# algoterranean/3dgan

Hardware: AMD Instinct MI355X
Metric: images/sec (whole node), CIFAR-10 IWGAN bs=512 (higher is better)
Workload: dtype bf16; 1 GPU; --model iwgan --dataset cifar(32x32x3 synthetic) --batch_size 512/GPU --latent_size 200 --optimizer adam --lr 1e-4 --beta1 0.5 --beta2 0.9 --n_disc_train 5; one step = 5 D + 1 G optimizer steps on 6 fresh batches; global_batch=512, parallelism=dp1, ranks_seen=1

## Files before the change

### 3dgan_amd/_lib.py

```python
import ctypes as C
import os

_HERE = os.path.dirname(os.path.abspath(__file__))
LIB_PATH = os.environ.get('TDG_LIB_PATH') or os.path.join(_HERE, 'lib3dgan_hip.so')

F32, BF16 = 0, 1
ACT_NONE, ACT_RELU, ACT_LRELU, ACT_TANH, ACT_SIGMOID = 0, 1, 2, 3, 4
MASK_NONE, MASK_LRELU, MASK_RELU = 0, 1, 2
COL_NONE, COL_SUM, COL_BN = 0, 1, 2


class ConvDesc(C.Structure):
    _fields_ = [(n, C.c_int32) for n in
                ('n', 'h', 'w', 'c', 'cs', 'oh', 'ow', 'k', 'ks', 'kh', 'kw', 'stride', 'pad_t', 'pad_l', 'dtype')]


class Epilogue(C.Structure):
    _fields_ = [('bias', C.c_void_p), ('act', C.c_int32), ('leak', C.c_float),
                ('mask_mode', C.c_int32), ('mask_src', C.c_void_p), ('accumulate', C.c_int32),
                ('col_partial', C.c_void_p), ('col_partial_bytes', C.c_size_t), ('col_mode', C.c_int32),
                ('col_images', C.c_int32), ('col_nblk_out', C.POINTER(C.c_int32)),
                ('splitk_ws', C.c_void_p), ('splitk_ws_bytes', C.c_size_t)]


class PackJob(C.Structure):
    _fields_ = [('desc', ConvDesc), ('w', C.c_void_p), ('packed_fwd', C.c_void_p), ('packed_bwd', C.c_void_p)]


class LaunchRecord(C.Structure):
    _fields_ = [('kernel', C.c_char * 64), ('ms', C.c_double), ('flops', C.c_double)]


_vp, _i, _f, _sz, _u64 = C.c_void_p, C.c_int, C.c_float, C.c_size_t, C.c_uint64
_PD, _PE = C.POINTER(ConvDesc), C.POINTER(Epilogue)

SIGNATURES = {
    'tdg_last_error': (C.c_char_p, []),
    'tdg_version': (_i, []),
    'tdg_last_kernel': (C.c_char_p, []),
    'tdg_timing_begin': (_i, []),
    'tdg_timing_end': (_i, [C.POINTER(LaunchRecord), _i, C.POINTER(_i)]),
    'tdg_packed_filter_fwd_bytes': (_sz, [_PD]),
    'tdg_packed_filter_bwd_bytes': (_sz, [_PD]),
    'tdg_pack_filter_fwd': (_i, [_PD, _vp, _vp, _vp]),
    'tdg_pack_filter_bwd': (_i, [_PD, _vp, _vp, _vp]),
    'tdg_pack_filters': (_i, [C.POINTER(PackJob), _i, _vp]),
    'tdg_conv2d_fwd': (_i, [_PD, _i, _vp, _vp, _vp, _PE, _vp]),
    'tdg_conv2d_bwd_data': (_i, [_PD, _i, _vp, _vp, _vp, _PE, _vp]),
    'tdg_conv2d_bwd_filter_workspace_bytes': (_sz, [_PD, _i]),
    'tdg_conv2d_bwd_filter': (_i, [_PD, _i, _vp, _vp, _vp, _f, _vp, _sz, _vp]),
    'tdg_conv2d_bwd_filter2': (_i, [_PD, _i, _vp, _i, _vp, _vp, _vp, _f, _vp, _sz, _vp]),
    'tdg_conv2d_dispatch': (_i, [_PD, _i, _i, _PE, _i, C.c_char_p, _sz]),
    'tdg_rowdot': (_i, [_i, _vp, _i, _i, _vp, _vp, _i, _vp, _vp]),
    'tdg_rowouter': (_i, [_i, _vp, _vp, _i, _i, _i, _f, _vp, _vp, _vp]),
    'tdg_col_finalize_sum': (_i, [_vp, _i, _i, _vp, _f, _vp]),
    'tdg_instance_norm_fwd': (_i, [_i, _vp, _i, _i, _i, _i, _vp, _vp, _f, _i, _f, _vp, _i, _vp, _vp]),
    'tdg_instance_norm_bwd': (_i, [_i, _vp, _i, _vp, _i, _i, _i, _i, _vp, _vp, _vp, _i, _f, _vp, _vp, _vp, _f, _vp, _sz, _vp]),
    'tdg_add_act': (_i, [_i, _vp, _vp, _sz, _i, _f, _vp, _vp]),
    'tdg_bn_fwd_from_partials': (_i, [_i, _vp, _i, _i, _i, _vp, _f, _i, _f, _vp, _vp, _i, _vp, _vp, _i, _vp, _vp]),
    'tdg_colsum_weighted': (_i, [_i, _vp, _i, _i, _i, _vp, _vp, _f, _vp, _sz, _vp]),
    'tdg_colsum_workspace_bytes': (_sz, [_i, _i]),
    'tdg_bn_workspace_bytes': (_sz, [_i, _i]),
    'tdg_bn_fwd': (_i, [_i, _vp, _i, _i, _i, _vp, _f, _i, _f, _vp, _vp, _i, _vp, _vp, _sz, _vp]),
    'tdg_bn_fwd_groups': (_i, [_i, _vp, _i, _i, _i, _i, _vp, _f, _i, _f, _vp, _vp, _i, _vp, _vp, _sz, _vp]),
    'tdg_bn_bwd': (_i, [_i, _vp, _i, _vp, _i, _i, _i, _vp, _vp, _i, _f, _vp, _vp, _f, _vp, _f, _vp, _sz, _vp]),
    'tdg_affine_cast_pair': (_i, [_i, _vp, _i, _vp, _i, _sz, _f, _f, _vp, _vp, _vp]),
    'tdg_bias_act': (_i, [_i, _vp, _i, _i, _i, _vp, _i, _f, _vp, _vp]),
    'tdg_act_bwd': (_i, [_i, _vp, _vp, _sz, _i, _f, _vp, _vp]),
    'tdg_affine_cast': (_i, [_i, _vp, _sz, _f, _f, _vp, _vp]),
    'tdg_affine_cast_rows': (_i, [_i, _vp, _i, _i, _i, _f, _f, _vp, _vp]),
    'tdg_cast_to_f32': (_i, [_i, _vp, _sz, _vp, _vp]),
    'tdg_cast_from_f32': (_i, [_i, _vp, _sz, _vp, _vp]),
    'tdg_gp_interp': (_i, [_i, _vp, _vp, _vp, _i, _i, _vp, _vp]),
    'tdg_sumsq': (_i, [_i, _vp, _sz, _vp, _f, _vp, _sz, _vp]),
    'tdg_reduce_workspace_bytes': (_sz, [_sz]),
    'tdg_mean_f32': (_i, [_vp, _i, _vp, _vp]),
    'tdg_sum_f32': (_i, [_vp, _i, _vp, _f, _vp]),
    'tdg_mean_segments_f32': (_i, [_vp, _i, _i, _vp, _vp]),
    'tdg_gan_logloss': (_i, [_vp, _vp, _i, _vp, _vp, _vp, _vp, _vp]),
    'tdg_p2p_xent': (_i, [_i, _vp, _i, _i, _i, _vp, _vp, _vp]),
    'tdg_p2p_l1': (_i, [_i, _vp, _vp, _i, _i, _f, _vp, _i, _vp, _vp, _sz, _vp]),
    'tdg_cgan_prep': (_i, [_i, _vp, _i, _i, _vp, _i, _vp, _vp, _vp, _vp, _i, _vp, _i, _vp]),
    'tdg_cgan_head_fwd': (_i, [_i, _vp, _i, _i, _i, _i, _i, _vp, _vp, _vp, _vp, _vp, _i, _vp]),
    'tdg_cgan_head_bwd': (_i, [_i, _vp, _i, _vp, _i, _i, _i, _i, _i, _vp, _i, _f, _vp, _vp, _vp, _vp, _sz, _vp]),
    'tdg_cgan_head_noise_fwd': (_i, [_i, _vp, _i, _i, _i, _i, _i, _vp, _vp, _vp, _vp, _vp, _vp, _vp, _i, _vp]),
    'tdg_cgan_head_noise_bwd': (_i, [_i, _vp, _i, _vp, _i, _i, _i, _i, _i, _vp, _vp, _i, _f, _vp, _vp, _vp, _vp, _sz, _vp]),
    'tdg_cgan_join': (_i, [_i, _i, _i, _i, _i, _vp, _i, _vp, _i, _vp, _i, _vp]),
    'tdg_cgan_wgan_loss': (_i, [_i, _vp, _i, _i, _i, _vp, _vp, _vp]),
    'tdg_cgan_metrics': (_i, [_vp, _vp, _vp, _i, _i, _vp, _vp, _vp, _sz, _vp]),
    'tdg_cgan_metrics_workspace_bytes': (_sz, []),
    'tdg_cgan_eval_batch': (_i, [_vp, _vp, _vp, _vp, _f, _i, _i, _i, _vp, _vp, _vp, _sz, _vp]),
    'tdg_cgan_eval_workspace_bytes': (_sz, []),
    'tdg_cgan_eval_acc_bytes': (_sz, [_i]),
    'tdg_cgan_eval_moments': (_i, [_vp, _i, _i, _vp, _vp]),
    'tdg_cgan_eval_finish': (_i, [_vp, _vp, _i, _f, _vp, _vp, _vp, _vp]),
    'tdg_cgan_sample_stats': (_i, [_vp, _vp, _vp, _vp, _vp, _f, _i, _i, _f, _vp, _vp, _vp, _vp, _sz, _vp]),
    'tdg_cgan_sample_stats_workspace_bytes': (_sz, [_i, _i]),
    'tdg_cgan_rmse_loss': (_i, [_i, _vp, _vp, _i, _i, _vp, _i, _vp, _vp, _sz, _vp]),
    'tdg_cgan_rmse_loss_workspace_bytes': (_sz, [_i, _i]),
    'tdg_cgan_bar_fill': (_i, [_i, _vp, _i, _i, _vp, _i, _vp, _vp]),
    'tdg_mde_loss': (_i, [_i, _vp, _i, _i, _vp, _i, _vp, _vp, _i, _vp, _vp, _sz, _vp]),
    'tdg_mde_loss_workspace_bytes': (_sz, [_i]),
    'tdg_xsamp_prep': (_i, [_i, _vp, _vp, _vp, _vp, _vp, _vp, _vp, _i, _i, _i, _i, _vp, _i, _vp, _i, _vp, _i, _vp, _vp]),
    'tdg_xsamp_head_fwd': (_i, [_i, _vp, _i, _i, _i, _i, _vp, _vp, _vp, _vp, _i, _vp]),
    'tdg_xsamp_head_bwd': (_i, [_i, _vp, _i, _vp, _vp, _i, _i, _i, _i, _vp, _i, _f, _vp, _vp, _vp, _vp, _sz, _vp]),
    'tdg_cgan_full_gather': (_i, [_vp, _vp, _i, _i, _i, _vp, _i, _vp, _vp, _vp]),
    'tdg_cgan_full_store': (_i, [_vp, _vp, _i, C.c_longlong, _vp, _vp, _vp, _vp]),
    'tdg_cgan_full_blend': (_i, [_vp, _vp, C.c_longlong, _i, _i, _i, _i, _vp, _vp, _vp]),
    'tdg_cgan_full_rmse': (_i, [_vp, _vp, _i, _i, _vp, _vp, _sz, _vp]),
    'tdg_cgan_full_gather_rep': (_i, [_vp, _vp, _i, _i, _i, _vp, _i, _i, _vp, _vp, _vp]),
    'tdg_cgan_full_sample_store': (_i, [_vp, _vp, _vp, _i, _i, C.c_longlong, _vp, _vp, _vp, _vp, _vp, _vp]),
    'tdg_vae_reparam': (_i, [_i, _vp, _i, _vp, _i, _i, _i, _vp, _i, _vp]),
    'tdg_vae_reparam_bwd': (_i, [_i, _vp, _i, _vp, _i, _i, _i, _vp, _i, _vp]),
    'tdg_vae_reparam_bwd_kl': (_i, [_i, _vp, _i, _vp, _i, _vp, _i, _f, _i, _i, _vp, _i, _vp]),
    'tdg_gp_rows': (_i, [_i, _vp, _i, _i, _f, _vp, _vp, _vp]),
    'tdg_vae_kl': (_i, [_i, _vp, _i, _i, _i, _vp, _vp, _sz, _vp]),
    'tdg_vae_bce': (_i, [_i, _vp, _vp, _i, _i, _i, _vp, _vp, _vp, _sz, _vp]),
    'tdg_dropout': (_i, [_i, _vp, _i, _i, _i, _vp, _f, _vp]),
    'tdg_l1_loss': (_i, [_i, _vp, _vp, _i, _i, _i, _f, _f, _vp, _vp, _vp, _sz, _vp]),
    'tdg_gp_scalars': (_i, [_vp, _f, _vp, _vp]),
    'tdg_gp_sumsq': (_i, [_i, _vp, _sz, _vp, _f, _vp, _vp, _sz, _vp]),
    'tdg_scale_by_dev': (_i, [_i, _vp, _sz, _vp, _vp, _vp]),
    'tdg_fill_f32': (_i, [_vp, _sz, _f, _vp]),
    'tdg_bias_grad': (_i, [_i, _vp, _i, _i, _i, _vp, _f, _vp, _sz, _vp]),
    'tdg_adam_step': (_i, [_vp, _vp, _vp, _vp, _sz, _f, _f, _f, _f, _f, _vp]),
    'tdg_adam_step_dev': (_i, [_vp, _vp, _vp, _vp, _sz, _f, _f, _f, _f, _f, _vp, _vp]),
    'tdg_add_i32': (_i, [_vp, _i, _vp]),
    'tdg_rmsprop_step': (_i, [_vp, _vp, _vp, _vp, _sz, _f, _f, _f, _f, _f, _vp]),
    'tdg_rmsprop_centered_step': (_i, [_vp, _vp, _vp, _vp, _vp, _sz, _f, _f, _f, _f, _f, _vp]),
    'tdg_adagrad_step': (_i, [_vp, _vp, _vp, _sz, _f, _f, _vp]),
    'tdg_adadelta_step': (_i, [_vp, _vp, _vp, _vp, _sz, _f, _f, _f, _f, _vp]),
    'tdg_ftrl_step': (_i, [_vp, _vp, _vp, _vp, _sz, _f, _f, _f, _f, _vp]),
    'tdg_sgd_momentum_step': (_i, [_vp, _vp, _vp, _sz, _f, _f, _f, _vp]),
    'tdg_clamp': (_i, [_vp, _sz, _f, _f, _vp]),
    'tdg_check_finite': (_i, [_vp, _sz, _vp, _vp]),
# ... 43 lines not shown
```

### 3dgan_amd/csrc/tdg_elementwise.hip

```cpp
#include <stdarg.h>

#include <atomic>

#include "tdg_common.h"
#include <type_traits>

static thread_local char g_err[512] = "";
void tdg_set_error(const char* fmt, ...) {
  va_list ap;
  va_start(ap, fmt);
  vsnprintf(g_err, sizeof(g_err), fmt, ap);
  va_end(ap);
}
extern "C" const char* tdg_last_error(void) { return g_err; }
extern "C" int tdg_version(void) { return 100; }
static thread_local const char* g_last_kernel = "";
void tdg_note_kernel(const char* name) { g_last_kernel = name; }
extern "C" const char* tdg_last_kernel(void) { return g_last_kernel; }

#include <vector>
struct TimingSlot { const char* name; double flops; hipEvent_t e0, e1; };
static std::vector<TimingSlot> g_slots;
static int g_timing_on = 0, g_timing_n = 0;
bool tdg_timing_enabled() { return g_timing_on != 0; }
void tdg_timing_start(const char* name, double flops, hipStream_t s) {
  if (!g_timing_on) return;
  if (g_timing_n == (int)g_slots.size()) {
    TimingSlot t;
    t.name = ""; t.flops = 0;
    (void)hipEventCreate(&t.e0);
    (void)hipEventCreate(&t.e1);
    g_slots.push_back(t);
  }
  TimingSlot& t = g_slots[g_timing_n];
  t.name = name;
  t.flops = flops;
  (void)hipEventRecord(t.e0, s);
}
void tdg_timing_stop(hipStream_t s) {
  if (!g_timing_on) return;
  (void)hipEventRecord(g_slots[g_timing_n].e1, s);
  ++g_timing_n;
}
extern "C" int tdg_timing_begin(void) {
  g_timing_on = 1;
  g_timing_n = 0;
  return TDG_OK;
}
extern "C" int tdg_timing_end(TdgLaunchRecord* out, int capacity, int* count) {
  g_timing_on = 0;
  TDG_CHECK_ARG(count != nullptr, "tdg_timing_end: null count");
  int n = 0;
  for (int i = 0; i < g_timing_n; ++i) {
    if (hipEventSynchronize(g_slots[i].e1) != hipSuccess) { tdg_set_error("tdg_timing_end: event sync failed"); return TDG_EHIP; }
    float ms = 0.f;
    (void)hipEventElapsedTime(&ms, g_slots[i].e0, g_slots[i].e1);
    if (out && n < capacity) {
      strncpy(out[n].kernel, g_slots[i].name, sizeof(out[n].kernel) - 1);
      out[n].kernel[sizeof(out[n].kernel) - 1] = 0;
      out[n].ms = ms;
      out[n].flops = g_slots[i].flops;
    }
    ++n;
  }
  *count = n;
  g_timing_n = 0;
  return TDG_OK;
}

static inline int ew_blocks(size_t n, int per_block = 1024) {
  size_t b = (n + per_block - 1) / per_block;
  return (int)(b < 1 ? 1 : (b > 4096 ? 4096 : b));
}

__device__ __forceinline__ float wave_sum(float v) {
#pragma unroll
  for (int o = 32; o > 0; o >>= 1) v += __shfl_down(v, o, 64);
  return v;
}

__device__ __forceinline__ float block_sum256(float v, float* sh ) {
  v = wave_sum(v);
  if ((threadIdx.x & 63) == 0) sh[threadIdx.x >> 6] = v;
  __syncthreads();
  float r = 0.f;
  if (threadIdx.x == 0) r = sh[0] + sh[1] + sh[2] + sh[3];
  __syncthreads();
// ... 134 lines not shown
  const int CL = g.CL, RL = 256 / CL;
  const int tx = threadIdx.x % CL, ty = threadIdx.x / CL;
  const int r0 = blockIdx.x * g.rows_per_blk;
  const int r1 = min(g.rows, r0 + g.rows_per_blk);
  const T* x = static_cast<const T*>(a.x) + (size_t)blockIdx.z * g.rows * g.xcs;
  const T* y = static_cast<const T*>(a.y);
  float* const partial = a.partial + (size_t)blockIdx.z * gridDim.x * 2 * g.C;
  const int c = (blockIdx.y * CL + tx) * VW;
  Acc s0[VW], s1[VW];
#pragma unroll
  for (int e = 0; e < VW; ++e) s0[e] = s1[e] = 0;
  if (c < g.C) {
    float pivot[VW], bta[VW];
#pragma unroll
    for (int e = 0; e < VW; ++e) pivot[e] = bta[e] = 0.f;
    if (MODE == COL_BN_STATS) load_vw<T, VW>(x + c, pivot);
    if (MODE == COL_BN_BWD) {
#pragma unroll
      for (int e = 0; e < VW; ++e) bta[e] = a.beta[c + e];
    }
    for (int rb = r0 + ty; rb < r1; rb += 4 * RL) {
      float v4[4][VW], p4[4][VW];
#pragma unroll
      for (int u = 0; u < 4; ++u) {
        const int r = rb + u * RL;
        if (r < r1) {
          load_vw<T, VW>(x + (size_t)r * g.xcs + c, v4[u]);
          if (MODE == COL_BN_BWD) load_vw<T, VW>(y + (size_t)r * g.cs + c, p4[u]);
        }
      }
#pragma unroll
      for (int u = 0; u < 4; ++u) {
        const int r = rb + u * RL;
        if (r >= r1) continue;
        float (&v)[VW] = v4[u];
        if (MODE == COL_BN_STATS) {
#pragma unroll
          for (int e = 0; e < VW; ++e) { const float d = v[e] - pivot[e]; s0[e] += d; s1[e] += d * d; }
        } else if (MODE == COL_BN_BWD) {
          float (&pre)[VW] = p4[u];
#pragma unroll
          for (int e = 0; e < VW; ++e) {
            const float dpre = v[e] * act_deriv_from_pre(pre[e], a.act, a.leak);
            s0[e] += dpre; s1[e] += dpre * (pre[e] - bta[e]);
          }
        } else if (MODE == COL_SUM) {
#pragma unroll
          for (int e = 0; e < VW; ++e) s0[e] += v[e];
        } else {
          const float k = a.coef ? a.coef[r] : 1.f;
#pragma unroll
          for (int e = 0; e < VW; ++e) s0[e] += v[e] * k;
        }
      }
    }
  }
#pragma unroll
  for (int e = 0; e < VW; ++e) { sh[0][e][threadIdx.x] = s0[e]; sh[1][e][threadIdx.x] = s1[e]; }
  __syncthreads();
  if (ty == 0 && c < g.C) {
#pragma unroll
    for (int e = 0; e < VW; ++e) {
      Acc t0 = 0, t1 = 0;
      for (int k = 0; k < RL; ++k) { t0 += sh[0][e][k * CL + tx]; t1 += sh[1][e][k * CL + tx]; }
      partial[((size_t)blockIdx.x * 2 + 0) * g.C + c + e] = (float)t0;
      partial[((size_t)blockIdx.x * 2 + 1) * g.C + c + e] = (float)t1;
    }
  }
}

enum { FIN_BN_STATS = 0, FIN_BN_BWD = 1, FIN_ACC = 2, FIN_ACC2 = 3 };
struct FinArgs {
  const float* partial; int nblk, C, rows;
  const void* x0;
  const float* pivot_f;
  float eps;
  float* out0;
  float* out1;
  float beta_acc;
  long long x0_group;
};
#define FIN_CH 8
template <typename T, int MODE, int CH>
__global__ void __launch_bounds__(256) col_finalize_kernel(const FinArgs a) {
  constexpr int RL = 256 / CH;
  using Acc = typename std::conditional<sizeof(T) == 4, double, float>::type;
  __shared__ Acc sh[2][RL][CH];
  const int tx = threadIdx.x & (CH - 1), ty = threadIdx.x / CH;
  const int c = blockIdx.x * CH + tx;
  const float* const partial = a.partial + (size_t)blockIdx.y * a.nblk * 2 * a.C;
  Acc s0 = 0, s1 = 0;
  if (c < a.C)
    for (int b0 = ty; b0 < a.nblk; b0 += 4 * RL) {
      float p0[4], p1[4];
#pragma unroll
      for (int u = 0; u < 4; ++u) {
        const int b = b0 + RL * u;
        const bool ok = b < a.nblk;
        p0[u] = ok ? partial[((size_t)b * 2 + 0) * a.C + c] : 0.f;
        p1[u] = (ok && MODE != FIN_ACC) ? partial[((size_t)b * 2 + 1) * a.C + c] : 0.f;
      }
#pragma unroll
      for (int u = 0; u < 4; ++u) { s0 += p0[u]; s1 += p1[u]; }
    }
  sh[0][ty][tx] = s0;
  sh[1][ty][tx] = s1;
  __syncthreads();
  if (ty != 0 || c >= a.C) return;
  s0 = s1 = 0;
#pragma unroll
  for (int k = 0; k < RL; ++k) { s0 += sh[0][k][tx]; s1 += sh[1][k][tx]; }
  const Acc inv = (Acc)1 / (Acc)a.rows;
  if (MODE == FIN_BN_STATS) {
    const float pivot = a.pivot_f ? a.pivot_f[c] : (a.x0 ? to_f32<T>(static_cast<const T*>(a.x0)[(size_t)blockIdx.y * a.x0_group + c]) : 0.f);
    const Acc md = s0 * inv;
    const Acc var = s1 * inv - md * md > 0 ? s1 * inv - md * md : 0;
    float* const out = a.out0 + (size_t)blockIdx.y * 2 * a.C;
    out[c] = (float)(pivot + md);
    out[a.C + c] = (float)(1.0 / sqrt((double)var + (double)a.eps));
  } else if (MODE == FIN_BN_BWD) {
    a.out0[c] = (float)((a.beta_acc != 0.f ? (Acc)a.beta_acc * a.out0[c] : 0) + s0);
    a.out1[c] = (float)(s0 * inv);
    a.out1[a.C + c] = (float)(s1 * inv);
  } else if (MODE == FIN_ACC2) {
    a.out0[c] = (float)((a.beta_acc != 0.f ? (Acc)a.beta_acc * a.out0[c] : 0) + s0);
    a.out1[c] = (float)((a.beta_acc != 0.f ? (Acc)a.beta_acc * a.out1[c] : 0) + s1);
  } else {
    a.out0[c] = (float)((a.beta_acc != 0.f ? (Acc)a.beta_acc * a.out0[c] : 0) + s0);
  }
}
template <typename T, int MODE>
static void launch_col_finalize(const FinArgs& f, hipStream_t s, int ngroups = 1) {
  if (f.nblk >= 1024)
    hipLaunchKernelGGL((col_finalize_kernel<T, MODE, 2>), dim3((f.C + 1) / 2, ngroups), dim3(256), 0, s, f);
  else
    hipLaunchKernelGGL((col_finalize_kernel<T, MODE, FIN_CH>), dim3((f.C + FIN_CH - 1) / FIN_CH, ngroups), dim3(256), 0, s, f);
}

template <typename T, int VW>
__device__ __forceinline__ void store_vw(T* p, const float (&v)[VW]) {
  if constexpr (VW == 1) {
    p[0] = from_f32<T>(v[0]);
  } else if constexpr (sizeof(T) == 4) {
    *reinterpret_cast<f32x4*>(p) = f32x4{v[0], v[1], v[2], v[3]};
  } else {
    *reinterpret_cast<bf16x4*>(p) = bf16x4{(bf16_t)v[0], (bf16_t)v[1], (bf16_t)v[2], (bf16_t)v[3]};
  }
}

template <typename T, int VW>
__global__ void __launch_bounds__(256) bn_fwd_apply_kernel(const ColGeom g, const T* __restrict__ u,
                                                          const float* __restrict__ beta, const float* __restrict__ stats,
                                                          int act, float leak, T* __restrict__ pre, T* __restrict__ h, int hcs) {
  const int CL = g.CL, RL = 256 / CL, C = g.C;
  const int tx = threadIdx.x % CL, ty = threadIdx.x / CL;
  const int c = (blockIdx.y * CL + tx) * VW;
  if (c >= C) return;
  stats += (size_t)blockIdx.z * 2 * C;
  u += (size_t)blockIdx.z * g.rows * g.cs;
  if (pre) pre += (size_t)blockIdx.z * g.rows * g.cs;
  h += (size_t)blockIdx.z * g.rows * hcs;
  float mean[VW], rstd[VW], b[VW];
#pragma unroll
  for (int e = 0; e < VW; ++e) { mean[e] = stats[c + e]; rstd[e] = stats[C + c + e]; b[e] = beta[c + e]; }
  for (int r = blockIdx.x * RL + ty; r < g.rows; r += gridDim.x * RL) {
    const size_t i = (size_t)r * g.cs + c;
    float v[VW], p[VW], a[VW];
    load_vw<T, VW>(u + i, v);
#pragma unroll
    for (int e = 0; e < VW; ++e) { p[e] = (v[e] - mean[e]) * rstd[e] + b[e]; a[e] = apply_act(p[e], act, leak); }
    if (pre) store_vw<T, VW>(pre + i, p);
    store_vw<T, VW>(h + (size_t)r * hcs + c, a);
  }
}

template <typename T, int VW, bool DB>
__global__ void __launch_bounds__(256) bn_bwd_apply_kernel(const ColGeom g, const T* __restrict__ dh, int dhcs, const T* __restrict__ pre,
                                                          const float* __restrict__ beta, const float* __restrict__ stats,
                                                          const float* __restrict__ sums, int act, float leak, T* __restrict__ du,
                                                          float* __restrict__ db_partial) {
  __shared__ float sh[DB ? VW : 1][DB ? 256 : 1];
  const int CL = g.CL, RL = 256 / CL, C = g.C;
  const int tx = threadIdx.x % CL, ty = threadIdx.x / CL;
  const int c = (blockIdx.y * CL + tx) * VW;
  const bool okc = c < C;
  if (!DB && !okc) return;
  float rstd[VW], b[VW], m0[VW], m1[VW], acc[VW];
#pragma unroll
  for (int e = 0; e < VW; ++e) {
    rstd[e] = okc ? stats[C + c + e] : 0.f; b[e] = okc ? beta[c + e] : 0.f; m0[e] = okc ? sums[c + e] : 0.f; m1[e] = okc ? sums[C + c + e] : 0.f;
    acc[e] = 0.f;
  }
  if (okc)
    for (int r = blockIdx.x * RL + ty; r < g.rows; r += gridDim.x * RL) {
      const size_t i = (size_t)r * g.cs + c;
      float d[VW], p[VW], o[VW];
      load_vw<T, VW>(dh + (size_t)r * dhcs + c, d);
      load_vw<T, VW>(pre + i, p);
#pragma unroll
      for (int e = 0; e < VW; ++e) {
        const float f = act_deriv_from_pre(p[e], act, leak);
        o[e] = rstd[e] * (d[e] * f - m0[e] - (p[e] - b[e]) * m1[e]);
        if (DB) acc[e] += to_f32<T>(from_f32<T>(o[e]));
      }
      store_vw<T, VW>(du + i, o);
    }
  if constexpr (DB) {
#pragma unroll
    for (int e = 0; e < VW; ++e) sh[e][threadIdx.x] = acc[e];
    __syncthreads();
    if (ty == 0 && okc) {
#pragma unroll
// ... 127 lines not shown

extern "C" int tdg_bn_bwd(int dtype, const void* dh, int dh_cs, const void* pre, int rows, int c, int cs, const float* beta,
                          const float* stats, int act, float leak, void* du, float* dbeta, float beta_acc,
                          float* dbias, float dbias_acc, void* workspace, size_t workspace_bytes, void* stream) {
  TDG_CHECK_ARG(dh && pre && beta && stats && du && dbeta && workspace, "tdg_bn_bwd: null pointer");
  TDG_CHECK_ARG(rows > 0 && c > 0 && cs >= c && dh_cs >= c, "tdg_bn_bwd: bad shape");
  if (workspace_bytes < tdg_bn_workspace_bytes(rows, c)) { tdg_set_error("tdg_bn_bwd: workspace too small"); return TDG_EWORKSPACE; }
  hipStream_t s = (hipStream_t)stream;
  ColGeom g = col_geom(rows, c, cs, dh, pre, tdg_dtype_size(dtype), dh_cs % 4 == 0);
  g.xcs = dh_cs;
  ColArgs a; memset(&a, 0, sizeof(a));
  a.x = dh; a.y = pre; a.beta = beta; a.act = act; a.leak = leak; a.partial = static_cast<float*>(workspace);
  float* sums = a.partial + (size_t)1024 * 2 * c;
  FinArgs f; memset(&f, 0, sizeof(f));
  f.partial = a.partial; f.nblk = g.nblk; f.C = c; f.rows = rows; f.out0 = dbeta; f.out1 = sums; f.beta_acc = beta_acc;
  ColGeom ga = col_geom(rows, c, cs, dh, (const void*)((uintptr_t)pre | (uintptr_t)du), tdg_dtype_size(dtype), dh_cs % 4 == 0);
  ga.xcs = dh_cs;
  int arows = apply_row_blocks(ga);
  if (dbias && arows > 1024) arows = 1024;
  const dim3 agrid(arows, ga.ncol);
  FinArgs fb; memset(&fb, 0, sizeof(fb));
  fb.partial = a.partial; fb.nblk = arows; fb.C = c; fb.rows = rows; fb.out0 = dbias; fb.beta_acc = dbias_acc;
  DISPATCH_T(dtype, {
    int rc = run_col_partial<T, COL_BN_BWD>(g, a, s);
    if (rc) return rc;
    launch_col_finalize<T, FIN_BN_BWD>(f, s);
    if (dbias) {
      if (ga.vw == 4)
        hipLaunchKernelGGL((bn_bwd_apply_kernel<T, 4, true>), agrid, dim3(256), 0, s, ga, static_cast<const T*>(dh), dh_cs,
                           static_cast<const T*>(pre), beta, stats, sums, act, leak, static_cast<T*>(du), a.partial);
      else
        hipLaunchKernelGGL((bn_bwd_apply_kernel<T, 1, true>), agrid, dim3(256), 0, s, ga, static_cast<const T*>(dh), dh_cs,
                           static_cast<const T*>(pre), beta, stats, sums, act, leak, static_cast<T*>(du), a.partial);
      launch_col_finalize<T, FIN_ACC>(fb, s);
    } else {
      if (ga.vw == 4)
        hipLaunchKernelGGL((bn_bwd_apply_kernel<T, 4, false>), agrid, dim3(256), 0, s, ga, static_cast<const T*>(dh), dh_cs,
                           static_cast<const T*>(pre), beta, stats, sums, act, leak, static_cast<T*>(du), nullptr);
      else
        hipLaunchKernelGGL((bn_bwd_apply_kernel<T, 1, false>), agrid, dim3(256), 0, s, ga, static_cast<const T*>(dh), dh_cs,
                           static_cast<const T*>(pre), beta, stats, sums, act, leak, static_cast<T*>(du), nullptr);
    }
  })
  TDG_HIP_LAUNCH_CHECK("bn_bwd");
  return TDG_OK;
}

extern "C" int tdg_bias_grad(int dtype, const void* dy, int rows, int c, int cs, float* db, float beta, void* workspace,
                             size_t workspace_bytes, void* stream) {
  TDG_CHECK_ARG(dy && db && workspace && rows > 0 && c > 0 && cs >= c, "tdg_bias_grad: bad argument");
  if (workspace_bytes < tdg_bn_workspace_bytes(rows, c)) { tdg_set_error("tdg_bias_grad: workspace too small"); return TDG_EWORKSPACE; }
  hipStream_t s = (hipStream_t)stream;
  const ColGeom g = col_geom(rows, c, cs, dy, nullptr, tdg_dtype_size(dtype));
  ColArgs a; memset(&a, 0, sizeof(a));
  a.x = dy; a.partial = static_cast<float*>(workspace);
  FinArgs f; memset(&f, 0, sizeof(f));
  f.partial = a.partial; f.nblk = g.nblk; f.C = c; f.rows = rows; f.out0 = db; f.beta_acc = beta;
  DISPATCH_T(dtype, {
    int rc = run_col_partial<T, COL_SUM>(g, a, s);
    if (rc) return rc;
    launch_col_finalize<T, FIN_ACC>(f, s);
  })
  TDG_HIP_LAUNCH_CHECK("bias_grad");
  return TDG_OK;
}

extern "C" int tdg_colsum_weighted(int dtype, const void* x, int rows, int cols, int cs, const float* coef, float* dw,
                                   float beta, void* workspace, size_t workspace_bytes, void* stream) {
  TDG_CHECK_ARG(x && dw && workspace && rows > 0 && cols > 0 && cs >= cols, "tdg_colsum_weighted: bad argument");
  if (workspace_bytes < tdg_bn_workspace_bytes(rows, cols)) { tdg_set_error("tdg_colsum_weighted: workspace too small"); return TDG_EWORKSPACE; }
  hipStream_t s = (hipStream_t)stream;
  const ColGeom g = col_geom(rows, cols, cs, x, nullptr, tdg_dtype_size(dtype));
  ColArgs a; memset(&a, 0, sizeof(a));
  a.x = x; a.coef = coef; a.partial = static_cast<float*>(workspace);
  FinArgs f; memset(&f, 0, sizeof(f));
  f.partial = a.partial; f.nblk = g.nblk; f.C = cols; f.rows = rows; f.out0 = dw; f.beta_acc = beta;
  DISPATCH_T(dtype, {
    int rc = run_col_partial<T, COL_WSUM>(g, a, s);
    if (rc) return rc;
    launch_col_finalize<T, FIN_ACC>(f, s);
  })
  TDG_HIP_LAUNCH_CHECK("colsum_weighted");
  return TDG_OK;
}

template <typename T>
__global__ void __launch_bounds__(256) instance_norm_fwd_kernel(const T* __restrict__ u, int hw, int c, int cs,
                                                               const float* __restrict__ scale, const float* __restrict__ shift, float eps,
                                                               int act, float leak, T* __restrict__ h, int hcs, float* __restrict__ stats) {
  __shared__ float sh[2][4][64];
  const int n = blockIdx.x, tx = threadIdx.x & 63, ty = threadIdx.x >> 6;
  const int ch = blockIdx.y * 64 + tx;
  const bool okc = ch < c;
  const T* un = u + (size_t)n * hw * cs;
  const float pivot = okc ? to_f32<T>(un[ch]) : 0.f;
  float s0 = 0.f, s1 = 0.f;
  if (okc)
    for (int r = ty; r < hw; r += 4) { const float d = to_f32<T>(un[(size_t)r * cs + ch]) - pivot; s0 += d; s1 += d * d; }
  sh[0][ty][tx] = s0; sh[1][ty][tx] = s1;
  __syncthreads();
  s0 = sh[0][0][tx] + sh[0][1][tx] + sh[0][2][tx] + sh[0][3][tx];
  s1 = sh[1][0][tx] + sh[1][1][tx] + sh[1][2][tx] + sh[1][3][tx];
  if (!okc) return;
  const float md = s0 / (float)hw, var = fmaxf(s1 / (float)hw - md * md, 0.f);
  const float mu = pivot + md, rstd = rsqrtf(var + eps);
  if (ty == 0) { stats[((size_t)n * 2 + 0) * c + ch] = mu; stats[((size_t)n * 2 + 1) * c + ch] = rstd; }
  const float g = scale[ch], b = shift[ch];
  T* hn = h + (size_t)n * hw * hcs;
  for (int r = ty; r < hw; r += 4)
    hn[(size_t)r * hcs + ch] = from_f32<T>(apply_act(g * (to_f32<T>(un[(size_t)r * cs + ch]) - mu) * rstd + b, act, leak));
}
extern "C" int tdg_instance_norm_fwd(int dtype, const void* u, int n, int hw, int c, int cs, const float* scale, const float* shift,
                                     float eps, int act, float leak, void* h, int h_cs, float* stats, void* stream) {
  TDG_CHECK_ARG(u && scale && shift && h && stats && n > 0 && hw > 0 && c > 0 && cs >= c && h_cs >= c, "tdg_instance_norm_fwd: bad argument");
  DISPATCH_T(dtype, {
    hipLaunchKernelGGL(instance_norm_fwd_kernel<T>, dim3(n, (c + 63) / 64), dim3(256), 0, (hipStream_t)stream, static_cast<const T*>(u),
                       hw, c, cs, scale, shift, eps, act, leak, static_cast<T*>(h), h_cs, stats);
  })
  TDG_HIP_LAUNCH_CHECK("instance_norm_fwd");
  return TDG_OK;
}
template <typename T>
__global__ void __launch_bounds__(256) instance_norm_bwd_kernel(const T* __restrict__ dh, int dhcs, const T* __restrict__ u, int hw, int c,
                                                               int cs, const float* __restrict__ scale, const float* __restrict__ shift,
                                                               const float* __restrict__ stats, int act, float leak, T* __restrict__ du,
                                                               float* __restrict__ part) {
  __shared__ float sh[2][4][64];
  const int n = blockIdx.x, tx = threadIdx.x & 63, ty = threadIdx.x >> 6;
  const int ch = blockIdx.y * 64 + tx;
  const bool okc = ch < c;
  const T* un = u + (size_t)n * hw * cs;
  const T* dn = dh + (size_t)n * hw * dhcs;
  const float mu = okc ? stats[((size_t)n * 2 + 0) * c + ch] : 0.f, rstd = okc ? stats[((size_t)n * 2 + 1) * c + ch] : 0.f;
  const float g0 = okc ? scale[ch] : 0.f, b0 = okc ? shift[ch] : 0.f;
  float s0 = 0.f, s1 = 0.f;
  if (okc)
    for (int r = ty; r < hw; r += 4) {
      const float xh = (to_f32<T>(un[(size_t)r * cs + ch]) - mu) * rstd;
      const float g = to_f32<T>(dn[(size_t)r * dhcs + ch]) * act_deriv_from_pre(g0 * xh + b0, act, leak);
      s0 += g; s1 += g * xh;
    }
  sh[0][ty][tx] = s0; sh[1][ty][tx] = s1;
  __syncthreads();
  s0 = sh[0][0][tx] + sh[0][1][tx] + sh[0][2][tx] + sh[0][3][tx];
  s1 = sh[1][0][tx] + sh[1][1][tx] + sh[1][2][tx] + sh[1][3][tx];
  if (!okc) return;
  if (ty == 0) { part[((size_t)n * 2 + 0) * c + ch] = s1; part[((size_t)n * 2 + 1) * c + ch] = s0; }
  const float m0 = s0 / (float)hw, m1 = s1 / (float)hw;
  T* dun = du + (size_t)n * hw * cs;
  for (int r = ty; r < hw; r += 4) {
    const float xh = (to_f32<T>(un[(size_t)r * cs + ch]) - mu) * rstd;
    const float g = to_f32<T>(dn[(size_t)r * dhcs + ch]) * act_deriv_from_pre(g0 * xh + b0, act, leak);
    dun[(size_t)r * cs + ch] = from_f32<T>(g0 * rstd * (g - m0 - xh * m1));
  }
}
extern "C" int tdg_instance_norm_bwd(int dtype, const void* dh, int dh_cs, const void* u, int n, int hw, int c, int cs,
                                     const float* scale, const float* shift, const float* stats, int act, float leak, void* du,
                                     float* dscale, float* dshift, float beta, void* workspace, size_t workspace_bytes, void* stream) {
  TDG_CHECK_ARG(dh && u && scale && shift && stats && du && dscale && dshift && workspace && n > 0 && hw > 0 && c > 0 && cs >= c && dh_cs >= c,
                "tdg_instance_norm_bwd: bad argument");
  if (workspace_bytes < (size_t)n * 2 * c * sizeof(float)) { tdg_set_error("tdg_instance_norm_bwd: workspace too small"); return TDG_EWORKSPACE; }
  float* part = static_cast<float*>(workspace);
  FinArgs f; memset(&f, 0, sizeof(f));
  f.partial = part; f.nblk = n; f.C = c; f.rows = 1; f.out0 = dscale; f.out1 = dshift; f.beta_acc = beta;
  DISPATCH_T(dtype, {
    hipLaunchKernelGGL(instance_norm_bwd_kernel<T>, dim3(n, (c + 63) / 64), dim3(256), 0, (hipStream_t)stream, static_cast<const T*>(dh),
// ... 208 lines not shown
  }
  for (size_t i = blockIdx.x * (size_t)256 + threadIdx.x; i < n; i += (size_t)gridDim.x * 256) {
    const size_t r = i / c;
    const int ch = (int)(i - r * c);
    out[r * cs + ch] = from_f32<T>(scale * (in[i] + shift));
  }
}
template <typename T>
__global__ void __launch_bounds__(256) affine_cast_pair_kernel(const float* __restrict__ a, int ca, const float* __restrict__ b, int cb,
                                                              size_t rows, float scale, float shift, T* __restrict__ out_ab,
                                                              T* __restrict__ out_a0) {
  for (size_t r = blockIdx.x * (size_t)256 + threadIdx.x; r < rows; r += (size_t)gridDim.x * 256) {
    float v[4] = {0.f, 0.f, 0.f, 0.f}, w[4] = {0.f, 0.f, 0.f, 0.f};
    for (int ch = 0; ch < ca; ++ch) v[ch] = w[ch] = scale * (a[r * ca + ch] + shift);
    for (int ch = 0; ch < cb; ++ch) v[ca + ch] = scale * (b[r * cb + ch] + shift);
    store_vw<T, 4>(out_ab + r * 4, v);
    store_vw<T, 4>(out_a0 + r * 4, w);
  }
}
extern "C" int tdg_affine_cast_pair(int dtype, const float* a, int ca, const float* b, int cb, size_t rows, float scale, float shift,
                                    void* out_ab, void* out_a0, void* stream) {
  TDG_CHECK_ARG(a && b && out_ab && out_a0 && rows > 0 && ca > 0 && cb > 0 && ca + cb == 4, "tdg_affine_cast_pair: bad argument");
  TDG_CHECK_ARG((((uintptr_t)out_ab | (uintptr_t)out_a0) & 15) == 0, "tdg_affine_cast_pair: outputs must be 16-byte aligned");
  DISPATCH_T(dtype, {
    hipLaunchKernelGGL(affine_cast_pair_kernel<T>, dim3(ew_blocks(rows)), dim3(256), 0, (hipStream_t)stream, a, ca, b, cb, rows, scale,
                       shift, static_cast<T*>(out_ab), static_cast<T*>(out_a0));
  })
  TDG_HIP_LAUNCH_CHECK("affine_cast_pair");
  return TDG_OK;
}

extern "C" int tdg_affine_cast_rows(int dtype, const float* in, int rows, int c, int cs, float scale, float shift, void* out,
                                    void* stream) {
  TDG_CHECK_ARG(in && out && rows > 0 && c > 0 && cs >= c, "tdg_affine_cast_rows: bad argument");
  const size_t n = (size_t)rows * c;
  DISPATCH_T(dtype, {
    hipLaunchKernelGGL(affine_cast_rows_kernel<T>, dim3(ew_blocks(n)), dim3(256), 0, (hipStream_t)stream, in, n, c, cs, scale,
                       shift, static_cast<T*>(out));
  })
  TDG_HIP_LAUNCH_CHECK("affine_cast_rows");
  return TDG_OK;
}
extern "C" int tdg_cast_from_f32(int dtype, const float* in, size_t n, void* out, void* stream) {
  return tdg_affine_cast(dtype, in, n, 1.f, 0.f, out, stream);
}

template <typename T>
__global__ void __launch_bounds__(256) cast_to_f32_kernel(const T* __restrict__ in, size_t n, float* __restrict__ out) {
  for (size_t i = blockIdx.x * (size_t)256 + threadIdx.x; i < n; i += (size_t)gridDim.x * 256) out[i] = to_f32<T>(in[i]);
}
extern "C" int tdg_cast_to_f32(int dtype, const void* in, size_t n, float* out, void* stream) {
  TDG_CHECK_ARG(in && out && n > 0, "tdg_cast_to_f32: bad argument");
  DISPATCH_T(dtype, {
    hipLaunchKernelGGL(cast_to_f32_kernel<T>, dim3(ew_blocks(n)), dim3(256), 0, (hipStream_t)stream, static_cast<const T*>(in),
                       n, out);
  })
  TDG_HIP_LAUNCH_CHECK("cast_to_f32");
  return TDG_OK;
}

template <typename T>
__global__ void __launch_bounds__(256) gp_interp_kernel(const T* __restrict__ x, const T* __restrict__ g,
                                                       const float* __restrict__ alpha, int rows, int cols, T* __restrict__ xhat) {
  for (int r = blockIdx.x; r < rows; r += gridDim.x) {
    const float al = alpha[r];
    for (int c = threadIdx.x; c < cols; c += 256) {
      const size_t i = (size_t)r * cols + c;
      const float xv = to_f32<T>(x[i]);
      xhat[i] = from_f32<T>(xv + al * (to_f32<T>(g[i]) - xv));
    }
  }
}
extern "C" int tdg_gp_interp(int dtype, const void* x, const void* g, const float* alpha, int rows, int cols, void* xhat,
                             void* stream) {
  TDG_CHECK_ARG(x && g && alpha && xhat && rows > 0 && cols > 0, "tdg_gp_interp: bad argument");
  DISPATCH_T(dtype, {
    hipLaunchKernelGGL(gp_interp_kernel<T>, dim3(rows < 4096 ? rows : 4096), dim3(256), 0, (hipStream_t)stream,
                       static_cast<const T*>(x), static_cast<const T*>(g), alpha, rows, cols, static_cast<T*>(xhat));
  })
  TDG_HIP_LAUNCH_CHECK("gp_interp");
  return TDG_OK;
}

#define RED_BLOCKS 256
extern "C" size_t tdg_reduce_workspace_bytes(size_t) { return RED_BLOCKS * sizeof(float); }

template <typename T>
__global__ void __launch_bounds__(256) sumsq_partial_kernel(const T* __restrict__ x, size_t n, float* __restrict__ partial,
                                                           float* __restrict__ acc, float beta, float gp_lambda = 0.f,
                                                           float* __restrict__ gp_scal = nullptr) {
  __shared__ float sh[4];
  float s = 0.f;
  constexpr int VW = 16 / (int)sizeof(T);
  if ((((uintptr_t)x) & 15) == 0) {
    const size_t nv = n / VW;
    for (size_t i = blockIdx.x * (size_t)256 + threadIdx.x; i < nv; i += (size_t)gridDim.x * 256) {
      float v[VW];
      if constexpr (sizeof(T) == 2) {
        const bf16x8 t = reinterpret_cast<const bf16x8*>(x)[i];
#pragma unroll
        for (int e = 0; e < 8; ++e) v[e] = (float)t[e];
      } else {
        const f32x4 t = reinterpret_cast<const f32x4*>(x)[i];
#pragma unroll
        for (int e = 0; e < 4; ++e) v[e] = t[e];
      }
#pragma unroll
      for (int e = 0; e < VW; ++e) s += v[e] * v[e];
    }
    for (size_t i = nv * VW + blockIdx.x * (size_t)256 + threadIdx.x; i < n; i += (size_t)gridDim.x * 256) {
      const float v = to_f32<T>(x[i]);
      s += v * v;
    }
  } else {
    for (size_t i = blockIdx.x * (size_t)256 + threadIdx.x; i < n; i += (size_t)gridDim.x * 256) {
      const float v = to_f32<T>(x[i]);
      s += v * v;
    }
  }
  s = block_sum256(s, sh);
  if (threadIdx.x == 0) partial[blockIdx.x] = s;
  if (!last_block_arrives(TICKET_SUMSQ, gridDim.x)) return;
  float t = 0.f;
  for (int i = threadIdx.x; i < (int)gridDim.x; i += 256) t += partial[i];
  t = block_sum256(t, sh);
  if (threadIdx.x == 0) {
    const float ss = (beta != 0.f ? beta * acc[0] : 0.f) + t;
    acc[0] = ss;
    if (gp_scal) {
      const float sl = sqrtf(ss);
      gp_scal[0] = (sl - 1.f) * (sl - 1.f);
      gp_scal[1] = gp_lambda * 2.f * (sl - 1.f) / sl;
    }
  }
}
__global__ void __launch_bounds__(256) reduce_final_kernel(const float* __restrict__ partial, int np, float* __restrict__ acc,
                                                          float beta, float scale) {
  __shared__ float sh[4];
  const float* p = partial + (size_t)blockIdx.x * np;
  float s = 0.f;
  for (int i = threadIdx.x; i < np; i += 256) s += p[i];
  s = block_sum256(s, sh);
  if (threadIdx.x == 0) acc[blockIdx.x] = (beta != 0.f ? beta * acc[blockIdx.x] : 0.f) + scale * s;
}
__global__ void __launch_bounds__(256) reduce_mean_kernel(const float* __restrict__ partial, int np, float* __restrict__ out) {
  __shared__ float sh[4];
  const float* p = partial + (size_t)blockIdx.x * np;
  float s = 0.f;
  for (int i = threadIdx.x; i < np; i += 256) s += p[i];
  s = block_sum256(s, sh);
  if (threadIdx.x == 0) out[blockIdx.x] = s / (float)np;
}
extern "C" int tdg_sumsq(int dtype, const void* x, size_t n, float* acc, float beta, void* workspace,
                         size_t workspace_bytes, void* stream) {
  TDG_CHECK_ARG(x && acc && workspace && n > 0, "tdg_sumsq: bad argument");
  if (workspace_bytes < RED_BLOCKS * sizeof(float)) { tdg_set_error("tdg_sumsq: workspace too small"); return TDG_EWORKSPACE; }
  TDG_TICKET_STREAM("tdg_sumsq", stream);
  DISPATCH_T(dtype, {
    hipLaunchKernelGGL(sumsq_partial_kernel<T>, dim3(RED_BLOCKS), dim3(256), 0, (hipStream_t)stream, static_cast<const T*>(x),
                       n, static_cast<float*>(workspace), acc, beta);
  })
  TDG_HIP_LAUNCH_CHECK("sumsq");
  return TDG_OK;
}
extern "C" int tdg_gp_sumsq(int dtype, const void* x, size_t n, float* sumsq, float lambda, float* scal, void* workspace,
                            size_t workspace_bytes, void* stream) {
  TDG_CHECK_ARG(x && sumsq && scal && workspace && n > 0, "tdg_gp_sumsq: bad argument");
  if (workspace_bytes < RED_BLOCKS * sizeof(float)) { tdg_set_error("tdg_gp_sumsq: workspace too small"); return TDG_EWORKSPACE; }
  TDG_TICKET_STREAM("tdg_gp_sumsq", stream);
  DISPATCH_T(dtype, {
    hipLaunchKernelGGL(sumsq_partial_kernel<T>, dim3(RED_BLOCKS), dim3(256), 0, (hipStream_t)stream, static_cast<const T*>(x),
                       n, static_cast<float*>(workspace), sumsq, 0.f, lambda, scal);
  })
  TDG_HIP_LAUNCH_CHECK("gp_sumsq");
  return TDG_OK;
}
extern "C" int tdg_mean_segments_f32(const float* x, int nseg, int seglen, float* out, void* stream) {
  TDG_CHECK_ARG(x && out && nseg > 0 && nseg <= 65535 && seglen > 0, "tdg_mean_segments_f32: bad argument");
  hipLaunchKernelGGL(reduce_mean_kernel, dim3(nseg), dim3(256), 0, (hipStream_t)stream, x, seglen, out);
  TDG_HIP_LAUNCH_CHECK("mean_segments_f32");
  return TDG_OK;
}
extern "C" int tdg_sum_f32(const float* x, int n, float* out, float beta, void* stream) {
  TDG_CHECK_ARG(x && out && n > 0, "tdg_sum_f32: bad argument");
  hipLaunchKernelGGL(reduce_final_kernel, dim3(1), dim3(256), 0, (hipStream_t)stream, x, n, out, beta, 1.f);
  TDG_HIP_LAUNCH_CHECK("sum_f32");
  return TDG_OK;
}
extern "C" int tdg_mean_f32(const float* x, int n, float* out, void* stream) {
  TDG_CHECK_ARG(x && out && n > 0, "tdg_mean_f32: bad argument");
  hipLaunchKernelGGL(reduce_mean_kernel, dim3(1), dim3(256), 0, (hipStream_t)stream, x, n, out);
  TDG_HIP_LAUNCH_CHECK("mean_f32");
  return TDG_OK;
}

__global__ void __launch_bounds__(256) gan_logloss_kernel(const float* __restrict__ dr, const float* __restrict__ df, int n,
                                                         float* __restrict__ sr, float* __restrict__ sfd, float* __restrict__ sfg,
                                                         float* __restrict__ scal) {
  __shared__ float sh[4];
  float ld = 0.f, lg = 0.f;
  const float inv = 1.f / (float)n;
  for (int i = threadIdx.x; i < n; i += 256) {
    const float r = dr[i], f = df[i];
    ld += -logf(r + 1e-8f) - logf(1.f - f + 1e-8f);
    lg += -logf(f + 1e-8f);
    sr[i] = -inv / (r + 1e-8f) * r * (1.f - r);
    sfd[i] = inv / (1.f - f + 1e-8f) * f * (1.f - f);
    sfg[i] = -inv / (f + 1e-8f) * f * (1.f - f);
  }
  ld = block_sum256(ld, sh);
  lg = block_sum256(lg, sh);
  if (threadIdx.x == 0) { scal[0] = ld * inv; scal[1] = lg * inv; }
}
extern "C" int tdg_gan_logloss(const float* d_real, const float* d_fake, int n, float* seed_real, float* seed_fake_d,
                               float* seed_fake_g, float* scal, void* stream) {
  TDG_CHECK_ARG(d_real && d_fake && seed_real && seed_fake_d && seed_fake_g && scal && n > 0, "tdg_gan_logloss: bad argument");
  hipLaunchKernelGGL(gan_logloss_kernel, dim3(1), dim3(256), 0, (hipStream_t)stream, d_real, d_fake, n, seed_real, seed_fake_d,
                     seed_fake_g, scal);
  TDG_HIP_LAUNCH_CHECK("gan_logloss");
  return TDG_OK;
}

template <typename T>
__global__ void __launch_bounds__(256) p2p_xent_kernel(const T* __restrict__ z, int rows, int cs, int mode, T* __restrict__ seed,
                                                      float* __restrict__ scal) {
  __shared__ float sh[4];
  float dr = 0.f, df = 0.f, gf = 0.f;
  const float inv = 1.f / (float)rows;
  for (int i = threadIdx.x; i < rows; i += 256) {
    const float zr = to_f32<T>(z[(size_t)i * cs]), zf = to_f32<T>(z[(size_t)(rows + i) * cs]);
    const float sr = log1pf(expf(-fabsf(zr))), sf = log1pf(expf(-fabsf(zf)));
    dr += fmaxf(zr, 0.f) - zr + sr;
    df += fmaxf(zf, 0.f) + sf;
    gf += fmaxf(zf, 0.f) - zf + sf;
    if (mode) {
      const float pr = 1.f / (1.f + expf(-zr)), pf = 1.f / (1.f + expf(-zf));
      seed[(size_t)i * cs] = from_f32<T>(mode == 1 ? (pr - 1.f) * inv : 0.f);
      seed[(size_t)(rows + i) * cs] = from_f32<T>(mode == 1 ? pf * inv : (pf - 1.f) * inv);
    }
  }
  dr = block_sum256(dr, sh);
  df = block_sum256(df, sh);
  gf = block_sum256(gf, sh);
  if (threadIdx.x == 0) { scal[0] = dr * inv; scal[1] = df * inv; scal[2] = gf * inv; }
}
extern "C" int tdg_p2p_xent(int dtype, const void* logits, int rows, int cs, int mode, void* seed, float* scal, void* stream) {
  TDG_CHECK_ARG(logits && scal && rows > 0 && cs > 0 && (mode == 0 || seed), "tdg_p2p_xent: bad argument");
  DISPATCH_T(dtype, {
    hipLaunchKernelGGL(p2p_xent_kernel<T>, dim3(1), dim3(256), 0, (hipStream_t)stream, static_cast<const T*>(logits), rows, cs,
                       mode, static_cast<T*>(seed), scal);
  })
  TDG_HIP_LAUNCH_CHECK("p2p_xent");
  return TDG_OK;
}
template <typename T>
__global__ void __launch_bounds__(256) p2p_l1_kernel(const T* __restrict__ y, const T* __restrict__ g, int rows, int cs, float wgt,
                                                    T* __restrict__ dg, int dgs, float* __restrict__ partial) {
  __shared__ float sh[4];
  float a = 0.f, q = 0.f;
  const float inv = 1.f / (float)rows;
  for (int i = blockIdx.x * 256 + threadIdx.x; i < rows; i += gridDim.x * 256) {
    const float d = 0.5f * (to_f32<T>(g[(size_t)i * cs]) - to_f32<T>(y[(size_t)i * cs]));
    a += fabsf(d);
    q += d * d;
    if (dg) {
      const float s = d > 0.f ? 1.f : (d < 0.f ? -1.f : 0.f);
      dg[(size_t)i * dgs] = from_f32<T>(to_f32<T>(dg[(size_t)i * dgs]) + wgt * 0.5f * s * inv);
    }
  }
  a = block_sum256(a, sh);
  q = block_sum256(q, sh);
  if (threadIdx.x == 0) { partial[blockIdx.x] = a; partial[RED_BLOCKS + blockIdx.x] = q; }
}
__global__ void __launch_bounds__(256) p2p_l1_final_kernel(const float* __restrict__ partial, int rows, float* __restrict__ scal) {
  __shared__ float sh[4];
  float a = 0.f, q = 0.f;
// ... 584 lines not shown
```

### 3dgan_amd/csrc/tdg_igemm.hip

```cpp
#include <stdarg.h>
#include <stdlib.h>

#include "tdg_igemm.h"
#include "tdg_wgrad_patch.h"
#include <type_traits>

#define OOB_OFFSET 0xFFFFFF00u

#ifdef TDG_STAMPS
#define TDG_STAMP(var)                                                                            \
  do {                                                                                            \
    __builtin_amdgcn_sched_barrier(0);                                                            \
    asm volatile("s_memtime %0\n\ts_waitcnt lgkmcnt(0)" : "=s"(var)::"memory");                  \
    __builtin_amdgcn_sched_barrier(0);                                                            \
  } while (0)
#else
#define TDG_STAMP(var) do { } while (0)
#endif

template <int I, int N, class F>
__device__ __forceinline__ void static_for(F&& f) {
  if constexpr (I < N) {
    f(IntC<I>{});
    static_for<I + 1, N>(f);
  }
}

template <typename T>
struct Mma;
template <>
struct Mma<bf16_t> {
  using frag = bf16x8;
  static __device__ __forceinline__ void run(f32x4& acc, const frag& a, const frag& b) {
    acc = __builtin_amdgcn_mfma_f32_16x16x32_bf16(a, b, acc, 0, 0, 0);
  }
};
template <>
struct Mma<float> {
  using frag = f32x4;
  static __device__ __forceinline__ void run(f32x4& acc, const frag& a, const frag& b) {
#pragma unroll
    for (int e = 0; e < 4; ++e) acc = __builtin_amdgcn_mfma_f32_16x16x4f32(a[e], b[e], acc, 0, 0, 0);
  }
};

__device__ __forceinline__ __amdgpu_buffer_rsrc_t make_rsrc(const void* p, unsigned bytes) {
  return __builtin_amdgcn_make_buffer_rsrc(const_cast<void*>(p), 0, (int)bytes, 0x00020000);
}

__device__ __forceinline__ i32x4 make_rsrc_words(const void* p, unsigned bytes) {
  const unsigned long long a = (unsigned long long)p;
  return i32x4{(int)(unsigned)a, (int)((unsigned)(a >> 32) & 0xffffu), (int)bytes, 0x00020000};
}
__device__ __forceinline__ void lds_dma_b128(const i32x4& rsrc, unsigned voff, unsigned lds_byte) {
  asm volatile("s_mov_b32 m0, %2\n\ts_nop 0\n\tbuffer_load_dwordx4 %0, %1, 0 offen lds" ::"v"(voff), "s"(rsrc), "s"(lds_byte) : "memory");
}

template <typename T>
__device__ __forceinline__ T buffer_load_elem(__amdgpu_buffer_rsrc_t r, unsigned off);
template <>
__device__ __forceinline__ float buffer_load_elem<float>(__amdgpu_buffer_rsrc_t r, unsigned off) {
  return __builtin_bit_cast(float, __builtin_amdgcn_raw_buffer_load_b32(r, off, 0, 0));
}
template <>
__device__ __forceinline__ bf16_t buffer_load_elem<bf16_t>(__amdgpu_buffer_rsrc_t r, unsigned off) {
  return __builtin_bit_cast(bf16_t, __builtin_amdgcn_raw_buffer_load_b16(r, off, 0, 0));
}

__device__ __forceinline__ int tap_dh(int pk) { return (pk << 24) >> 24; }
__device__ __forceinline__ int tap_dw(int pk) { return (pk << 16) >> 24; }

__device__ __forceinline__ int lds_swz(int row, int chunk) {
  return row * IG_BKB + ((chunk ^ ((row >> 1) & 7)) << 4);
}

struct KChunk { int tap, cv; bool ok; };
__device__ __forceinline__ KChunk k_decode(unsigned chunk, const FastDiv& fd_ck, const FastDiv& fd_nt, int nslices) {
  const unsigned u = fd_div(chunk, fd_ck);
  const unsigned j = chunk - u * fd_ck.d;
  const unsigned sl = fd_div(u, fd_nt);
  KChunk r;
  r.tap = (int)(u - sl * fd_nt.d);
  r.cv = (int)(sl * fd_ck.d + j);
  r.ok = (int)sl < nslices;
  return r;
}

// ... 2174 lines not shown
        __builtin_amdgcn_sched_group_barrier(0x008, TK, 0);
      });
      __builtin_amdgcn_sched_barrier(0);
#ifdef TDG_STAMPS
      unsigned long long wt1, wt2, wt3;
      TDG_STAMP(wt1);
#endif
      asm volatile("s_waitcnt vmcnt(0)" ::: "memory");
#ifdef TDG_STAMPS
      TDG_STAMP(wt2);
#endif
      __syncthreads();
#ifdef TDG_STAMPS
      TDG_STAMP(wt3);
      w_wait += wt2 - wt1; w_bar += wt3 - wt2;
#endif
      __builtin_amdgcn_sched_barrier(0);
      const char* nA = smem + nstage;
      const char* nG = nA + SLAB;
      static_for<0, NTAIL>([&](auto u_c) {
        constexpr int u = decltype(u_c)::value, t = TS + u;
        constexpr int g_lo = u == 0 ? 0 : 1 + ((TNW - 1) * (u - 1)) / (NTAIL - 1 > 0 ? NTAIL - 1 : 1);
        constexpr int g_hi = u == 0 ? 1 : (u == NTAIL - 1 ? TNW : 1 + ((TNW - 1) * u) / (NTAIL - 1 > 0 ? NTAIL - 1 : 1));
        if constexpr (u == 0) static_for<0, TK>([&](auto i_c) { constexpr int i = decltype(i_c)::value; FA[0][i] = frag(nA, 0, col_a + i * 16); });
        static_for<g_lo, g_hi>([&](auto g_c) { constexpr int g = decltype(g_c)::value; FG[0][g] = frag(nG, 0, col_g + g * 16); });
        mma_tile(IntC<1>{}, IntC<t>{});
        constexpr bool has_piece = u < 8 - NPA && TDG_WG_ABLATE != 3;
        if constexpr (has_piece) ld.template piece<u>(dn2, mstep + 2 * WD_MR, stage * STAGE);
        __builtin_amdgcn_sched_group_barrier(0x100, 2 * ((u == 0 ? TK : 0) + (g_hi - g_lo)), 0);
        __builtin_amdgcn_sched_group_barrier(0x008, TK, 0);
        if constexpr (has_piece) __builtin_amdgcn_sched_group_barrier(0x020, 1, 0);
      });
      stage ^= 1;
      dn1 = dn2;
    }
    asm volatile("s_waitcnt vmcnt(0)" ::: "memory");
  };
  if constexpr (TN1 == TN) {
    run(IntC<TN>{});
  } else {
    if (wn == 0) run(IntC<TN>{});
    else run(IntC<TN1>{});
  }
  TDG_STAMP(ws2);

  float* slab = args.slabs + (size_t)split * (size_t)args.slab_stride;
  const int Ceff = (int)args.fd_c.d * VEC;
#pragma unroll
  for (int i = 0; i < TK; ++i) {
    const int kk = kk0 + wk * 64 + i * 16 + r16;
    if (kk >= args.KK) continue;
    const int tap = kk / Ceff;
    const int c = kk - tap * Ceff;
    if (c >= args.Clog) continue;
    float* rowp = slab + ((size_t)tap * args.Clog + c) * (size_t)args.Nlog;
#pragma unroll
    for (int j = 0; j < TN; ++j) {
      const int n = n0 + (wn * TN + j) * 16 + q * 4;
      if (j >= tnw) continue;
      if (n + 3 < args.Nlog && (args.Nlog & 3) == 0) {
        *reinterpret_cast<f32x4*>(rowp + n) = acc[i][j];
      } else {
#pragma unroll
        for (int e = 0; e < 4; ++e)
          if (n + e < args.Nlog) rowp[n + e] = acc[i][j][e];
      }
    }
  }
#ifdef TDG_STAMPS
  if (args.stamps) {
    asm volatile("s_waitcnt vmcnt(0)" ::: "memory");
    TDG_STAMP(ws3);
    if (lane == 0) {
      unsigned long long* o = args.stamps + (((size_t)blockIdx.z * gridDim.x + blockIdx.x) * 8 + wave) * 8;
      o[0] = ws0; o[1] = ws1; o[2] = ws2; o[3] = ws3; o[4] = (ws2 - ws1) - w_wait - w_bar; o[5] = w_wait; o[6] = w_bar;
    }
  }
#endif
}

__global__ void __launch_bounds__(256) slab_reduce_kernel(const float* __restrict__ slabs, float* __restrict__ dw,
                                                         size_t n, int nsplit, size_t stride, float beta) {
  __shared__ f32x4 sh[16][16];
  const int tx = threadIdx.x & 15, tz = threadIdx.x >> 4;
  const size_t n4 = (n + 3) >> 2;
  const size_t i = (size_t)blockIdx.x * 16 + tx;
  f32x4 s = {0.f, 0.f, 0.f, 0.f};
  if (i < n4)
    for (int z = tz; z < nsplit; z += 16) s += *reinterpret_cast<const f32x4*>(slabs + (size_t)z * stride + 4 * i);
  sh[tz][tx] = s;
  __syncthreads();
  if (tz != 0 || i >= n4) return;
  s = sh[0][tx];
#pragma unroll
  for (int k = 1; k < 16; ++k) s += sh[k][tx];
#pragma unroll
  for (int e = 0; e < 4; ++e)
    if (4 * i + e < n) dw[4 * i + e] = (beta != 0.f ? beta * dw[4 * i + e] : 0.f) + s[e];
}

__global__ void __launch_bounds__(256) slab_reduce_few_kernel(const float* __restrict__ slabs, float* __restrict__ dw,
                                                             size_t n, int nsplit, size_t stride, float beta) {
  const size_t n4 = (n + 3) >> 2;
  const size_t i = (size_t)blockIdx.x * 256 + threadIdx.x;
  if (i >= n4) return;
  f32x4 v[8];
#pragma unroll
  for (int z = 0; z < 8; ++z)
    v[z] = z < nsplit ? *reinterpret_cast<const f32x4*>(slabs + (size_t)z * stride + 4 * i) : f32x4{0.f, 0.f, 0.f, 0.f};
  f32x4 s = v[0];
#pragma unroll
  for (int z = 1; z < 8; ++z) s += v[z];
  if (4 * i + 3 < n) {
    f32x4 o = s;
    if (beta != 0.f) o += beta * *reinterpret_cast<const f32x4*>(dw + 4 * i);
    *reinterpret_cast<f32x4*>(dw + 4 * i) = o;
  } else {
#pragma unroll
    for (int e = 0; e < 4; ++e)
      if (4 * i + e < n) dw[4 * i + e] = (beta != 0.f ? beta * dw[4 * i + e] : 0.f) + s[e];
  }
}

struct PackArgs {
  const float* w;
  void* out;
  int rows, ntaps, C, Ceff, Kp;
  int CK;
  int stride_tap, stride_row, stride_ch;
  FastDiv fd_slice, fd_ck;
  unsigned char tap_ids[IG_MAX_TAPS];
};
static inline void pack_finish(PackArgs* a) {
  a->fd_slice = make_fastdiv((uint32_t)(a->ntaps * a->CK));
  a->fd_ck = make_fastdiv((uint32_t)a->CK);
}

#define PACK_TK 64
#define PACK_RT 4
template <typename T>
__device__ __forceinline__ void pack_tiles(const PackArgs& a, int bx, int byg, float (*tile)[33]) {
  const int k0 = bx * PACK_TK;
  const int tx = threadIdx.x & 31, ty = threadIdx.x >> 5;
  const bool row_fast = a.stride_row == 1;
  const int kmax = a.ntaps * a.Ceff;
  auto k_src = [&](int k) -> int {
    if (k >= kmax) return -1;
    const int sl = (int)fd_div((unsigned)k, a.fd_slice), kr = k - sl * (a.ntaps * a.CK);
    const int ti = (int)fd_div((unsigned)kr, a.fd_ck), c = sl * a.CK + (kr - ti * a.CK);
    return c < a.C ? (int)a.tap_ids[ti] * a.stride_tap + c * a.stride_ch : -1;
  };
  int ks[PACK_TK / 8];
  if (row_fast) {
#pragma unroll
    for (int p = 0; p < PACK_TK / 8; ++p) ks[p] = k_src(k0 + ty + 8 * p);
  } else {
#pragma unroll
    for (int h = 0; h < PACK_TK / 32; ++h) ks[h] = k_src(k0 + h * 32 + tx);
  }
  T* out = static_cast<T*>(a.out);
  for (int s = 0; s < PACK_RT; ++s) {
    const int r0 = (byg * PACK_RT + s) * 32;
    if (r0 >= a.rows) break;
    if (row_fast) {
      const int r = r0 + tx;
#pragma unroll
      for (int p = 0; p < PACK_TK / 8; ++p)
        tile[ty + 8 * p][tx] = (ks[p] >= 0 && r < a.rows) ? a.w[(size_t)ks[p] + (size_t)r] : 0.f;
    } else {
#pragma unroll
      for (int h = 0; h < PACK_TK / 32; ++h)
#pragma unroll
        for (int p = 0; p < 4; ++p) {
          const int i = ty + 8 * p, r = r0 + i;
          tile[h * 32 + tx][i] = (ks[h] >= 0 && r < a.rows) ? a.w[(size_t)ks[h] + (size_t)r * a.stride_row] : 0.f;
        }
    }
    __syncthreads();
#pragma unroll
    for (int p = 0; p < 4; ++p) {
      const int rl = ty + 8 * p;
      const int r = r0 + rl, k = k0 + 2 * tx;
      if (r >= a.rows || k >= a.Kp) continue;
      const float v0 = tile[2 * tx][rl], v1 = tile[2 * tx + 1][rl];
      if (k + 1 < a.Kp && ((a.Kp & 1) == 0)) {
        if constexpr (sizeof(T) == 2) {
          typedef bf16_t bf16x2_t __attribute__((ext_vector_type(2)));
          *reinterpret_cast<bf16x2_t*>(out + (size_t)r * a.Kp + k) = bf16x2_t{(bf16_t)v0, (bf16_t)v1};
        } else {
          *reinterpret_cast<float2*>(out + (size_t)r * a.Kp + k) = float2{v0, v1};
        }
      } else {
        out[(size_t)r * a.Kp + k] = from_f32<T>(v0);
        if (k + 1 < a.Kp) out[(size_t)r * a.Kp + k + 1] = from_f32<T>(v1);
      }
    }
    __syncthreads();
  }
}

template <typename T>
__global__ void __launch_bounds__(256) pack_filter_kernel(const PackArgs a) {
  __shared__ float tile[PACK_TK][33];
  pack_tiles<T>(a, blockIdx.x, blockIdx.y, tile);
// ... 1822 lines not shown
        case 1: hipLaunchKernelGGL(bwd_col2im_kernel<1>, grid, dim3(256), cp.lds, s, f); break;
        case 2: hipLaunchKernelGGL(bwd_col2im_kernel<2>, grid, dim3(256), cp.lds, s, f); break;
        case 3: hipLaunchKernelGGL(bwd_col2im_kernel<3>, grid, dim3(256), cp.lds, s, f); break;
        case 4: hipLaunchKernelGGL(bwd_col2im_kernel<4>, grid, dim3(256), cp.lds, s, f); break;
        default: hipLaunchKernelGGL(bwd_col2im_kernel<5>, grid, dim3(256), cp.lds, s, f); break;
      }
    });
  }
  if (p.form == BWD_FUSED) {
    if (dry) return answer(dry, "bwd_fused_kernel<bf16>");
    const FusedPlan& fp = p.fp;
    FusedBwdArgs f;
    memset(&f, 0, sizeof(f));
    f.y = static_cast<const bf16_t*>(y);
    f.w = static_cast<const bf16_t*>(wp);
    f.x = static_cast<bf16_t*>(x);
    set_epilogue(f, epi);
    f.SH = d->oh; f.SW = d->ow; f.Cs = d->ks; f.ke = fp.ke;
    f.OH = d->h; f.OW = d->w; f.Cso = d->cs; f.C = d->c;
    f.GH = fp.GH; f.GW = fp.GW;
    f.nhm = fp.nhm; f.nwm = fp.nwm; f.dh_min = fp.dh_min; f.dw_min = fp.dw_min; f.ntap = fp.ntap;
    f.KP = fp.KP; f.PP = fp.PP; f.wpitch = fp.wpitch; f.TA = fp.TA; f.ntr = fp.ntr; f.TW = fp.TW; f.ntc = fp.ntc; f.y_off = fp.y_off;
    f.fd_vpp = make_fastdiv(fp.PP / 8);
    f.fd_hc = make_fastdiv(fp.TW + fp.nwm - 1);
#ifdef TDG_STAMPS
    f.stamps = stamp_ptr();
#endif
    return tdg_launch<bwd_fused_kernel>("bwd_fused_kernel<bf16>", 160 * 1024, flops, s, [&] {
      hipLaunchKernelGGL(bwd_fused_kernel, dim3(n_images * fp.ntr * fp.ntc), dim3(512), fp.lds, s, f);
    });
  }
  IgArgs a = ig_args(y, wp, x, epi);
  a.src_bytes = (unsigned)((long long)n_images * d->oh * d->ow * d->ks * p.es);
  a.w_bytes = (unsigned)p.bytes;
  a.SH = d->oh; a.SW = d->ow; a.sigma = 1;
  a.C = p.C; a.Cs = d->ks;
  a.fd_c = make_fastdiv(p.veca ? p.C / p.vec : p.C);
  a.fd_ck = make_fastdiv(p.ck);
  a.nslices = (int)(a.fd_c.d / a.fd_ck.d);
  a.N = d->c; a.OH = d->h; a.OW = d->w; a.os = d->stride; a.Cso = d->cs;
  for (int i = 0; i < p.nc; ++i) {
    const BwdClassPlan& pc = p.cls[i];
    if (pc.ntaps == 0 || pc.GH <= 0 || pc.GW <= 0) {
      TDG_CHECK_ARG(pc.GH <= 0 || pc.GW <= 0, "tdg_conv2d_bwd_data: filter smaller than stride");
      continue;
    }
    IgClass& c = a.cls[a.nclasses++];
    c.M = n_images * pc.GH * pc.GW;
    c.GH = pc.GH; c.GW = pc.GW;
    c.ntaps = pc.ntaps;
    c.K = c.ntaps * p.C;
    c.Kp = p.Kp[i];
    c.nsteps = p.Kp[i] / p.bke;
    c.oh0 = pc.oh0; c.ow0 = pc.ow0;
    c.w_off_bytes = (unsigned)p.off[i];
    c.fd_ghw = make_fastdiv(c.GH * c.GW);
    c.fd_gw = make_fastdiv(c.GW);
    for (int t = 0; t < c.ntaps; ++t) c.tap[t] = pack_tap(pc.dh[t], pc.dw[t]);
    c.nh = pc.nh; c.nw = pc.nw; c.dh0 = pc.dh[0]; c.dw0 = pc.dw[0]; c.sh = c.sw = -1;
    c.fd_nw = make_fastdiv(c.nw);
    c.fd_nt = make_fastdiv(c.ntaps);
  }
  return choose_and_launch_fwd(a, p.veca, pick_bn(d->c), d->dtype, flops, epi, sw, s, dry);
}

int tdg_conv2d_bwd_data(const TdgConvDesc* d, int n_images, const void* y, const void* wp, void* x,
                        const TdgEpilogue* epi, void* stream) {
  return conv_bwd_data(d, n_images, y, wp, x, epi, (hipStream_t)stream, nullptr);
}

size_t tdg_conv2d_bwd_filter_workspace_bytes(const TdgConvDesc* d, int n_images) {
  if (validate_desc(d, "tdg_conv2d_bwd_filter_workspace_bytes") != TDG_OK) return 0;
  return plan_wgrad(d, n_images, conv_switches()).ws_bytes;
}

static int validate_wgrad(const TdgConvDesc* d, int n_images) {
  int rc = validate_desc(d, "tdg_conv2d_bwd_filter");
  if (rc) return rc;
  TDG_CHECK_ARG(n_images > 0 && n_images <= d->n, "tdg_conv2d_bwd_filter: n_images %d outside (0, %d]", n_images, d->n);
  return TDG_OK;
}

static int bwd_filter_impl(const TdgConvDesc* d, const ConvSwitches& sw, int n_images, const void* x, int n_first, const void* x2,
                           const void* y, float* dw, float beta, void* workspace, size_t workspace_bytes, hipStream_t s, const char** dry);

static int conv_bwd_filter(const TdgConvDesc* d, int n_images, const void* x, const void* y, float* dw, float beta, void* workspace,
                           size_t workspace_bytes, hipStream_t s, const char** dry) {
  const int rc = validate_wgrad(d, n_images);
  if (rc) return rc;
  return bwd_filter_impl(d, conv_switches(), n_images, x, n_images, nullptr, y, dw, beta, workspace, workspace_bytes, s, dry);
}

static int conv_bwd_filter2(const TdgConvDesc* d, int n_images, const void* x, int n_first, const void* x2, const void* y, float* dw,
                            float beta, void* workspace, size_t workspace_bytes, hipStream_t s, const char** dry) {
  TDG_CHECK_ARG(n_first > 0 && n_first < n_images && x2, "tdg_conv2d_bwd_filter2: n_first %d outside (0, %d) or null x2", n_first, n_images);
  int rc = validate_wgrad(d, n_images);
  if (rc) return rc;
  const ConvSwitches sw = conv_switches();
  if (plan_wgrad(d, n_images, sw).dma && ((long long)n_first * d->oh * d->ow) % 2 == 0)
    return bwd_filter_impl(d, sw, n_images, x, n_first, x2, y, dw, beta, workspace, workspace_bytes, s, dry);
  rc = bwd_filter_impl(d, sw, n_first, x, n_first, nullptr, y, dw, beta, workspace, workspace_bytes, s, dry);
  if (rc) return rc;
  const char* y2 = static_cast<const char*>(y) + (size_t)n_first * d->oh * d->ow * d->ks * tdg_dtype_size(d->dtype);
  const int n2 = n_images - n_first;
  return bwd_filter_impl(d, sw, n2, x2, n2, nullptr, y2, dw, 1.0f, workspace, workspace_bytes, s, dry);
}

static int bwd_filter_impl(const TdgConvDesc* d, const ConvSwitches& sw, int n_images, const void* x, int n_first, const void* x2,
                           const void* y, float* dw, float beta, void* workspace, size_t workspace_bytes, hipStream_t s, const char** dry) {
  const WgradPlan p = plan_wgrad(d, n_images, sw);
  TDG_CHECK_ARG(x && y && dw && workspace, "tdg_conv2d_bwd_filter: null pointer");
  if (workspace_bytes < p.ws_bytes) {
    tdg_set_error("tdg_conv2d_bwd_filter: workspace %zu < %zu bytes", workspace_bytes, p.ws_bytes);
    return TDG_EWORKSPACE;
  }
  const int es = tdg_dtype_size(d->dtype), vec = 16 / es;
  const int ce = eff_channels(d->c, d->cs, vec);
  const bool veca = ce != 0;
  const int C = veca ? ce : d->c;
  TDG_CHECK_ARG(d->ks % vec == 0, "tdg_conv2d_bwd_filter: small-side channel stride %d not a multiple of %d", d->ks, vec);
  TDG_CHECK_ARG(((uintptr_t)y & 15) == 0 && (!veca || ((uintptr_t)x & 15) == 0), "tdg_conv2d_bwd_filter: operands must be 16-byte aligned");
  WgArgs a;
  memset(&a, 0, sizeof(a));
  a.src = x;
  a.g = y;
  a.slabs = static_cast<float*>(workspace);
  a.src_bytes = (unsigned)((long long)n_first * d->h * d->w * d->cs * es);
  a.src2 = x2;
  a.src2_bytes = (unsigned)((long long)(n_images - n_first) * d->h * d->w * d->cs * es);
  a.g_bytes = (unsigned)((long long)n_images * d->oh * d->ow * d->ks * es);
  a.M = n_images * d->oh * d->ow;
  a.m_switch = n_first * d->oh * d->ow;
  a.img_switch = n_first;
  TDG_CHECK_ARG(!x2 || ((uintptr_t)x2 & 15) == 0, "tdg_conv2d_bwd_filter2: x2 must be 16-byte aligned");
  a.GH = d->oh; a.GW = d->ow; a.SH = d->h; a.SW = d->w; a.sigma = d->stride;
  a.C = C; a.Clog = d->c; a.Cs = d->cs; a.ntaps = d->kh * d->kw;
  a.KK = a.ntaps * C;
  a.fd_c = make_fastdiv(veca ? C / vec : C);
  a.fd_ghw = make_fastdiv(d->oh * d->ow);
  a.fd_gw = make_fastdiv(d->ow);
  a.N = (int)tdg_round_up(d->k, vec) <= d->ks ? (int)tdg_round_up(d->k, vec) : d->k;
  a.Gs = d->ks;
  a.Nlog = d->k;
  a.nsplit = p.nsplit;
  a.m_per_split = p.m_per_split;
  a.slab_stride = tdg_round_up((long long)a.ntaps * d->c * d->k, 4);
  a.ntiles_n = tdg_ceil_div(a.N, p.bn);
  a.ntiles_k = p.ntiles_k;
  for (int kh = 0; kh < d->kh; ++kh)
    for (int kw = 0; kw < d->kw; ++kw) a.tap[kh * d->kw + kw] = pack_tap(kh - d->pad_t, kw - d->pad_l);
  const WgChoice c = choose_wgrad(d, p, a, veca, sw);
  if (dry) return answer(dry, wgrad_choice_name(c));
  const int rc = launch_wgrad(a, c, conv_flops(d, n_images), s);
  if (rc) return rc;
  const size_t n = (size_t)a.ntaps * d->c * d->k;
  return tdg_launch("slab_reduce", 0, 0.0, s, [&] {
    if (a.nsplit <= 8 && ((uintptr_t)dw & 15) == 0) {
      hipLaunchKernelGGL(slab_reduce_few_kernel, dim3((unsigned)(((n + 3) / 4 + 255) / 256)), dim3(256), 0, s, a.slabs, dw, n, a.nsplit,
                         (size_t)a.slab_stride, beta);
    } else {
      const int blocks = (int)(((n + 3) / 4 + 15) / 16);
      hipLaunchKernelGGL(slab_reduce_kernel, dim3(blocks), dim3(256), 0, s, a.slabs, dw, n, a.nsplit, (size_t)a.slab_stride, beta);
    }
  }, false);
}

int tdg_conv2d_bwd_filter(const TdgConvDesc* d, int n_images, const void* x, const void* y, float* dw,
                          float beta, void* workspace, size_t workspace_bytes, void* stream) {
  return conv_bwd_filter(d, n_images, x, y, dw, beta, workspace, workspace_bytes, (hipStream_t)stream, nullptr);
}

int tdg_conv2d_bwd_filter2(const TdgConvDesc* d, int n_images, const void* x, int n_first, const void* x2, const void* y,
                           float* dw, float beta, void* workspace, size_t workspace_bytes, void* stream) {
  return conv_bwd_filter2(d, n_images, x, n_first, x2, y, dw, beta, workspace, workspace_bytes, (hipStream_t)stream, nullptr);
}

int tdg_conv2d_dispatch(const TdgConvDesc* d, int n_images, int form, const TdgEpilogue* epi, int n_first, char* name, size_t name_bytes) {
  TDG_CHECK_ARG(name && name_bytes > 0, "tdg_conv2d_dispatch: no name buffer");
  name[0] = 0;
  void* const p = reinterpret_cast<void*>((uintptr_t)4096);
  TdgEpilogue e;
  int nblk = 0;
  if (epi) {
    e = *epi;
    if (e.col_nblk_out) e.col_nblk_out = &nblk;
  }
  const char* kernel = nullptr;
  int rc;
  switch (form) {
    case TDG_FORM_FWD: rc = conv_fwd(d, n_images, p, p, p, epi ? &e : nullptr, nullptr, &kernel); break;
    case TDG_FORM_BWD_DATA: rc = conv_bwd_data(d, n_images, p, p, p, epi ? &e : nullptr, nullptr, &kernel); break;
    case TDG_FORM_BWD_FILTER:
      rc = n_first ? conv_bwd_filter2(d, n_images, p, n_first, p, p, static_cast<float*>(p), 0.f, p, (size_t)-1, nullptr, &kernel)
                   : conv_bwd_filter(d, n_images, p, p, static_cast<float*>(p), 0.f, p, (size_t)-1, nullptr, &kernel);
      break;
    default: TDG_CHECK_ARG(false, "tdg_conv2d_dispatch: bad form %d", form);
  }
  if (rc == TDG_OK) snprintf(name, name_bytes, "%s", kernel);
  return rc;
}

}
```

### 3dgan_amd/engine.py

```python
import collections
import ctypes as C
import math

import numpy as np
import torch

from . import _lib
from . import kernels as K
from .ops import activations as A


Part = collections.namedtuple('Part', 'name store optimizer repack')


def default_session(args):
    from .runtime import Session
    return Session(dtype=getattr(args, 'dtype_code', K.BF16), seed=getattr(args, 'seed', 0) or 0)


class Replica:

    def __init__(self, args, sess=None):
        self.args = args
        self.sess = sess = sess or default_session(args)
        self.parts, self._staging = [], ()
        self.use_graphs = bool(getattr(args, 'use_graphs', True)) and sess.device.type == 'cuda'
        self._warm, self._graphs = set(), {}

    @classmethod
    def train_function(cls, x, args, sess=None):
        replica = cls(x, args, sess)

        def train_func(sess_=None, args_=None):
            return replica.train_func(sess_, args_)
        train_func.replica = replica
        return train_func

    def register(self, name, store, optimizer, repack):
        self.parts.append(Part(name, store, optimizer, repack))

    def stores(self):
        return [p.store for p in self.parts]

    def optimizers(self):
        return {'optimizers/' + p.name: p.optimizer for p in self.parts}

    def refresh(self):
        for p in self.parts:
            p.repack()

    def load_variables(self, arrays):
        for store in self.stores():
            store.load(arrays)
        self.refresh()

    def variables(self):
        d = {}
        for store in self.stores():
            d.update(store.state_dict())
        return d

    def gradients(self):
        d = {}
        for store in self.stores():
            d.update(store.grads_dict())
        return d

    def staging(self, *shapes):
        self._staging = tuple(torch.zeros(*s, dtype=torch.float32, device=self.sess.device) for s in shapes)
        return self._staging

    def _stage(self, batch):
        for buf, t in zip(self._staging, batch if len(self._staging) > 1 else (batch,)):
            buf.copy_(t.reshape(buf.shape))

    def _run(self, name, body):
        if not self.use_graphs or self.sess.inject:
            return body()
        g = self._graphs.get(name)
        if g is not None:
            return g.replay()
        if name not in self._warm:
            self._warm.add(name)
            return body()
        torch.cuda.synchronize()
        g = torch.cuda.CUDAGraph()
        with torch.cuda.graph(g, capture_error_mode='thread_local'):
            body()
        self._graphs[name] = g
        g.replay()

    def optimizer_step(self, store, grads, apply, what):
        self._run(*grads)
        self.sess.assert_finite(store, what)
        self._scale = self.sess.allreduce_mean_scale(store.grads)
        self._run(*apply)
        self.sess.global_step += 1


class ParamStore:

    def __init__(self, device):
        self.device = device
        self.index = {}
        self.size = 0
        self.params = self.grads = None
        self.views, self.grad_views = {}, {}

    def declare(self, name, shape):
        if name in self.index:
            raise ValueError('variable %s already exists' % name)
        n = int(np.prod(shape))
        self.index[name] = (self.size, tuple(shape))
        self.size += (n + 3) // 4 * 4

    def allocate(self):
        self.params = torch.zeros(self.size, dtype=torch.float32, device=self.device)
        self.grads = torch.zeros(self.size, dtype=torch.float32, device=self.device)
        for name, (off, shape) in self.index.items():
            n = int(np.prod(shape))
            self.views[name] = self.params[off:off + n].view(shape)
            self.grad_views[name] = self.grads[off:off + n].view(shape)

    def __getitem__(self, name):
        return self.views[name]

    def grad(self, name):
        return self.grad_views[name]

    def load(self, arrays):
        for name in self.index:
            self.views[name].copy_(torch.as_tensor(np.asarray(arrays[name]), dtype=torch.float32))

    def state_dict(self):
        return {k: v.detach().cpu().numpy().copy() for k, v in self.views.items()}

    def grads_dict(self):
        return {k: v.detach().cpu().numpy().copy() for k, v in self.grad_views.items()}

    def num_params(self):
        return sum(int(np.prod(s)) for _, s in self.index.values())


def xavier_uniform_(t, shape, gen):
    if len(shape) == 1:
        fan_in = fan_out = shape[0]
    else:
        rf = int(np.prod(shape[:-2])) if len(shape) > 2 else 1
        fan_in, fan_out = rf * shape[-2], rf * shape[-1]
    lim = math.sqrt(6.0 / (fan_in + fan_out))
    t.copy_((torch.rand(shape, generator=gen, dtype=torch.float32) * 2 - 1) * lim)


def init_variable(store, name, shape, init, gen):
    cpu = torch.empty(shape, dtype=torch.float32)
    if init == 'xavier':
        xavier_uniform_(cpu, shape, gen)
    else:
        cpu.copy_(torch.randn(shape, generator=gen) * 0.02)
    store[name].copy_(cpu)


def declare_weights(store, net, layers):
    for l in layers:
        store.declare(net.var_name(l, 'weights'), l.filter_shape)
        store.declare(net.var_name(l, 'bias'), (l.out_size,))


def init_weights(store, net, layers, gen):
    for l in layers:
        init_variable(store, net.var_name(l, 'weights'), l.filter_shape, l.init, gen)
        init_variable(store, net.var_name(l, 'bias'), (l.out_size,), l.init, gen)


def conv_pads(spec, big, small):
    if spec.padding != 'SAME':
        return 0, 0
    return (max((small.h - 1) * spec.stride + spec.k - big.h, 0) // 2,
            max((small.w - 1) * spec.stride + spec.k - big.w, 0) // 2)


class Optimizer:

    def __init__(self, store):
        self.store = store
        self.t = 0

    def _slot(self, fill=0.0):
        return torch.full_like(self.store.params, fill)

# ... 254 lines not shown

    def share_filters(self, other):
        for L, O in zip(self.layers, other.layers):
            if L.rowdot:
                continue
            if L.spec.kind == 'residual' or L.spec is not O.spec:
                raise NotImplementedError('share_filters: layer %s' % L.spec.name)
            if (L.conv.fwd_bytes, L.conv.bwd_bytes) != (O.conv.fwd_bytes, O.conv.bwd_bytes):
                raise ValueError('layer %s: packed filter sizes differ between the two bindings' % L.spec.name)
            L.conv.w_fwd, L.conv.w_bwd = O.conv.w_fwd, O.conv.w_bwd
        self._pack_jobs = ()

    def forward_groups(self, ngroups, n):
        if ngroups * n > self.cap:
            raise ValueError('%d x %d images, capacity %d' % (ngroups, n, self.cap))
        for L in self.layers:
            if L.rowdot or L.spec.kind == 'residual' or L.spec.use_in:
                raise NotImplementedError('forward_groups: layer %s' % L.spec.name)
            rn = ngroups * n * L.rpi
            bias = self.store[L.bname]
            if L.spec.use_bn:
                epi, target = K.epilogue(bias=bias), L.pre
            else:
                epi, target = K.epilogue(bias=bias, act=L.act.code, leak=L.act.leak), L.h
            if L.spec.kind == 'deconv2d':
                L.conv.bwd_data(L.inp.ptr(0), target.ptr(0), rn, epi)
            else:
                L.conv.fwd(L.inp.ptr(0), target.ptr(0), rn, epi)
            if L.spec.use_bn:
                C = L.spec.out_size
                if getattr(L, 'bn_stats_groups', None) is None or L.bn_stats_groups.numel() < ngroups * 2 * C:
                    L.bn_stats_groups = torch.zeros(ngroups * 2 * C, dtype=torch.float32, device=self.device)
                K.bn_fwd_groups(self.ws, L.pre, C, self.store[L.bn_names[0]], L.act.code, None, L.h, L.bn_stats_groups,
                                n * L.rpi * L.h.h * L.h.w, ngroups, leak=L.act.leak)
        return self.layers[-1].h

    def forward(self, img0, n, bn_pass=0, keep_pre=True):
        for L in self.layers:
            r0, rn = img0 * L.rpi, n * L.rpi
            if L.rowdot:
                cols = L.spec.in_size
                _lib.call('tdg_rowdot', self.dtype, L.inp.ptr(r0), rn, cols, K.ptr(self.store[L.wname]),
                          K.ptr(self.store[L.bname]), L.act.code, K.ptr(L.out, 4 * r0), K.stream())
                continue
            if L.spec.kind == 'residual':
                L.res.forward(r0, rn, bn_pass)
                continue
            bias = self.store[L.bname]
            if L.spec.use_in:
                epi = K.epilogue(bias=bias)
                target = L.pre
            elif L.spec.use_bn:
                epi = K.colsum_epilogue(self.ws, rn * L.h.h * L.h.w, L.spec.out_size, K.COL_BN, bias=bias)
                target = L.pre
            else:
                epi = K.epilogue(bias=bias, act=L.act.code, leak=L.act.leak)
                target = L.h
            if L.spec.kind == 'deconv2d':
                L.conv.bwd_data(L.inp.ptr(r0), target.ptr(r0), rn, epi)
            else:
                L.conv.fwd(L.inp.ptr(r0), target.ptr(r0), rn, epi)
            if L.spec.use_in:
                K.in_fwd(L.pre, rn, L.spec.out_size, self.store[L.in_names[0]], self.store[L.in_names[1]], L.act.code, L.h,
                         L.in_stats[r0 * 2 * L.spec.out_size:], leak=L.act.leak, u_ptr=L.pre.ptr(r0), h_ptr=L.h.ptr(r0))
            elif L.spec.use_bn:
                rows = rn * L.h.h * L.h.w
                if K.nblk(epi):
                    K.bn_fwd_from_partials(epi, L.pre, L.spec.out_size, self.store[L.bn_names[bn_pass]], L.act.code,
                                           L.pre if keep_pre else None, L.h,
                                           L.bn_stats[bn_pass], bias, rows=rows, leak=L.act.leak,
                                           u_ptr=L.pre.ptr(r0), pre_ptr=L.pre.ptr(r0), h_ptr=L.h.ptr(r0))
                else:
                    K.bn_fwd(self.ws, L.pre, L.spec.out_size, self.store[L.bn_names[bn_pass]], L.act.code, L.pre, L.h,
                             L.bn_stats[bn_pass], rows=rows, leak=L.act.leak,
                             u_ptr=L.pre.ptr(r0), pre_ptr=L.pre.ptr(r0), h_ptr=L.h.ptr(r0))
        last = self.layers[-1]
        return last.out if last.rowdot else last.h

    def backward(self, img0, n, bn_pass=0, want_params=True, want_dx=False, acc=False, param_images=None,
                 dx_images=None, defer_wgrad=False):
        beta = 1.0 if acc else 0.0
        p0, pn = (img0, n) if param_images is None else param_images
        g = self.store.grad
        have_db = None
        for L in reversed(self.layers):
            r0, rn = img0 * L.rpi, n * L.rpi
            q0, qn = p0 * L.rpi, pn * L.rpi
            below = self.layers[L.idx - 1] if L.idx > 0 else None
            need_in = below is not None or want_dx
            d0, dn, dimg = r0, rn, img0
            if below is None and want_dx and dx_images is not None:
                d0, dn, dimg = dx_images[0] * L.rpi, dx_images[1] * L.rpi, dx_images[0]
            if below is not None and not below.spec.normed and below.spec.kind != 'residual' and below.act.code in (K.ACT_LRELU, K.ACT_RELU):
                mmode = K.MASK_LRELU if below.act.code == K.ACT_LRELU else K.MASK_RELU
                msrc, mleak = below.h, below.act.leak
            else:
                mmode, msrc, mleak = K.MASK_NONE, None, 0.0
            if L.rowdot:
                cols = L.spec.in_size
                if want_params and qn > 0:
                    K.colsum_weighted(self.ws, self.dtype, L.inp.ptr(q0), qn, cols, cols, _sub(L.seed, q0, qn),
                                      g(L.wname), beta)
                    _lib.call('tdg_sum_f32', K.ptr(L.seed, 4 * q0), qn, K.ptr(g(L.bname)), beta, K.stream())
                if need_in:
                    _lib.call('tdg_rowouter', self.dtype, K.ptr(L.seed, 4 * d0), K.ptr(self.store[L.wname]), dn, cols,
                              mmode, mleak, msrc.ptr(dimg * below.rpi) if msrc is not None else None, L.gin.ptr(d0), K.stream())
                continue
            if L.spec.kind == 'residual':
                L.res.backward(r0, rn, q0, qn, bn_pass, want_params, beta, need_in, mmode, mleak,
                               msrc.ptr(dimg * below.rpi) if msrc is not None else None)
                have_db = None
                continue
            hw = L.h.h * L.h.w
            if L.spec.use_in:
                scale, shift = self.store[L.in_names[0]], self.store[L.in_names[1]]
                if want_params:
                    dsc, dsh = g(L.in_names[0]), g(L.in_names[1])
                else:
                    if getattr(L, 'in_sink', None) is None:
                        L.in_sink = torch.zeros(2 * L.spec.out_size, dtype=torch.float32, device=self.device)
                    dsc, dsh = L.in_sink[:L.spec.out_size], L.in_sink[L.spec.out_size:]
                K.in_bwd(self.ws, L.gout, L.pre, rn, L.spec.out_size, scale, shift, L.in_stats[r0 * 2 * L.spec.out_size:], L.act.code,
                         L.delta, dsc, dsh, leak=L.act.leak, beta=beta if want_params else 0.0,
                         dh_ptr=L.gout.ptr(r0), u_ptr=L.pre.ptr(r0), du_ptr=L.delta.ptr(r0))
            elif L.spec.use_bn:
                if want_params:
                    dbeta = g(L.bn_names[bn_pass])
                else:
                    if getattr(L, 'dbeta_sink', None) is None:
                        L.dbeta_sink = torch.zeros(L.spec.out_size, dtype=torch.float32, device=self.device)
                    dbeta = L.dbeta_sink
                db_here = want_params and (q0, qn) == (r0, rn)
                K.bn_bwd(self.ws, L.gout, L.pre, L.spec.out_size, self.store[L.bn_names[bn_pass]], L.bn_stats[bn_pass],
                         L.act.code, L.delta, dbeta, rows=rn * hw, leak=L.act.leak, beta_acc=0.0,
                         dh_ptr=L.gout.ptr(r0), pre_ptr=L.pre.ptr(r0), du_ptr=L.delta.ptr(r0),
                         dbias=g(L.bname) if db_here else None, dbias_acc=beta)
                if db_here:
                    have_db = (L, None)
            elif L.act.code in (K.ACT_TANH, K.ACT_SIGMOID):
                _lib.call('tdg_act_bwd', self.dtype, L.gout.ptr(r0), L.h.ptr(r0), rn * L.h.image_elems, L.act.code,
                          L.act.leak, L.delta.ptr(r0), K.stream())
            elif L.idx == len(self.layers) - 1 and L.act.code in (K.ACT_LRELU, K.ACT_RELU):
                _lib.call('tdg_act_bwd', self.dtype, L.gout.ptr(r0), L.h.ptr(r0), rn * L.h.image_elems, L.act.code,
                          L.act.leak, L.delta.ptr(r0), K.stream())
            if want_params and qn > 0:
                if have_db is not None and have_db[0] is L and have_db[1] is None:
                    pass
                elif have_db is not None and have_db[0] is L and K.nblk(have_db[1]):
                    K.bias_grad_from_partials(have_db[1], L.spec.out_size, g(L.bname), beta)
                else:
                    K.bias_grad(self.ws, L.delta, L.spec.out_size, g(L.bname), rows=qn * hw, beta=beta, dy_ptr=L.delta.ptr(q0))
                if defer_wgrad:
                    pass
                elif L.spec.kind == 'deconv2d':
                    L.conv.bwd_filter(L.delta.ptr(q0), L.inp.ptr(q0), g(L.wname), qn, beta)
                else:
                    L.conv.bwd_filter(L.inp.ptr(q0), L.delta.ptr(q0), g(L.wname), qn, beta)
            if need_in:
                mptr = msrc.ptr(dimg * below.rpi) if msrc is not None else None
                fuse = (want_params and below is not None and not below.rowdot and not below.spec.normed and below.spec.kind != 'residual' and
                        below.act.code in (K.ACT_LRELU, K.ACT_RELU, K.ACT_NONE) and below.gout is below.delta and
                        L.rpi == 1 and below.rpi == 1 and p0 == img0 and 0 < pn <= n and (d0, dn) == (r0, rn))
                if fuse:
                    epi = K.colsum_epilogue(self.ws, dn * below.h.h * below.h.w, below.spec.out_size, K.COL_SUM,
                                            images=(pn if pn < n else 0), mask_mode=mmode, leak=mleak, mask_src=mptr)
                    have_db = (below, epi)
                else:
                    epi = K.epilogue(mask_mode=mmode, leak=mleak, mask_src=mptr)
                    have_db = None
                if L.spec.kind == 'deconv2d':
                    L.conv.fwd(L.delta.ptr(d0), L.gin.ptr(d0), dn, epi)
                else:
                    L.conv.bwd_data(L.delta.ptr(d0), L.gin.ptr(d0), dn, epi)
        return self.dx

    def tangent_forward(self, img0, n, acc=True):
        beta = 1.0 if acc else 0.0
        g = self.store.grad
        t_prev = self.tan_in
        for L in self.layers:
            r0, rn = img0 * L.rpi, n * L.rpi
            if L.rowdot:
                cols = L.spec.in_size
                K.colsum_weighted(self.ws, self.dtype, t_prev.ptr(0), rn, cols, cols, None, g(L.wname), beta)
                break
            if L.spec.normed or L.spec.kind != 'conv2d' or L.act.code not in (K.ACT_LRELU, K.ACT_RELU):
                raise NotImplementedError('tangent pass: layer %s is not a BN-free (l)relu conv' % L.spec.name)
            L.tan_src = _alias_rows(t_prev, L.rpi, *L.spec.in_shape) if t_prev is not self.tan_in else self.tan_in
            mmode = K.MASK_LRELU if L.act.code == K.ACT_LRELU else K.MASK_RELU
            L.conv.fwd(L.tan_src.ptr(0), L.tan.ptr(0), rn, K.epilogue(mask_mode=mmode, leak=L.act.leak, mask_src=L.h.ptr(r0)))
            t_prev = L.tan

    def tangent_wgrad(self, img0, n, layers, acc=True):
        beta = 1.0 if acc else 0.0
        for L in layers:
            L.conv.bwd_filter(L.tan_src.ptr(0), L.delta.ptr(img0 * L.rpi), self.store.grad(L.wname), n * L.rpi, beta)

    def conv_layers(self):
        return [L for L in self.layers if not L.rowdot]

    def merged_wgrad(self, n_first, n_tan, layers, acc=False):
        beta = 1.0 if acc else 0.0
        for L in layers:
            L.conv.bwd_filter2(L.inp.ptr(0), n_first * L.rpi, L.tan_src.ptr(0), L.delta.ptr(0), self.store.grad(L.wname),
                               (n_first + n_tan) * L.rpi, beta)

    def tangent_backward(self, img0, n, acc=True):
        beta = 1.0 if acc else 0.0
        g = self.store.grad
        t_prev = self.tan_in
        for L in self.layers:
            r0, rn = img0 * L.rpi, n * L.rpi
            if L.rowdot:
                cols = L.spec.in_size
                K.colsum_weighted(self.ws, self.dtype, t_prev.ptr(0), rn, cols, cols, None, g(L.wname), beta)
                break
            if L.spec.normed or L.spec.kind != 'conv2d' or L.act.code not in (K.ACT_LRELU, K.ACT_RELU):
                raise NotImplementedError('tangent pass: layer %s is not a BN-free (l)relu conv' % L.spec.name)
            t_in = _alias_rows(t_prev, L.rpi, *L.spec.in_shape) if t_prev is not self.tan_in else self.tan_in
            L.conv.bwd_filter(t_in.ptr(0), L.delta.ptr(r0), g(L.wname), rn, beta)
            mmode = K.MASK_LRELU if L.act.code == K.ACT_LRELU else K.MASK_RELU
            L.conv.fwd(t_in.ptr(0), L.tan.ptr(0), rn, K.epilogue(mask_mode=mmode, leak=L.act.leak, mask_src=L.h.ptr(r0)))
            t_prev = L.tan


class Residual:

    def __init__(self, seq, L, net, idx, capacity, n_bn_passes):
        self.seq, self.L, self.net, self.idx = seq, L, net, idx
        spec = self.spec = L.spec
        dt, dev = seq.dtype, seq.device
        oh, ow, oc = spec.out_shape
        A = lambda: K.Act(capacity, oh, ow, oc, dt, dev)
        self.S, self.hA, self.T = A(), A(), A()
        self.dZ, self.dT, self.dhA, self.dS = A(), A(), A(), A()
        self.preA = A() if spec.use_bn else None
        self.preB = A() if spec.use_bn else None
        pt = max((oh - 1) + spec.k - spec.in_shape[0], 0) // 2
        pl = max((ow - 1) + spec.k - spec.in_shape[1], 0) // 2
        self.convA = K.Conv(L.inp, self.S, spec.k, spec.k, 1, pt, pl)
        self.convB = K.Conv(self.hA, self.T, spec.k, spec.k, 1, pt, pl)
        self.names = {w: '%s/vars/%s%s/%s' % (net.name, spec.name, ab, w2) for ab in 'AB' for w2 in ('weights', 'bias')
                      for w in ['%s%s' % (ab, w2[0])]}
        self.shapes = {'Aw': (spec.k, spec.k, spec.in_size, oc), 'Ab': (oc,), 'Bw': (spec.k, spec.k, oc, oc), 'Bb': (oc,)}
        self._sink = torch.zeros(oc, dtype=torch.float32, device=dev)
        if spec.use_bn:
            self.statsA = [torch.zeros(2 * oc, dtype=torch.float32, device=dev) for _ in range(n_bn_passes)]
            self.statsB = [torch.zeros(2 * oc, dtype=torch.float32, device=dev) for _ in range(n_bn_passes)]
            self.bnA = [net.bn_name(p, idx, 0) for p in range(n_bn_passes)]
            self.bnB = [net.bn_name(p, idx, 1) for p in range(n_bn_passes)]

    def declare(self, store):
        for k in ('Aw', 'Ab', 'Bw', 'Bb'):
            store.declare(self.names[k], self.shapes[k])

    def declare_bn(self, store, p):
        if self.spec.use_bn:
            store.declare(self.bnA[p], (self.spec.out_size,))
            store.declare(self.bnB[p], (self.spec.out_size,))

    def variables(self):
        return [(self.names[k], self.shapes[k]) for k in ('Aw', 'Ab', 'Bw', 'Bb')]

    def pack_jobs(self, store):
        return [self.convA.pack_job(store[self.names['Aw']]), self.convB.pack_job(store[self.names['Bw']])]

    def forward(self, r0, rn, bn_pass):
        st, sp, L, ws = self.seq.store, self.spec, self.L, self.seq.ws
        act, oc, dt = L.act, sp.out_size, self.seq.dtype
        rows = rn * self.S.h * self.S.w
        nel = rn * self.S.image_elems
        self.convA.fwd(L.inp.ptr(r0), self.S.ptr(r0), rn, K.epilogue(bias=st[self.names['Ab']]))
        if sp.use_bn:
            K.bn_fwd(ws, self.S, oc, st[self.bnA[bn_pass]], act.code, self.preA, self.hA, self.statsA[bn_pass], rows=rows,
                     leak=act.leak, u_ptr=self.S.ptr(r0), pre_ptr=self.preA.ptr(r0), h_ptr=self.hA.ptr(r0))
        else:
            _lib.call('tdg_bias_act', dt, self.S.ptr(r0), rows, oc, self.S.cs, None, act.code, act.leak, self.hA.ptr(r0), K.stream())
        self.convB.fwd(self.hA.ptr(r0), self.T.ptr(r0), rn, K.epilogue(bias=st[self.names['Bb']]))
        branch = self.T
        if sp.use_bn:
            K.bn_fwd(ws, self.T, oc, st[self.bnB[bn_pass]], K.ACT_NONE, self.preB, self.preB, self.statsB[bn_pass], rows=rows,
                     u_ptr=self.T.ptr(r0), pre_ptr=self.preB.ptr(r0), h_ptr=self.preB.ptr(r0))
            branch = self.preB
        K.add_act(dt, branch.ptr(r0), self.S.ptr(r0), nel, L.h.ptr(r0), act.code, act.leak)

    def backward(self, r0, rn, q0, qn, bn_pass, want_params, beta, need_in, mmode, mleak, mptr):
        st, g, sp, L, ws = self.seq.store, self.seq.store.grad, self.spec, self.L, self.seq.ws
        act, oc, dt = L.act, sp.out_size, self.seq.dtype
# ... 45 lines not shown
```

### 3dgan_amd/kernels.py

```python
import ctypes as C

import torch

from . import _lib
from ._lib import (F32, BF16, ACT_NONE, ACT_RELU, ACT_LRELU, ACT_TANH, ACT_SIGMOID,
                   MASK_NONE, MASK_LRELU, MASK_RELU, COL_NONE, COL_SUM, COL_BN, ConvDesc, Epilogue)

TORCH_DTYPE = {F32: torch.float32, BF16: torch.bfloat16}
ELEM_SIZE = {F32: 4, BF16: 2}


def stream():
    return C.c_void_p(torch.cuda.current_stream().cuda_stream)


def ptr(t, byte_offset=0):
    if t is None:
        return C.c_void_p(0)
    return C.c_void_p(t.data_ptr() + byte_offset)


def pad_channels(c, multiple=8):
    return (c + multiple - 1) // multiple * multiple


class Act:

    def __init__(self, n, h, w, c, dtype, device, cs=None, buf=None):
        self.n, self.h, self.w, self.c = n, h, w, c
        self.cs = pad_channels(c) if cs is None else cs
        self.dtype = dtype
        self.buf = buf if buf is not None else torch.zeros(n * h * w * self.cs, dtype=TORCH_DTYPE[dtype], device=device)

    @property
    def rows(self):
        return self.n * self.h * self.w

    @property
    def image_elems(self):
        return self.h * self.w * self.cs

    def ptr(self, image=0):
        return ptr(self.buf, image * self.image_elems * ELEM_SIZE[self.dtype])

    def view(self, image0, count):
        e = self.image_elems
        return Act(count, self.h, self.w, self.c, self.dtype, self.buf.device, self.cs,
                   self.buf[image0 * e:(image0 + count) * e])

    def like(self):
        return Act(self.n, self.h, self.w, self.c, self.dtype, self.buf.device, self.cs)

    def window(self, c_off, c):
        assert c_off + c <= self.cs
        return Act(self.n, self.h, self.w, c, self.dtype, self.buf.device, self.cs, self.buf[c_off:])

    def set(self, array):
        t = torch.as_tensor(array, dtype=torch.float32).reshape(self.n, self.h, self.w, self.c)
        full = torch.zeros(self.n, self.h, self.w, self.cs, dtype=torch.float32)
        full[..., :self.c] = t
        self.buf.copy_(full.reshape(-1).to(self.buf.device, TORCH_DTYPE[self.dtype]))
        return self

    def get(self):
        return self.buf.float().reshape(self.n, self.h, self.w, self.cs)[..., :self.c].cpu().numpy()


def conv_desc(big, small, kh, kw, stride, pad_t, pad_l):
    assert big.dtype == small.dtype and big.n == small.n
    return ConvDesc(big.n, big.h, big.w, big.c, big.cs, small.h, small.w, small.c, small.cs,
                    kh, kw, stride, pad_t, pad_l, big.dtype)


_SPLITK = {}


def splitk_workspace(device):
    buf = _SPLITK.get(device)
    if buf is None:
        buf = _SPLITK[device] = torch.empty(64 << 20, dtype=torch.uint8, device=device)
    return buf


def epilogue(bias=None, act=ACT_NONE, leak=0.2, mask_mode=MASK_NONE, mask_src=None, accumulate=False):
    e = Epilogue()
    e.accumulate = 1 if accumulate else 0
    e.bias = bias.data_ptr() if bias is not None else None
    e.act, e.leak, e.mask_mode = act, leak, mask_mode
    e.mask_src = mask_src if isinstance(mask_src, int) or mask_src is None else mask_src.value
    return e


def colsum_epilogue(ws, rows, c, mode, images=0, **kw):
    e = epilogue(**kw)
    nblk_max = rows // 64 + 8
    nbytes = nblk_max * 2 * c * 4
    buf = ws.ensure(nbytes)
    e.col_partial, e.col_partial_bytes, e.col_mode, e.col_images = buf.data_ptr(), nbytes, mode, images
    e._nblk = C.c_int32(0)
    e.col_nblk_out = C.pointer(e._nblk)
    return e


def nblk(e):
    return int(e._nblk.value) if hasattr(e, '_nblk') else 0


def bias_grad_from_partials(e, c, db, beta=0.0):
    _lib.call('tdg_col_finalize_sum', C.c_void_p(e.col_partial), nblk(e), c, ptr(db), beta, stream())


def bn_fwd_from_partials(e, u, c, beta, act, pre, h, stats, bias, rows=None, leak=0.2, eps=1e-3, u_ptr=None, pre_ptr=None, h_ptr=None):
    rows = u.rows if rows is None else rows
    _lib.call('tdg_bn_fwd_from_partials', u.dtype, u_ptr or u.ptr(), rows, c, u.cs, ptr(beta), eps, act, leak,
              (pre_ptr or pre.ptr()) if pre is not None else None, h_ptr or h.ptr(), h.cs, ptr(stats), C.c_void_p(e.col_partial),
              nblk(e), ptr(bias), stream())


class GemmTimer:

    def __init__(self):
        self.records = []

    def wrap(self, kind, flops, fn):
        a, b = torch.cuda.Event(enable_timing=True), torch.cuda.Event(enable_timing=True)
        a.record()
        fn()
        b.record()
        symbol = _lib.load().tdg_last_kernel().decode()
        self.records.append((kind, a, b, flops, symbol))

    def summary(self, by_symbol=False):
        out = {}
        for kind, a, b, fl, symbol in self.records:
            key = symbol if by_symbol else kind
            n, ms, f = out.get(key, (0, 0.0, 0.0))
            out[key] = (n + 1, ms + a.elapsed_time(b), f + fl)
        return out


TIMER = None


def timing_begin():
    _lib.call('tdg_timing_begin')


def timing_end(capacity=65536):
    buf = (_lib.LaunchRecord * capacity)()
    n = C.c_int(0)
    _lib.call('tdg_timing_end', buf, capacity, C.byref(n))
    return [(buf[i].kernel.decode(), buf[i].ms, buf[i].flops) for i in range(min(n.value, capacity))]


def pack_all(jobs):
    _lib.call('tdg_pack_filters', jobs, len(jobs), stream())


def make_pack_jobs(job_list):
    return (_lib.PackJob * len(job_list))(*job_list)


class Conv:

    def __init__(self, big, small, kh, kw, stride, pad_t, pad_l):
        self.big, self.small = big, small
        self.desc = conv_desc(big, small, kh, kw, stride, pad_t, pad_l)
        lib = _lib.load()
        dev = big.buf.device
        self.fwd_bytes = lib.tdg_packed_filter_fwd_bytes(C.byref(self.desc))
        self.bwd_bytes = lib.tdg_packed_filter_bwd_bytes(C.byref(self.desc))
        if self.fwd_bytes == 0 or self.bwd_bytes == 0:
            raise _lib.TdgError('conv descriptor rejected: %s' % lib.tdg_last_error().decode())
        self.w_fwd = torch.zeros(self.fwd_bytes, dtype=torch.uint8, device=dev)
        self.w_bwd = torch.zeros(self.bwd_bytes, dtype=torch.uint8, device=dev)
        self.ws_bytes = lib.tdg_conv2d_bwd_filter_workspace_bytes(C.byref(self.desc), big.n)
        self.ws = None
        self.filter_shape = (kh, kw, big.c, small.c)

    def workspace(self):
        if self.ws is None:
            self.ws = torch.empty(max(self.ws_bytes, 16), dtype=torch.uint8, device=self.big.buf.device)
        return self.ws

    def pack(self, w, fwd=True, bwd=True):
        if fwd:
            _lib.call('tdg_pack_filter_fwd', C.byref(self.desc), ptr(w), ptr(self.w_fwd), stream())
        if bwd:
            _lib.call('tdg_pack_filter_bwd', C.byref(self.desc), ptr(w), ptr(self.w_bwd), stream())

    def pack_job(self, w, fwd=True, bwd=True):
        return _lib.PackJob(self.desc, ptr(w), ptr(self.w_fwd) if fwd else None, ptr(self.w_bwd) if bwd else None)

    def flops(self, n_images):
        d = self.desc
        return 2.0 * n_images * d.oh * d.ow * d.kh * d.kw * d.c * d.k

    def _tag(self, form):
        d = self.desc
        return '%s/%s/%dx%d_c%d_k%d' % (form, 'bf16' if d.dtype == BF16 else 'f32', d.kh, d.kw, d.c, d.k)

    def _with_splitk(self, epi):
        if epi is None:
            epi = epilogue()
        ws = splitk_workspace(self.big.buf.device)
        epi.splitk_ws, epi.splitk_ws_bytes = ws.data_ptr(), ws.numel()
        return epi

    def fwd(self, x_ptr, y_ptr, n_images, epi=None):
        epi = self._with_splitk(epi)

        def go():
            _lib.call('tdg_conv2d_fwd', C.byref(self.desc), n_images, x_ptr, ptr(self.w_fwd), y_ptr,
                      C.byref(epi) if epi is not None else None, stream())
        TIMER.wrap(self._tag('fwd'), self.flops(n_images), go) if TIMER is not None else go()

    def bwd_data(self, y_ptr, x_ptr, n_images, epi=None):
        epi = self._with_splitk(epi)

        def go():
            _lib.call('tdg_conv2d_bwd_data', C.byref(self.desc), n_images, y_ptr, ptr(self.w_bwd), x_ptr,
                      C.byref(epi) if epi is not None else None, stream())
        TIMER.wrap(self._tag('bwd_data'), self.flops(n_images), go) if TIMER is not None else go()

    def bwd_filter(self, x_ptr, y_ptr, dw, n_images, beta=0.0):
        ws = self.workspace()

        def go():
            _lib.call('tdg_conv2d_bwd_filter', C.byref(self.desc), n_images, x_ptr, y_ptr, ptr(dw), beta,
                      ptr(ws), ws.numel(), stream())
        TIMER.wrap(self._tag('bwd_filter'), self.flops(n_images), go) if TIMER is not None else go()


    def bwd_filter2(self, x_ptr, n_first, x2_ptr, y_ptr, dw, n_images, beta=0.0):
        ws = self.workspace()

        def go():
            _lib.call('tdg_conv2d_bwd_filter2', C.byref(self.desc), n_images, x_ptr, n_first, x2_ptr, y_ptr, ptr(dw), beta,
                      ptr(ws), ws.numel(), stream())
        TIMER.wrap(self._tag('bwd_filter'), self.flops(n_images), go) if TIMER is not None else go()


class Workspace:

    def __init__(self, device, nbytes=8 << 20):
        self.buf = torch.empty(nbytes, dtype=torch.uint8, device=device)
        self._retired = []

    def ensure(self, nbytes):
        if self.buf.numel() < nbytes:
            self._retired.append(self.buf)
            self.buf = torch.empty(nbytes, dtype=torch.uint8, device=self.buf.device)
        return self.buf


def bn_fwd(ws, u, c, beta, act, pre, h, stats, rows=None, leak=0.2, eps=1e-3, u_ptr=None, pre_ptr=None, h_ptr=None):
    rows = u.rows if rows is None else rows
    lib = _lib.load()
    need = lib.tdg_bn_workspace_bytes(rows, c)
    w = ws.ensure(need)
    _lib.call('tdg_bn_fwd', u.dtype, u_ptr or u.ptr(), rows, c, u.cs, ptr(beta), eps, act, leak,
              pre_ptr or pre.ptr(), h_ptr or h.ptr(), h.cs, ptr(stats), ptr(w), w.numel(), stream())


def bn_fwd_groups(ws, u, c, beta, act, pre, h, stats, rows_per_group, ngroups, leak=0.2, eps=1e-3, u_ptr=None, pre_ptr=None, h_ptr=None):
    need = ngroups * _lib.load().tdg_bn_workspace_bytes(rows_per_group, c)
    w = ws.ensure(need)
    _lib.call('tdg_bn_fwd_groups', u.dtype, u_ptr or u.ptr(), rows_per_group, ngroups, c, u.cs, ptr(beta), eps, act, leak,
              (pre_ptr or pre.ptr()) if pre is not None else None, h_ptr or h.ptr(), h.cs, ptr(stats), ptr(w), w.numel(), stream())


def bn_bwd(ws, dh, pre, c, beta, stats, act, du, dbeta, rows=None, leak=0.2, beta_acc=0.0,
           dh_ptr=None, pre_ptr=None, du_ptr=None, dbias=None, dbias_acc=0.0):
    rows = dh.rows if rows is None else rows
    lib = _lib.load()
    need = lib.tdg_bn_workspace_bytes(rows, c)
    w = ws.ensure(need)
    _lib.call('tdg_bn_bwd', dh.dtype, dh_ptr or dh.ptr(), dh.cs, pre_ptr or pre.ptr(), rows, c, pre.cs, ptr(beta), ptr(stats),
              act, leak, du_ptr or du.ptr(), ptr(dbeta), beta_acc, ptr(dbias) if dbias is not None else None, dbias_acc,
              ptr(w), w.numel(), stream())


def bias_grad(ws, dy, c, db, rows=None, beta=0.0, dy_ptr=None):
    rows = dy.rows if rows is None else rows
    need = _lib.load().tdg_bn_workspace_bytes(rows, c)
    w = ws.ensure(need)
    _lib.call('tdg_bias_grad', dy.dtype, dy_ptr or dy.ptr(), rows, c, dy.cs, ptr(db), beta, ptr(w), w.numel(), stream())


def colsum_weighted(ws, dtype, x_ptr, rows, cols, cs, coef, dw, beta=0.0):
    need = _lib.load().tdg_colsum_workspace_bytes(rows, cols)
    w = ws.ensure(need)
    _lib.call('tdg_colsum_weighted', dtype, x_ptr, rows, cols, cs, ptr(coef), ptr(dw), beta, ptr(w), w.numel(), stream())


def sumsq(ws, dtype, x_ptr, n, acc, beta=0.0):
    w = ws.ensure(4096)
    _lib.call('tdg_sumsq', dtype, x_ptr, n, ptr(acc), beta, ptr(w), w.numel(), stream())


def in_fwd(u, n, c, scale, shift, act, h, stats, leak=0.2, eps=1e-3, u_ptr=None, h_ptr=None):
    _lib.call('tdg_instance_norm_fwd', u.dtype, u_ptr or u.ptr(), n, u.h * u.w, c, u.cs, ptr(scale), ptr(shift), eps, act, leak,
              h_ptr or h.ptr(), h.cs, ptr(stats), stream())


def in_bwd(ws, dh, u, n, c, scale, shift, stats, act, du, dscale, dshift, leak=0.2, beta=0.0, dh_ptr=None, u_ptr=None, du_ptr=None):
    w = ws.ensure(n * 2 * c * 4)
    _lib.call('tdg_instance_norm_bwd', dh.dtype, dh_ptr or dh.ptr(), dh.cs, u_ptr or u.ptr(), n, u.h * u.w, c, u.cs, ptr(scale),
              ptr(shift), ptr(stats), act, leak, du_ptr or du.ptr(), ptr(dscale), ptr(dshift), beta, ptr(w), w.numel(), stream())


def add_act(dtype, a_ptr, b_ptr, n_elems, out_ptr, act=ACT_NONE, leak=0.2):
    _lib.call('tdg_add_act', dtype, a_ptr, b_ptr, n_elems, act, leak, out_ptr, stream())
```

### 3dgan_amd/models/gan.py

```python
import os

import torch

from .. import _lib
from .. import kernels as K
from .. import engine
from ..ops.layers import (dense, conv2d, deconv2d, flatten, reshape, random_normal, arg_scope,
                          variable_scope, placeholder, reset_graph)
from ..ops.activations import lrelu, relu, tanh, sigmoid
from ..util import tower_scope_range, average_gradients, init_optimizer, collection_to_dict

GP_LAMBDA = 10.0


def generator(batch_size, latent_size, args, reuse=False):
    h, w, c = args.image_shape
    s0h, s0w = h // 16, w // 16
    output_dim = h * w * c
    with arg_scope([dense, deconv2d], reuse=reuse, use_batch_norm=True, activation=relu):
        z = random_normal([batch_size, latent_size])
        y = dense(z, latent_size, s0h * s0w * 4 * latent_size, name='fc1')
        y = reshape(y, [-1, s0h, s0w, 4 * latent_size])
        y = deconv2d(y, 4 * latent_size, 2 * latent_size, 5, 2, name='dc1')
        y = deconv2d(y, 2 * latent_size, latent_size, 5, 2, name='dc2')
        y = deconv2d(y, latent_size, int(latent_size / 2), 5, 2, name='dc3')
        y = deconv2d(y, int(latent_size / 2), c, 5, 2, name='dc4', activation=tanh, use_batch_norm=False)
        y = reshape(y, [-1, output_dim])
    return y


def discriminator(x, args, reuse=False):
    use_bn = False if args.model == 'iwgan' else True
    final_activation = None if args.model in ['wgan', 'iwgan'] else sigmoid
    h, w, c = args.image_shape
    with arg_scope([conv2d], use_batch_norm=use_bn, activation=lrelu, reuse=reuse):
        x = reshape(x, [-1, h, w, c])
        x = conv2d(x, c, args.latent_size, 5, 2, name='c1', use_batch_norm=False)
        x = conv2d(x, args.latent_size, args.latent_size * 2, 5, 2, name='c2')
        x = conv2d(x, args.latent_size * 2, args.latent_size * 4, 5, 2, name='c3')
        x = reshape(x, [-1, 4 * 4 * 4 * args.latent_size])
        x = dense(x, 4 * 4 * 4 * args.latent_size, 1, use_batch_norm=False, activation=final_activation,
                  name='fc2', reuse=reuse)
        x = reshape(x, [-1])
    return x


class GanReplica(engine.Replica):

    S_DREAL, S_DFAKE, S_SUMSQ, S_GP, S_GPCOEF, S_GLOSS_AUX, S_GAN_D, S_GAN_G = 0, 1, 2, 3, 4, 5, 6, 7

    def __init__(self, x_source, args, sess):
        engine.Replica.__init__(self, args, sess)
        self.x_source, sess = x_source, self.sess
        self.model = args.model
        B, L = args.batch_size, args.latent_size
        h, w, c = args.image_shape
        dev, dt = sess.device, sess.dtype
        self.B = B
        self.iwgan = self.model == 'iwgan'
        self.display_d_loss = getattr(args, 'display_d_loss', True)
        self.gp_per_sample = bool(getattr(args, 'gp_per_sample', False))
        self._pen_rows = None

        reset_graph()
        x_sym = placeholder((None, h * w * c))
        for _x, scope, gpu_id in tower_scope_range(x_sym, args.n_gpus, B, sess):
            with variable_scope('generator') as gnet:
                g_sym = generator(B, L, args, reuse=False)
            with variable_scope('discriminator') as dnet:
                d_real = discriminator(_x, args, reuse=False)
                d_fake = discriminator(g_sym, args, reuse=True)
                if self.iwgan:
                    d_hat = discriminator(placeholder((None, h * w * c)), args, reuse=True)
        self.rows_per_image = d_real.rows_per_image
        self.gnet, self.dnet = gnet, dnet

        self.nslots = 3 if self.iwgan else 2
        self.ws = K.Workspace(dev)
        self.d_store, self.g_store = engine.ParamStore(dev), engine.ParamStore(dev)
        self.D = engine.SeqNet(dnet, self.nslots * B, (h, w, c), dt, dev, self.d_store,
                               n_bn_passes=(1 if self.iwgan else 2), need_input_grad=True,
                               tangent_capacity=(B if self.iwgan else 0), ws=self.ws)
        self.G = engine.SeqNet(gnet, B, (1, 1, L), dt, dev, self.g_store, ws=self.ws,
                               out_act=self.D.x.view(B, B), out_grad=self.D.dx.view(B, B))
        nd = int(getattr(args, 'n_disc_train', 1) or 1)
        self.G_ahead, self._ahead = None, None
        if self.model != 'gan' and nd > 1 and os.environ.get('TDG_G_AHEAD', '1') != '0':
            self.n_ahead = nd
            self.G_ahead = engine.SeqNet(gnet, nd * B, (1, 1, L), dt, dev, self.g_store, ws=self.ws, forward_only=True,
                                         out_act=K.Act(nd * B, h, w, c, dt, dev, cs=self.D.x.cs))
            self.G_ahead.share_filters(self.G)
        self.D.declare_variables()
        self.G.declare_variables()
        self.d_store.allocate()
        self.g_store.allocate()
        gen = torch.Generator().manual_seed(sess.seed)
        self.G.init_variables(gen)
        self.D.init_variables(gen)
        self.g_opt, self.d_opt = init_optimizer(args, self.g_store), init_optimizer(args, self.d_store)
        self.register('generator', self.g_store, self.g_opt, self.G.repack)
        self.register('discriminator', self.d_store, self.d_opt, self.D.repack)
        self.img_elems = self.D.x.image_elems
        self._d_big_layer = max(self.D.conv_layers(), key=lambda L: self.d_store[L.wname].numel())
        (self.x_stage,) = self.staging((B, h, w, c))
        self._seed_g = None
        self.alpha = torch.zeros(B, dtype=torch.float32, device=dev)
        self.scal = torch.zeros(16, dtype=torch.float32, device=dev)
        self.refresh()

    def _load_real(self, x01):
        h, w, c = self.args.image_shape
        n = self.B * h * w * c
        if x01.dtype != torch.float32 or x01.numel() != n:
            raise ValueError('expected a float32 batch of %d values in [0,1], got %s %s' % (n, x01.dtype, tuple(x01.shape)))
        self._stage(x01)

    def _rescale_real(self):
        h, w, c = self.args.image_shape
        _lib.call('tdg_affine_cast_rows', self.sess.dtype, K.ptr(self.x_stage), self.B * h * w, c, self.D.x.cs, 2.0, -0.5,
                  self.D.x.ptr(0), K.stream())

    def _generate(self, backward_follows=True):
        self.sess.random_normal(self.G.x, self.B, 'z')
        self.G.forward(0, self.B, keep_pre=backward_follows)

    def _generate_ahead(self):
        self.sess.random_normal(self.G_ahead.x, self.n_ahead * self.B, 'z')
        self.G_ahead.forward_groups(self.n_ahead, self.B)

    def _ahead_ok(self, n_steps):
        if self.G_ahead is None or n_steps != self.n_ahead or self.sess.inject.get('z'):
            return False
        staged = self.sess.staged.get('z')
        return staged is None or staged.numel() >= self.n_ahead * self.B * self.G_ahead.x.image_elems

    def _begin_ahead(self, n_steps):
        ahead = self._ahead_ok(n_steps)
        if ahead:
            self._run('g_ahead', self._generate_ahead)
        return ahead

    def _stage_ahead(self):
        if self._ahead is None:
            return ''
        B = self.B
        self.D.x.view(B, B).buf.copy_(self.G_ahead.layers[-1].h.view(self._ahead * B, B).buf)
        return '+ahead'

    def samples(self, n):
        h, w, c = self.args.image_shape
        n = min(n, self.B)
        self._rescale_real()
        self._generate(backward_follows=False)
        view = self.D.x.buf[:2 * self.B * h * w * self.D.x.cs].view(2, self.B, h, w, self.D.x.cs)
        both = view[:, :n, :, :, :c].float().cpu().numpy()
        return both[0], both[1]

    def _interpolate(self, out_slot=2):
        B = self.B
        self.sess.random_uniform(self.alpha, B, 'alpha')
        _lib.call('tdg_gp_interp', self.sess.dtype, self.D.x.ptr(0), self.D.x.ptr(B), K.ptr(self.alpha), B,
                  self.img_elems, self.D.x.ptr(out_slot * B), K.stream())

    def _d_forward(self, first_slot, nslots):
        B = self.B
        if self.iwgan:
            self.D.forward(first_slot * B, nslots * B)
        else:
            for s in range(first_slot, first_slot + nslots):
                self.D.forward(s * B, B, bn_pass=s)
        return self.D.layers[-1].out

    def _means(self, scores):
        R = self.B * self.rows_per_image
        _lib.call('tdg_mean_segments_f32', K.ptr(scores, 0), 2, R, K.ptr(self.scal, 4 * self.S_DREAL), K.stream())

    def _seeds(self, *values):
        bufs = self.__dict__.setdefault('_seed_bufs', {})
        buf = bufs.get(values)
        if buf is None:
            R = self.B * self.rows_per_image
            buf = torch.zeros_like(self.D.layers[-1].seed)
            for slot, v in enumerate(values):
                if v is not None:
                    buf[slot * R:(slot + 1) * R] = v
            bufs[values] = buf
        self.D.layers[-1].seed = buf

    def _penalty_from_v(self, tangent_seed=False, slot=2):
        B = self.B
        if self.gp_per_sample:
            if self._pen_rows is None:
                self._pen_rows = torch.zeros(B, dtype=torch.float32, device=self.sess.device)
                self._u_sink = K.Act(B, *self.args.image_shape, self.sess.dtype, self.sess.device) if not self.D.tangent_capacity else None
            u = self.D.tan_in if self.D.tangent_capacity else self._u_sink
            _lib.call('tdg_gp_rows', self.sess.dtype, self.D.dx.ptr(slot * B), B, self.img_elems, GP_LAMBDA, K.ptr(self._pen_rows),
                      u.ptr(0), K.stream())
            _lib.call('tdg_mean_f32', K.ptr(self._pen_rows), B, K.ptr(self.scal, 4 * self.S_GP), K.stream())
            return
        w = self.ws.ensure(4096)
        _lib.call('tdg_gp_sumsq', self.sess.dtype, self.D.dx.ptr(slot * B), B * self.img_elems, K.ptr(self.scal, 4 * self.S_SUMSQ), GP_LAMBDA,
                  K.ptr(self.scal, 4 * self.S_GP), K.ptr(w), w.numel(), K.stream())
        if tangent_seed:
            _lib.call('tdg_scale_by_dev', self.sess.dtype, self.D.dx.ptr(slot * B), B * self.img_elems,
                      K.ptr(self.scal, 4 * self.S_GPCOEF), self.D.tan_in.ptr(0), K.stream())

    def big_slice(self):
        big, store = self._d_big_layer, self.d_store
        lo, hi = store.index[big.wname][0], store.index[big.bname][0] + (big.spec.out_size + 3) // 4 * 4
        if all(L.rowdot for L in self.D.layers[big.idx + 1:]) and self.D.n_bn_passes == 1 and not any(L.spec.normed for L in self.D.layers):
            hi = store.size
        return lo, hi

    def d_step(self, x01):
        self._load_real(x01)
        sess, store = self.sess, self.d_store
        tag = self._stage_ahead()
        if sess.world_size > 1 and self.iwgan and os.environ.get('TDG_DSPLIT', '1') != '0':
            lo, hi = self.big_slice()
            self._run('d_grads_a' + tag, self._d_grads_a)
            self._scale = sess.allreduce_split(store.grads, lo, hi, between=lambda: self._run('d_grads_b', self._d_grads_b))
            sess.assert_finite(store, 'd_step')
            self._run('d_apply', self._d_apply)
            self.sess.global_step += 1
        elif sess.world_size == 1 and not sess.check_numerics and os.environ.get('TDG_ONE_BODY', '1') != '0':
            self._scale = 1.0
            self._run('d_step' + tag, self._d_grads_and_apply)
            self.sess.global_step += 1
        else:
            self.optimizer_step(store, ('d_grads' + tag, self._d_grads), ('d_apply', self._d_apply), 'd_step')

    def _d_grads_and_apply(self):
        self._d_grads()
        self._d_apply()

    def _g_grads_and_apply(self):
        self._g_grads()
        self._g_apply()

    def _d_apply(self):
        self.d_opt.step(self._scale)
        self.D.repack()

    def _g_apply(self):
        self.g_opt.step(self._scale)
        self.G.repack()

    def _d_grads(self):
        self._d_grads_a(whole=True)

    def _clip_critic(self):
        c = float(getattr(self.args, 'wgan_clip', 0.0) or 0.0)
        if c > 0.0:
            _lib.call('tdg_clamp', K.ptr(self.d_store.params), self.d_store.size, -c, c, K.stream())
            self.D.repack()

    def _d_grads_a(self, whole=False):
        B, R = self.B, self.B * self.rows_per_image
        self._clip_critic()
        self._rescale_real()
        if self._ahead is None:
            self._generate(backward_follows=False)
        if self.iwgan:
            self._interpolate()
        scores = self._d_forward(0, self.nslots)
        self._means(scores)
        self._seeds(-1.0 / R, 1.0 / R, 1.0) if self.iwgan else self._seeds(-1.0 / R, 1.0 / R)
        if self.iwgan:
            self.D.backward(0, 3 * B, want_params=True, want_dx=True, param_images=(0, 2 * B), dx_images=(2 * B, B),
                            defer_wgrad=True)
            self._penalty_from_v(tangent_seed=True)
            self.D.tangent_forward(2 * B, B, acc=True)
            convs = list(reversed(self.D.conv_layers())) if whole else [self._d_big_layer]
            self.D.merged_wgrad(2 * B, B, convs)
        else:
            self.D.backward(0, B, bn_pass=0, want_params=True, acc=False)
            self.D.backward(B, B, bn_pass=1, want_params=True, acc=True)

    def _d_grads_b(self):
        if self.iwgan:
            rest = [L for L in reversed(self.D.conv_layers()) if L is not self._d_big_layer]
            self.D.merged_wgrad(2 * self.B, self.B, rest)

    def g_step(self, x01):
        if self.display_d_loss:
            self._load_real(x01)
        sess, store = self.sess, self.g_store
        if sess.world_size > 1 and self.iwgan and self.display_d_loss and os.environ.get('TDG_GSPLIT', '1') != '0':
            self._run('g_grads_a', self._g_grads_critical)
            work = sess.allreduce_async(store.grads)
            self._run('g_grads_b', self._g_display_d_loss)
            work.wait()
            sess.assert_finite(store, 'g_step')
            self._scale = 1.0 / sess.world_size
            self._run('g_apply', self._g_apply)
            self.sess.global_step += 1
        elif sess.world_size == 1 and not sess.check_numerics and os.environ.get('TDG_ONE_BODY', '1') != '0':
            self._scale = 1.0
            self._run('g_step', self._g_grads_and_apply)
            self.sess.global_step += 1
        else:
            self.optimizer_step(store, ('g_grads', self._g_grads), ('g_apply', self._g_apply), 'g_step')

    def _g_grads_critical(self):
        B, R = self.B, self.B * self.rows_per_image
        self._generate()
        scores = self._d_forward(1, 1)
        _lib.call('tdg_mean_f32', K.ptr(scores, 4 * R), R, K.ptr(self.scal, 4 * self.S_DFAKE), K.stream())
        self._seeds(None, -1.0 / R)
        self.D.backward(B, B, want_params=False, want_dx=True)
        self.G.backward(0, B, want_params=True)

    def _g_display_d_loss(self):
        B, R = self.B, self.B * self.rows_per_image
        self._rescale_real()
        self._interpolate(out_slot=1)
        scores = self._d_forward(0, 2)
        _lib.call('tdg_mean_f32', K.ptr(scores, 0), R, K.ptr(self.scal, 4 * self.S_DREAL), K.stream())
        self._seeds(None, 1.0)
        self.D.backward(B, B, want_params=False, want_dx=True)
        self._penalty_from_v(slot=1)

    def _g_grads(self):
        B, R = self.B, self.B * self.rows_per_image
        self._generate()
        if self.display_d_loss:
            self._rescale_real()
            if self.iwgan:
                self._interpolate()
            scores = self._d_forward(0, self.nslots)
        else:
            scores = self._d_forward(1, 1)
        self._means(scores)
        if self.iwgan and self.display_d_loss:
            self._seeds(None, -1.0 / R, 1.0)
            self.D.backward(B, 2 * B, want_params=False, want_dx=True)
            self._penalty_from_v()
        else:
            self._seeds(None, -1.0 / R)
            self.D.backward(B, B, bn_pass=1, want_params=False, want_dx=True)
        self.G.backward(0, B, want_params=True)

    def _gan_grads(self):
        B, R = self.B, self.B * self.rows_per_image
        last = self.D.layers[-1]
        self._rescale_real()
        self._generate()
        scores = self._d_forward(0, 2)
        if self._seed_g is None:
            self._seed_g = torch.zeros(R, dtype=torch.float32, device=self.sess.device)
        _lib.call('tdg_gan_logloss', K.ptr(scores, 0), K.ptr(scores, 4 * R), R, K.ptr(last.seed, 0), K.ptr(last.seed, 4 * R),
                  K.ptr(self._seed_g), K.ptr(self.scal, 4 * self.S_GAN_D), K.stream())
        self.D.backward(0, B, bn_pass=0, want_params=True, acc=False)
        self.D.backward(B, B, bn_pass=1, want_params=True, acc=True)
        last.seed[R:2 * R].copy_(self._seed_g)
        self.D.backward(B, B, bn_pass=1, want_params=False, want_dx=True)
        self.G.backward(0, B, want_params=True)

    def _gan_apply(self):
        self.d_opt.step(self._scale)
        self.g_opt.step(self._scale)
        self.D.repack()
        self.G.repack()

    def gan_step(self, x01):
        self._load_real(x01)
        self._run('gan_grads', self._gan_grads)
        self.sess.assert_finite(self.d_store, 'gan_step')
        self.sess.assert_finite(self.g_store, 'gan_step')
        self._scale = average_gradients(self.sess, self.d_store)
        average_gradients(self.sess, self.g_store)
        self._run('gan_apply', self._gan_apply)
        self.sess.global_step += 2

    def losses(self):
        s = self.sess.report_scalars(self.scal, mean=getattr(self.args, 'mean_loss', False)).cpu().tolist()
        tower = self.sess.world_size - 1
        if self.model == 'gan':
            return collection_to_dict([('tower_%d/g_loss:0' % tower, s[self.S_GAN_G]),
                                       ('tower_%d/d_loss:0' % tower, s[self.S_GAN_D])])
        g_loss = -s[self.S_DFAKE]
        d_loss = s[self.S_DFAKE] - s[self.S_DREAL]
        if self.iwgan:
            d_loss += GP_LAMBDA * s[self.S_GP]
        return collection_to_dict([('tower_%d/g_loss:0' % tower, g_loss),
                                   ('tower_%d/d_loss:0' % tower, d_loss)])

    def train_func(self, sess=None, args=None):
        args = args or self.args
        if self.model == 'gan':
            self.gan_step(self.x_source.next_batch())
            return self.losses()
        ahead = self._begin_ahead(args.n_disc_train)
        try:
            for i in range(args.n_disc_train):
                self._ahead = i if ahead else None
                self.d_step(self.x_source.next_batch())
        finally:
            self._ahead = None
        self.g_step(self.x_source.next_batch())
        return self.losses()


def gan(x, args, sess=None):
    return GanReplica.train_function(x, args, sess)
```

### include/tdg.h

```cpp
#ifndef TDG_H_
#define TDG_H_

#include <stddef.h>
#include <stdint.h>

#ifdef __cplusplus
extern "C" {
#endif

#define TDG_OK 0
#define TDG_EINVAL (-1)
#define TDG_EUNSUPPORTED (-2)
#define TDG_EHIP (-3)
#define TDG_EWORKSPACE (-4)

#define TDG_F32 0
#define TDG_BF16 1

#define TDG_ACT_NONE 0
#define TDG_ACT_RELU 1
#define TDG_ACT_LRELU 2
#define TDG_ACT_TANH 3
#define TDG_ACT_SIGMOID 4

#define TDG_MASK_NONE 0
#define TDG_MASK_LRELU 1
#define TDG_MASK_RELU 2

typedef struct TdgConvDesc {
  int32_t n, h, w, c, cs;
  int32_t oh, ow, k, ks;
  int32_t kh, kw, stride;
  int32_t pad_t, pad_l;
  int32_t dtype;
} TdgConvDesc;

typedef struct TdgEpilogue {
  const float* bias;
  int32_t act;
  float leak;
  int32_t mask_mode;
  const void* mask_src;
  int32_t accumulate;
  float* col_partial;
  size_t col_partial_bytes;
  int32_t col_mode;
  int32_t col_images;
  int32_t* col_nblk_out;
  void* splitk_ws;
  size_t splitk_ws_bytes;
} TdgEpilogue;
enum { TDG_COL_NONE = 0, TDG_COL_SUM = 1, TDG_COL_BN = 2 };

const char* tdg_last_error(void);
int tdg_version(void);
const char* tdg_last_kernel(void);

typedef struct TdgLaunchRecord {
  char kernel[64];
  double ms;
  double flops;
} TdgLaunchRecord;
int tdg_timing_begin(void);
int tdg_timing_end(TdgLaunchRecord* out, int capacity, int* count);

size_t tdg_packed_filter_fwd_bytes(const TdgConvDesc* d);
size_t tdg_packed_filter_bwd_bytes(const TdgConvDesc* d);
int tdg_pack_filter_fwd(const TdgConvDesc* d, const float* w, void* packed, void* stream);
int tdg_pack_filter_bwd(const TdgConvDesc* d, const float* w, void* packed, void* stream);

typedef struct TdgPackJob {
  TdgConvDesc desc;
  const float* w;
  void* packed_fwd;
  void* packed_bwd;
} TdgPackJob;
int tdg_pack_filters(const TdgPackJob* jobs, int n_jobs, void* stream);

int tdg_conv2d_fwd(const TdgConvDesc* d, int n_images, const void* x, const void* w_packed_fwd,
                   void* y, const TdgEpilogue* epi, void* stream);
int tdg_conv2d_bwd_data(const TdgConvDesc* d, int n_images, const void* y, const void* w_packed_bwd,
                        void* x, const TdgEpilogue* epi, void* stream);
size_t tdg_conv2d_bwd_filter_workspace_bytes(const TdgConvDesc* d, int n_images);
int tdg_conv2d_bwd_filter(const TdgConvDesc* d, int n_images, const void* x, const void* y,
                          float* dw, float beta, void* workspace, size_t workspace_bytes, void* stream);
int tdg_conv2d_bwd_filter2(const TdgConvDesc* d, int n_images, const void* x, int n_first, const void* x2, const void* y,
                           float* dw, float beta, void* workspace, size_t workspace_bytes, void* stream);
enum { TDG_FORM_FWD = 0, TDG_FORM_BWD_DATA = 1, TDG_FORM_BWD_FILTER = 2 };
int tdg_conv2d_dispatch(const TdgConvDesc* d, int n_images, int form, const TdgEpilogue* epi, int n_first, char* name,
                        size_t name_bytes);

int tdg_rowdot(int dtype, const void* x, int rows, int cols, const float* w, const float* bias,
               int act, float* out, void* stream);
int tdg_rowouter(int dtype, const float* dout, const float* w, int rows, int cols, int mask_mode,
                 float leak, const void* mask_src, void* dx, void* stream);
int tdg_col_finalize_sum(const float* partial, int nblk, int c, float* out, float beta, void* stream);
int tdg_colsum_weighted(int dtype, const void* x, int rows, int cols, int cs, const float* coef,
                        float* dw, float beta, void* workspace, size_t workspace_bytes, void* stream);
size_t tdg_colsum_workspace_bytes(int rows, int cols);

size_t tdg_bn_workspace_bytes(int rows, int c);
int tdg_bn_fwd(int dtype, const void* u, int rows, int c, int cs, const float* beta, float eps,
               int act, float leak, void* pre, void* h, int h_cs, float* stats, void* workspace,
               size_t workspace_bytes, void* stream);
int tdg_bn_fwd_groups(int dtype, const void* u, int rows_per_group, int ngroups, int c, int cs, const float* beta,
                      float eps, int act, float leak, void* pre, void* h, int h_cs, float* stats, void* workspace,
                      size_t workspace_bytes, void* stream);
int tdg_instance_norm_fwd(int dtype, const void* u, int n, int hw, int c, int cs, const float* scale, const float* shift,
                          float eps, int act, float leak, void* h, int h_cs, float* stats, void* stream);
int tdg_instance_norm_bwd(int dtype, const void* dh, int dh_cs, const void* u, int n, int hw, int c, int cs, const float* scale,
                          const float* shift, const float* stats, int act, float leak, void* du, float* dscale, float* dshift,
                          float beta, void* workspace, size_t workspace_bytes, void* stream);
int tdg_add_act(int dtype, const void* a, const void* b, size_t n, int act, float leak, void* out, void* stream);
int tdg_bn_fwd_from_partials(int dtype, const void* u, int rows, int c, int cs, const float* beta, float eps, int act,
                             float leak, void* pre, void* h, int h_cs, float* stats, const float* partial, int nblk,
                             const float* pivot_bias, void* stream);
int tdg_bn_bwd(int dtype, const void* dh, int dh_cs, const void* pre, int rows, int c, int cs,
               const float* beta, const float* stats, int act, float leak, void* du, float* dbeta,
               float beta_acc, float* dbias, float dbias_acc, void* workspace, size_t workspace_bytes, void* stream);

int tdg_bias_act(int dtype, const void* x, int rows, int c, int cs, const float* bias, int act,
                 float leak, void* y, void* stream);
int tdg_act_bwd(int dtype, const void* dy, const void* post, size_t n, int act, float leak, void* dx,
                void* stream);
int tdg_affine_cast(int dtype, const float* in, size_t n, float scale, float shift, void* out, void* stream);
int tdg_affine_cast_pair(int dtype, const float* a, int ca, const float* b, int cb, size_t rows, float scale, float shift,
                         void* out_ab, void* out_a0, void* stream);
int tdg_affine_cast_rows(int dtype, const float* in, int rows, int c, int cs, float scale, float shift, void* out,
                         void* stream);
int tdg_cast_to_f32(int dtype, const void* in, size_t n, float* out, void* stream);
int tdg_cast_from_f32(int dtype, const float* in, size_t n, void* out, void* stream);
int tdg_gp_interp(int dtype, const void* x, const void* g, const float* alpha, int rows, int cols,
                  void* xhat, void* stream);
int tdg_sumsq(int dtype, const void* x, size_t n, float* acc, float beta, void* workspace,
              size_t workspace_bytes, void* stream);
size_t tdg_reduce_workspace_bytes(size_t n);
int tdg_mean_f32(const float* x, int n, float* out, void* stream);
int tdg_sum_f32(const float* x, int n, float* out, float beta, void* stream);
int tdg_mean_segments_f32(const float* x, int nseg, int seglen, float* out, void* stream);
int tdg_gan_logloss(const float* d_real, const float* d_fake, int n, float* seed_real, float* seed_fake_d,
                    float* seed_fake_g, float* scal, void* stream);
int tdg_p2p_xent(int dtype, const void* logits, int rows, int cs, int mode, void* seed, float* scal, void* stream);
int tdg_p2p_l1(int dtype, const void* y, const void* g, int rows, int cs, float weight, void* dg, int dgs, float* scal,
               void* workspace, size_t workspace_bytes, void* stream);
int tdg_cgan_prep(int dtype, const float* y, int n, int version, void* depth_real, int depth_cs, void* depth_fake, float* ybar,
                  float* crop, void* g_ones, int g_cs, void* rgb_ybar, int rgb_cs, void* stream);
int tdg_cgan_head_fwd(int dtype, const void* cat, int n, int hw, int cin, int cs, int crop, const float* w, const float* b,
                      const float* ybar, float* yhat, void* fake, int fake_cs, void* stream);
int tdg_cgan_head_bwd(int dtype, const void* dfake, int fake_cs, const void* cat, int n, int hw, int cin, int cs, int crop,
                      const float* w, int mask_mode, float leak, void* dcat, float* dw, float* db, void* workspace,
                      size_t workspace_bytes, void* stream);
int tdg_cgan_head_noise_fwd(int dtype, const void* cat, int n, int hw, int cin, int cs, int crop, const float* w, const float* b,
                            const float* u, const float* ybar, float* yhat, float* g, void* fake, int fake_cs, void* stream);
int tdg_cgan_head_noise_bwd(int dtype, const void* dfake, int fake_cs, const void* cat, int n, int hw, int cin, int cs, int crop,
                            const float* w, const float* u, int mask_mode, float leak, void* dcat, float* dw, float* db,
                            void* workspace, size_t workspace_bytes, void* stream);
int tdg_cgan_join(int dtype, int mode, int n_rgb, int rows, int c, void* comb, int comb_cs, void* rgb, int rgb_cs, void* depth,
                  int depth_cs, void* stream);
int tdg_cgan_wgan_loss(int dtype, const void* logits, int rows, int cs, int mode, void* seed, float* scal, void* stream);
int tdg_cgan_metrics(const float* y, const float* pred, const float* offset, int n, int hw, unsigned long long* counts, float* out,
                     void* workspace, size_t workspace_bytes, void* stream);
size_t tdg_cgan_metrics_workspace_bytes(void);
int tdg_cgan_eval_batch(const float* y, const float* pred, const float* offset, const float* image, float image_scale, int n, int hw,
                        int sets, unsigned long long* counts, double* acc, void* workspace, size_t workspace_bytes, void* stream);
size_t tdg_cgan_eval_workspace_bytes(void);
size_t tdg_cgan_eval_acc_bytes(int hw);
int tdg_cgan_eval_moments(const float* y, int n, int hw, double* acc, void* stream);
int tdg_cgan_sample_stats(const float* y, const float* g, const float* pred, const float* offset, const float* image,
                          float image_scale, int n, int hw, float unit, float* out, float* mean_img, float* var_img,
                          void* workspace, size_t workspace_bytes, void* stream);
size_t tdg_cgan_sample_stats_workspace_bytes(int n, int hw);
int tdg_cgan_rmse_loss(int dtype, const float* y, const float* yhat, int n, int hw, void* dg, int dg_cs, float* scal,
                       void* workspace, size_t workspace_bytes, void* stream);
size_t tdg_cgan_rmse_loss_workspace_bytes(int n, int hw);
int tdg_cgan_bar_fill(int dtype, const float* ybar, int n, int hw2, void* win, int win_cs, float* plane, void* stream);
int tdg_mde_loss(int dtype, const float* y_full, int n, int hw, const void* m, int m_cs, float* mean_out, void* seed, int seed_cs,
                 float* scal, void* workspace, size_t workspace_bytes, void* stream);
size_t tdg_mde_loss_workspace_bytes(int n);
int tdg_xsamp_prep(int dtype, const float* x, const float* x_loc, const float* y_loc, const float* m, const float* y, const int* x_rows,
                   const int* y_rows, int n, int S, int T, int off, void* g_in, int g_cs, void* rgb_in, int rgb_cs, void* depth_real,
                   int depth_cs, float* target, void* stream);
int tdg_xsamp_head_fwd(int dtype, const void* cat, int n, int hw, int cin, int cs, const float* w, const float* b, float* g,
                       void* fake, int fake_cs, void* stream);
int tdg_xsamp_head_bwd(int dtype, const void* dfake, int fake_cs, const float* g, const void* cat, int n, int hw, int cin, int cs,
                       const float* w, int mask_mode, float leak, void* dcat, float* dw, float* db, void* workspace,
                       size_t workspace_bytes, void* stream);
int tdg_cgan_eval_finish(const double* acc, const unsigned long long* counts, int hw, float unit, double* scalars, float* mean_img,
                         float* var_img, void* stream);
int tdg_cgan_full_gather(const float* image, const float* depth, int H, int W, int stride, const int* chunk, int batch,
                         float* x_stage, float* y_stage, void* stream);
int tdg_cgan_full_store(const float* yhat, const float* ybar, int batch, long long slots, int* chunk, float* store_yhat,
                        float* store_ybar, void* stream);
int tdg_cgan_full_blend(const float* store_yhat, const float* store_ybar, long long slots, int H, int W, int stride, int offset,
                        float* canvas_yhat, float* canvas_g, void* stream);
int tdg_cgan_full_rmse(const float* depth, const float* canvas, int H, int W, double* out, void* workspace, size_t workspace_bytes,
                       void* stream);
int tdg_cgan_full_gather_rep(const float* image, const float* depth, int H, int W, int stride, const int* chunk, int batch, int rep,
                             float* x_stage, float* y_stage, void* stream);
int tdg_cgan_full_sample_store(const float* yhat, const float* ybar, const float* crop, int batch, int draws, long long slots,
                               int* chunk, float* store_yhat, float* store_var, float* store_ybar, float* store_err, void* stream);
int tdg_vae_reparam(int dtype, const void* heads, int hs, const void* eps, int es, int rows, int L, void* z, int zs,
                    void* stream);
int tdg_vae_reparam_bwd(int dtype, const void* dz, int zs, const void* eps, int es, int rows, int L, void* dheads, int hs,
                        void* stream);
int tdg_vae_reparam_bwd_kl(int dtype, const void* dz, int zs, const void* eps, int es, const void* heads, int hs_in,
                           float kl_weight, int rows, int L, void* dheads, int hs, void* stream);
int tdg_vae_kl(int dtype, const void* heads, int hs, int rows, int L, float* scal, void* workspace, size_t workspace_bytes,
               void* stream);
int tdg_vae_bce(int dtype, const float* x, const void* d, int rows, int c, int cs, void* seed, float* scal, void* workspace,
                size_t workspace_bytes, void* stream);
int tdg_l1_loss(int dtype, const float* x, const void* d, int rows, int c, int cs, float scale, float shift, void* seed,
                float* scal, void* workspace, size_t workspace_bytes, void* stream);
int tdg_dropout(int dtype, void* y, int rows, int c, int ycs, const float* u, float keep, void* stream);
int tdg_gp_scalars(const float* sumsq, float lambda, float* scal, void* stream);
int tdg_gp_sumsq(int dtype, const void* x, size_t n, float* sumsq, float lambda, float* scal, void* workspace,
                 size_t workspace_bytes, void* stream);
// ... 51 lines not shown
```

Measured before the change: 31730 images/sec.

## Defer gradient reduction finalizes into one multi-job kernel and fuse critic input prep

```diff
diff --git a/3dgan_amd/_lib.py b/3dgan_amd/_lib.py
--- a/3dgan_amd/_lib.py
+++ b/3dgan_amd/_lib.py
@@ -8,6 +8,8 @@
 ACT_NONE, ACT_RELU, ACT_LRELU, ACT_TANH, ACT_SIGMOID = 0, 1, 2, 3, 4
 MASK_NONE, MASK_LRELU, MASK_RELU = 0, 1, 2
 COL_NONE, COL_SUM, COL_BN = 0, 1, 2
+FIN_COLSUM, FIN_SUM, FIN_SLABS = 0, 1, 2
+FINALIZE_MAX_JOBS = 64
 
 
 class ConvDesc(C.Structure):
@@ -25,6 +27,16 @@
 
 class PackJob(C.Structure):
     _fields_ = [('desc', ConvDesc), ('w', C.c_void_p), ('packed_fwd', C.c_void_p), ('packed_bwd', C.c_void_p)]
+
+
+class FinalizeJob(C.Structure):
+    _fields_ = [('kind', C.c_int32), ('acc_f32', C.c_int32), ('src', C.c_void_p), ('out', C.c_void_p), ('n', C.c_int64),
+                ('stride', C.c_int64), ('count', C.c_int32), ('beta', C.c_float)]
+
+
+class SlabLayout(C.Structure):
+    _fields_ = [('ngroups', C.c_int32), ('nsplit', C.c_int32 * 2), ('reserved', C.c_int32), ('slab_stride', C.c_int64),
+                ('n', C.c_int64), ('bytes', C.c_size_t)]
 
 
 class LaunchRecord(C.Structure):
@@ -51,6 +63,14 @@
     'tdg_conv2d_bwd_filter': (_i, [_PD, _i, _vp, _vp, _vp, _f, _vp, _sz, _vp]),
     'tdg_conv2d_bwd_filter2': (_i, [_PD, _i, _vp, _i, _vp, _vp, _vp, _f, _vp, _sz, _vp]),
     'tdg_conv2d_dispatch': (_i, [_PD, _i, _i, _PE, _i, C.c_char_p, _sz]),
+    'tdg_conv2d_bwd_filter_slabs': (_i, [_PD, _i, _vp, _vp, _vp, _sz, C.POINTER(SlabLayout), _vp]),
+    'tdg_conv2d_bwd_filter2_slabs': (_i, [_PD, _i, _vp, _i, _vp, _vp, _vp, _sz, C.POINTER(SlabLayout), _vp]),
+    'tdg_conv2d_bwd_filter_slab_layout': (_i, [_PD, _i, _i, C.POINTER(SlabLayout)]),
+    'tdg_bias_grad_partial': (_i, [_i, _vp, _i, _i, _i, _vp, _sz, C.POINTER(_i), _vp]),
+    'tdg_colsum_weighted_partial': (_i, [_i, _vp, _i, _i, _i, _vp, _vp, _sz, C.POINTER(_i), _vp]),
+    'tdg_col_partial_bytes': (_sz, [_i, _i, _i, _i]),
+    'tdg_finalize_multi': (_i, [C.POINTER(FinalizeJob), _i, _vp]),
+    'tdg_critic_inputs': (_i, [_i, _vp, _i, _i, _i, _i, _f, _f, _vp, _vp, _vp, _vp, _vp, _vp]),
     'tdg_rowdot': (_i, [_i, _vp, _i, _i, _vp, _vp, _i, _vp, _vp]),
     'tdg_rowouter': (_i, [_i, _vp, _vp, _i, _i, _i, _f, _vp, _vp, _vp]),
     'tdg_col_finalize_sum': (_i, [_vp, _i, _i, _vp, _f, _vp]),
diff --git a/3dgan_amd/csrc/tdg_elementwise.hip b/3dgan_amd/csrc/tdg_elementwise.hip
--- a/3dgan_amd/csrc/tdg_elementwise.hip
+++ b/3dgan_amd/csrc/tdg_elementwise.hip
@@ -3,6 +3,7 @@
 #include <atomic>
 
 #include "tdg_common.h"
+#include "tdg_reduce.h"
 #include <type_traits>
 
 static thread_local char g_err[512] = "";
@@ -303,13 +304,13 @@
 };
 #define FIN_CH 8
 template <typename T, int MODE, int CH>
-__global__ void __launch_bounds__(256) col_finalize_kernel(const FinArgs a) {
+__device__ __forceinline__ void col_finalize_body(const FinArgs& a, const int bx, const int by, const unsigned tid,
+                                                  typename std::conditional<sizeof(T) == 4, double, float>::type (*sh)[256 / CH][CH]) {
   constexpr int RL = 256 / CH;
   using Acc = typename std::conditional<sizeof(T) == 4, double, float>::type;
-  __shared__ Acc sh[2][RL][CH];
-  const int tx = threadIdx.x & (CH - 1), ty = threadIdx.x / CH;
-  const int c = blockIdx.x * CH + tx;
-  const float* const partial = a.partial + (size_t)blockIdx.y * a.nblk * 2 * a.C;
+  const int tx = tid & (CH - 1), ty = tid / CH;
+  const int c = bx * CH + tx;
+  const float* const partial = a.partial + (size_t)by * a.nblk * 2 * a.C;
   Acc s0 = 0, s1 = 0;
   if (c < a.C)
     for (int b0 = ty; b0 < a.nblk; b0 += 4 * RL) {
@@ -329,14 +330,14 @@
   __syncthreads();
   if (ty != 0 || c >= a.C) return;
   s0 = s1 = 0;
-#pragma unroll
+#pragma unroll 8
   for (int k = 0; k < RL; ++k) { s0 += sh[0][k][tx]; s1 += sh[1][k][tx]; }
   const Acc inv = (Acc)1 / (Acc)a.rows;
   if (MODE == FIN_BN_STATS) {
-    const float pivot = a.pivot_f ? a.pivot_f[c] : (a.x0 ? to_f32<T>(static_cast<const T*>(a.x0)[(size_t)blockIdx.y * a.x0_group + c]) : 0.f);
+    const float pivot = a.pivot_f ? a.pivot_f[c] : (a.x0 ? to_f32<T>(static_cast<const T*>(a.x0)[(size_t)by * a.x0_group + c]) : 0.f);
     const Acc md = s0 * inv;
     const Acc var = s1 * inv - md * md > 0 ? s1 * inv - md * md : 0;
-    float* const out = a.out0 + (size_t)blockIdx.y * 2 * a.C;
+    float* const out = a.out0 + (size_t)by * 2 * a.C;
     out[c] = (float)(pivot + md);
     out[a.C + c] = (float)(1.0 / sqrt((double)var + (double)a.eps));
   } else if (MODE == FIN_BN_BWD) {
@@ -349,6 +350,12 @@
   } else {
     a.out0[c] = (float)((a.beta_acc != 0.f ? (Acc)a.beta_acc * a.out0[c] : 0) + s0);
   }
+}
+template <typename T, int MODE, int CH>
+__global__ void __launch_bounds__(256) col_finalize_kernel(const FinArgs a) {
+  using Acc = typename std::conditional<sizeof(T) == 4, double, float>::type;
+  __shared__ Acc sh[2][256 / CH][CH];
+  col_finalize_body<T, MODE, CH>(a, blockIdx.x, blockIdx.y, threadIdx.x, sh);
 }
 template <typename T, int MODE>
 static void launch_col_finalize(const FinArgs& f, hipStream_t s, int ngroups = 1) {
@@ -642,6 +649,38 @@
   })
   TDG_HIP_LAUNCH_CHECK("colsum_weighted");
   return TDG_OK;
+}
+
+static int col_partial_only(const char* who, int dtype, const void* x, int rows, int c, int cs, const float* coef, bool weighted,
+                            float* partial, size_t partial_bytes, int* nblk_out, void* stream) {
+  TDG_CHECK_ARG(x && partial && nblk_out && rows > 0 && c > 0 && cs >= c, "%s: bad argument", who);
+  const ColGeom g = col_geom(rows, c, cs, x, nullptr, tdg_dtype_size(dtype));
+  if (partial_bytes < (size_t)g.nblk * 2 * c * sizeof(float)) {
+    tdg_set_error("%s: partial buffer %zu < %zu bytes", who, partial_bytes, (size_t)g.nblk * 2 * c * sizeof(float));
+    return TDG_EWORKSPACE;
+  }
+  ColArgs a; memset(&a, 0, sizeof(a));
+  a.x = x; a.coef = coef; a.partial = partial;
+  DISPATCH_T(dtype, {
+    const int rc = weighted ? run_col_partial<T, COL_WSUM>(g, a, (hipStream_t)stream) : run_col_partial<T, COL_SUM>(g, a, (hipStream_t)stream);
+    if (rc) return rc;
+  })
+  *nblk_out = g.nblk;
+  return TDG_OK;
+}
+extern "C" int tdg_bias_grad_partial(int dtype, const void* dy, int rows, int c, int cs, float* partial, size_t partial_bytes,
+                                     int* nblk_out, void* stream) {
+  return col_partial_only("tdg_bias_grad_partial", dtype, dy, rows, c, cs, nullptr, false, partial, partial_bytes, nblk_out, stream);
+}
+extern "C" int tdg_colsum_weighted_partial(int dtype, const void* x, int rows, int cols, int cs, const float* coef, float* partial,
+                                           size_t partial_bytes, int* nblk_out, void* stream) {
+  return col_partial_only("tdg_colsum_weighted_partial", dtype, x, rows, cols, cs, coef, true, partial, partial_bytes, nblk_out, stream);
+}
+extern "C" size_t tdg_col_partial_bytes(int dtype, int rows, int c, int cs) {
+  if (rows <= 0 || c <= 0 || cs < c) return 0;
+  const ColGeom g4 = col_geom(rows, c, cs, nullptr, nullptr, tdg_dtype_size(dtype));
+  const ColGeom g1 = col_geom(rows, c, cs, nullptr, nullptr, tdg_dtype_size(dtype), false);
+  return (size_t)(g4.nblk > g1.nblk ? g4.nblk : g1.nblk) * 2 * c * sizeof(float);
 }
 
 template <typename T>
@@ -1016,6 +1055,65 @@
   return TDG_OK;
 }
 
+template <typename T, bool VEC>
+__global__ void __launch_bounds__(256) critic_inputs_kernel(const float* __restrict__ in, size_t rows, int c, int cs, int pix_per_image,
+                                                           float scale, float shift, const T* __restrict__ g_src,
+                                                           const float* __restrict__ alpha, T* slot0, T* slot1, T* xhat) {
+  for (size_t r = blockIdx.x * (size_t)256 + threadIdx.x; r < rows; r += (size_t)gridDim.x * 256) {
+    const float al = alpha[r / (size_t)pix_per_image];
+    if constexpr (VEC) {
+      bf16x8 x8 = reinterpret_cast<const bf16x8*>(slot0)[r];
+#pragma unroll
+      for (int ch = 0; ch < 8; ++ch)
+        if (ch < c) x8[ch] = from_f32<bf16_t>(scale * (in[r * c + ch] + shift));
+      const bf16x8 g8 = g_src ? reinterpret_cast<const bf16x8*>(g_src)[r] : reinterpret_cast<const bf16x8*>(slot1)[r];
+      bf16x8 h8;
+#pragma unroll
+      for (int ch = 0; ch < 8; ++ch) {
+        const float xv = (float)x8[ch];
+        h8[ch] = from_f32<bf16_t>(xv + al * ((float)g8[ch] - xv));
+      }
+      reinterpret_cast<bf16x8*>(slot0)[r] = x8;
+      if (g_src) reinterpret_cast<bf16x8*>(slot1)[r] = g8;
+      reinterpret_cast<bf16x8*>(xhat)[r] = h8;
+    } else {
+      for (int ch = 0; ch < cs; ++ch) {
+        const size_t i = r * cs + ch;
+        T x = slot0[i];
+        if (ch < c) slot0[i] = x = from_f32<T>(scale * (in[r * c + ch] + shift));
+        const T g = g_src ? g_src[i] : slot1[i];
+        if (g_src) slot1[i] = g;
+        const float xv = to_f32<T>(x);
+        xhat[i] = from_f32<T>(xv + al * (to_f32<T>(g) - xv));
+      }
+    }
+  }
+}
+extern "C" int tdg_critic_inputs(int dtype, const float* in, int n_images, int pix_per_image, int c, int cs, float scale, float shift,
+                                 const void* g_src, const float* alpha, void* slot0, void* slot1, void* xhat, void* stream) {
+  TDG_CHECK_ARG(in && alpha && slot0 && slot1 && xhat && n_images > 0 && pix_per_image > 0 && c > 0 && cs >= c,
+                "tdg_critic_inputs: bad argument");
+  TDG_CHECK_ARG(slot0 != slot1 && slot0 != xhat && (xhat != slot1 || !g_src) && g_src != slot1 && g_src != xhat && g_src != slot0,
+                "tdg_critic_inputs: overlapping tensors (only xhat == slot1 without g_src is allowed)");
+  const size_t rows = (size_t)n_images * pix_per_image;
+  const bool vec = dtype == TDG_BF16 && cs == 8 &&
+                   ((((uintptr_t)slot0 | (uintptr_t)slot1 | (uintptr_t)xhat | (uintptr_t)g_src) & 15) == 0);
+  const dim3 grid(ew_blocks(rows, 256));
+  hipStream_t s = (hipStream_t)stream;
+  if (vec) {
+    hipLaunchKernelGGL((critic_inputs_kernel<bf16_t, true>), grid, dim3(256), 0, s, in, rows, c, cs, pix_per_image, scale, shift,
+                       static_cast<const bf16_t*>(g_src), alpha, static_cast<bf16_t*>(slot0), static_cast<bf16_t*>(slot1),
+                       static_cast<bf16_t*>(xhat));
+  } else {
+    DISPATCH_T(dtype, {
+      hipLaunchKernelGGL((critic_inputs_kernel<T, false>), grid, dim3(256), 0, s, in, rows, c, cs, pix_per_image, scale, shift,
+                         static_cast<const T*>(g_src), alpha, static_cast<T*>(slot0), static_cast<T*>(slot1), static_cast<T*>(xhat));
+    })
+  }
+  TDG_HIP_LAUNCH_CHECK("critic_inputs");
+  return TDG_OK;
+}
+
 #define RED_BLOCKS 256
 extern "C" size_t tdg_reduce_workspace_bytes(size_t) { return RED_BLOCKS * sizeof(float); }
 
@@ -1068,14 +1166,18 @@
     }
   }
 }
+__device__ __forceinline__ void reduce_final_body(const float* __restrict__ partial, int np, float* __restrict__ acc, float beta,
+                                                  float scale, const int seg, float* sh ) {
+  const float* p = partial + (size_t)seg * np;
+  float s = 0.f;
+  for (int i = threadIdx.x; i < np; i += 256) s += p[i];
+  s = block_sum256(s, sh);
+  if (threadIdx.x == 0) acc[seg] = (beta != 0.f ? beta * acc[seg] : 0.f) + scale * s;
+}
 __global__ void __launch_bounds__(256) reduce_final_kernel(const float* __restrict__ partial, int np, float* __restrict__ acc,
                                                           float beta, float scale) {
   __shared__ float sh[4];
-  const float* p = partial + (size_t)blockIdx.x * np;
-  float s = 0.f;
-  for (int i = threadIdx.x; i < np; i += 256) s += p[i];
-  s = block_sum256(s, sh);
-  if (threadIdx.x == 0) acc[blockIdx.x] = (beta != 0.f ? beta * acc[blockIdx.x] : 0.f) + scale * s;
+  reduce_final_body(partial, np, acc, beta, scale, blockIdx.x, sh);
 }
 __global__ void __launch_bounds__(256) reduce_mean_kernel(const float* __restrict__ partial, int np, float* __restrict__ out) {
   __shared__ float sh[4];
@@ -1126,6 +1228,128 @@
   hipLaunchKernelGGL(reduce_mean_kernel, dim3(1), dim3(256), 0, (hipStream_t)stream, x, n, out);
   TDG_HIP_LAUNCH_CHECK("mean_f32");
   return TDG_OK;
+}
+
+enum { FINJ_FOLLOWS = 1, FINJ_ACC_F32 = 2, FINJ_CH2 = 4, FINJ_FEW = 8, FINJ_WIDE = 16 };
+struct FinJobDev {
+  const float* src;
+  float* out;
+  long long n, stride;
+  int kind, count;
+  float beta;
+  int flags;
+};
+struct FinMultiArgs {
+  int njobs;
+  int start[TDG_FINALIZE_MAX_JOBS + 1];
+  FinJobDev job[TDG_FINALIZE_MAX_JOBS];
+};
+static_assert(sizeof(FinMultiArgs) <= 4096, "kernel argument block");
+
+__global__ void __launch_bounds__(256) finalize_multi_kernel(const FinMultiArgs m) {
+  __shared__ __attribute__((aligned(16))) char smem[4096];
+  int j = 0;
+  while (j + 1 < m.njobs && (int)blockIdx.x >= m.start[j + 1]) ++j;
+  const int local = blockIdx.x - m.start[j];
+  for (;;) {
+    unsigned tid = threadIdx.x;
+    asm volatile("" : "+v"(tid));
+    const FinJobDev& q = m.job[j];
+    if (q.kind == TDG_FIN_COLSUM) {
+      FinArgs f;
+      f.partial = q.src; f.nblk = q.count; f.C = (int)q.n; f.rows = 1; f.x0 = nullptr; f.pivot_f = nullptr; f.eps = 0.f;
+      f.out0 = q.out; f.out1 = nullptr; f.beta_acc = q.beta; f.x0_group = 0;
+      if (q.flags & FINJ_ACC_F32) {
+        if (q.flags & FINJ_CH2) col_finalize_body<bf16_t, FIN_ACC, 2>(f, local, 0, tid, reinterpret_cast<float (*)[128][2]>(smem));
+        else col_finalize_body<bf16_t, FIN_ACC, FIN_CH>(f, local, 0, tid, reinterpret_cast<float (*)[256 / FIN_CH][FIN_CH]>(smem));
+      } else {
+        if (q.flags & FINJ_CH2) col_finalize_body<float, FIN_ACC, 2>(f, local, 0, tid, reinterpret_cast<double (*)[128][2]>(smem));
+        else col_finalize_body<float, FIN_ACC, FIN_CH>(f, local, 0, tid, reinterpret_cast<double (*)[256 / FIN_CH][FIN_CH]>(smem));
+      }
+    } else if (q.kind == TDG_FIN_SUM) {
+      reduce_final_body(q.src, (int)q.n, q.out, q.beta, 1.f, 0, reinterpret_cast<float*>(smem));
+    } else if (q.flags & FINJ_FEW) {
+      slab_reduce_few_body(q.src, q.out, (size_t)q.n, q.count, (size_t)q.stride, q.beta, (size_t)local * 256 + tid);
+    } else if (q.flags & FINJ_WIDE) {
+      const size_t n4 = ((size_t)q.n + 3) >> 2;
+#pragma unroll 1
+      for (int p = 0; p < 16 && ((size_t)local * 16 + p) * 16 < n4; ++p) {
+        slab_reduce_body(q.src, q.out, (size_t)q.n, q.count, (size_t)q.stride, q.beta, (size_t)local * 16 + p, tid,
+                         reinterpret_cast<f32x4 (*)[16]>(smem));
+        __syncthreads();
+      }
+    } else {
+      slab_reduce_body(q.src, q.out, (size_t)q.n, q.count, (size_t)q.stride, q.beta, (size_t)local, tid, reinterpret_cast<f32x4 (*)[16]>(smem));
+    }
+    if (j + 1 >= m.njobs || !(m.job[j + 1].flags & FINJ_FOLLOWS)) break;
+    ++j;
+    __syncthreads();
+  }
+}
+
+static inline int finj_flags(const TdgFinalizeJob& q);
+static inline int finj_blocks(const TdgFinalizeJob& q) {
+  if (q.kind == TDG_FIN_COLSUM) return q.count >= 1024 ? (int)((q.n + 1) / 2) : (int)((q.n + FIN_CH - 1) / FIN_CH);
+  if (q.kind == TDG_FIN_SUM) return 1;
+  return (int)((((q.n + 3) / 4) + (finj_flags(q) & FINJ_FEW ? 255 : 15)) / (finj_flags(q) & FINJ_FEW ? 256 : 16));
+}
+static inline int finj_flags(const TdgFinalizeJob& q) {
+  if (q.kind == TDG_FIN_COLSUM) return (q.acc_f32 ? FINJ_ACC_F32 : 0) | (q.count >= 1024 ? FINJ_CH2 : 0);
+  if (q.kind == TDG_FIN_SLABS) return q.count <= 8 && ((uintptr_t)q.out & 15) == 0 ? FINJ_FEW : 0;
+  return 0;
+}
+extern "C" int tdg_finalize_multi(const TdgFinalizeJob* jobs, int n_jobs, void* stream) {
+  TDG_CHECK_ARG(jobs && n_jobs > 0 && n_jobs <= TDG_FINALIZE_MAX_JOBS, "tdg_finalize_multi: %d jobs outside [1, %d]", n_jobs,
+                TDG_FINALIZE_MAX_JOBS);
+  int leader[TDG_FINALIZE_MAX_JOBS];
+  for (int j = 0; j < n_jobs; ++j) {
+    const TdgFinalizeJob& q = jobs[j];
+    TDG_CHECK_ARG(q.kind == TDG_FIN_COLSUM || q.kind == TDG_FIN_SUM || q.kind == TDG_FIN_SLABS, "tdg_finalize_multi: job %d has kind %d", j, q.kind);
+    TDG_CHECK_ARG(q.src && q.out && q.n > 0 && q.n <= 0x7fffffffLL, "tdg_finalize_multi: job %d: null pointer or n = %lld", j, (long long)q.n);
+    if (q.kind != TDG_FIN_SUM) TDG_CHECK_ARG(q.count > 0, "tdg_finalize_multi: job %d: count %d", j, q.count);
+    if (q.kind == TDG_FIN_COLSUM) TDG_CHECK_ARG((long long)q.count * 2 * q.n <= 0x7fffffffLL * 64, "tdg_finalize_multi: job %d: partials too large", j);
+    if (q.kind == TDG_FIN_SLABS)
+      TDG_CHECK_ARG(((uintptr_t)q.src & 15) == 0 && q.stride % 4 == 0 && q.stride >= (q.n + 3) / 4 * 4,
+                    "tdg_finalize_multi: job %d: slabs must be 16-byte aligned with a stride >= round_up(n, 4) that is a multiple of 4 floats", j);
+    leader[j] = j;
+    const long long len = q.kind == TDG_FIN_SUM ? 1 : q.n;
+    for (int i = j - 1; i >= 0; --i) {
+      const TdgFinalizeJob& e = jobs[i];
+      const long long elen = e.kind == TDG_FIN_SUM ? 1 : e.n;
+      if (q.out + len <= e.out || e.out + elen <= q.out) continue;
+      TDG_CHECK_ARG(e.kind == q.kind && e.out == q.out && elen == len && (finj_flags(e) & FINJ_CH2) == (finj_flags(q) & FINJ_CH2),
+                    "tdg_finalize_multi: jobs %d and %d write overlapping outputs in different ways: launch them separately", i, j);
+      leader[j] = leader[i];
+      break;
+    }
+  }
+  static FinMultiArgs m;
+  m.njobs = 0;
+  m.start[0] = 0;
+  for (int l = 0; l < n_jobs; ++l) {
+    if (leader[l] != l) continue;
+    const int first = m.njobs;
+    bool few = false, many = false;
+    for (int j = l; j < n_jobs; ++j)
+      if (leader[j] == l && jobs[j].kind == TDG_FIN_SLABS) (finj_flags(jobs[j]) & FINJ_FEW ? few : many) = true;
+    const bool wide = few && many;
+    for (int j = l; j < n_jobs; ++j) {
+      if (leader[j] != l) continue;
+      const TdgFinalizeJob& q = jobs[j];
+      FinJobDev& d = m.job[m.njobs];
+      d.src = q.src; d.out = q.out; d.n = q.n; d.stride = q.stride; d.kind = q.kind; d.count = q.count; d.beta = q.beta;
+      d.flags = finj_flags(q) | (j != l ? FINJ_FOLLOWS : 0);
+      if (wide && !(d.flags & FINJ_FEW)) d.flags |= FINJ_WIDE;
+      ++m.njobs;
+    }
+    const long long end = (long long)m.start[first] + (wide ? (int)((((jobs[l].n + 3) / 4) + 255) / 256) : finj_blocks(jobs[l]));
+    TDG_CHECK_ARG(end <= 0x7fffffffLL, "tdg_finalize_multi: too many blocks");
+    for (int k = first + 1; k <= m.njobs; ++k) m.start[k] = (int)end;
+  }
+  hipStream_t s = (hipStream_t)stream;
+  return tdg_launch("finalize_multi", 0, 0.0, s, [&] {
+    hipLaunchKernelGGL(finalize_multi_kernel, dim3(m.start[m.njobs]), dim3(256), 0, s, m);
+  }, false);
 }
 
 __global__ void __launch_bounds__(256) gan_logloss_kernel(const float* __restrict__ dr, const float* __restrict__ df, int n,
diff --git a/3dgan_amd/csrc/tdg_igemm.hip b/3dgan_amd/csrc/tdg_igemm.hip
--- a/3dgan_amd/csrc/tdg_igemm.hip
+++ b/3dgan_amd/csrc/tdg_igemm.hip
@@ -3,6 +3,7 @@
 
 #include "tdg_igemm.h"
 #include "tdg_wgrad_patch.h"
+#include "tdg_reduce.h"
 #include <type_traits>
 
 #define OOB_OFFSET 0xFFFFFF00u
@@ -2343,44 +2344,12 @@
 __global__ void __launch_bounds__(256) slab_reduce_kernel(const float* __restrict__ slabs, float* __restrict__ dw,
                                                          size_t n, int nsplit, size_t stride, float beta) {
   __shared__ f32x4 sh[16][16];
-  const int tx = threadIdx.x & 15, tz = threadIdx.x >> 4;
-  const size_t n4 = (n + 3) >> 2;
-  const size_t i = (size_t)blockIdx.x * 16 + tx;
-  f32x4 s = {0.f, 0.f, 0.f, 0.f};
-  if (i < n4)
-    for (int z = tz; z < nsplit; z += 16) s += *reinterpret_cast<const f32x4*>(slabs + (size_t)z * stride + 4 * i);
-  sh[tz][tx] = s;
-  __syncthreads();
-  if (tz != 0 || i >= n4) return;
-  s = sh[0][tx];
-#pragma unroll
-  for (int k = 1; k < 16; ++k) s += sh[k][tx];
-#pragma unroll
-  for (int e = 0; e < 4; ++e)
-    if (4 * i + e < n) dw[4 * i + e] = (beta != 0.f ? beta * dw[4 * i + e] : 0.f) + s[e];
+  slab_reduce_body(slabs, dw, n, nsplit, stride, beta, blockIdx.x, threadIdx.x, sh);
 }
 
 __global__ void __launch_bounds__(256) slab_reduce_few_kernel(const float* __restrict__ slabs, float* __restrict__ dw,
                                                              size_t n, int nsplit, size_t stride, float beta) {
-  const size_t n4 = (n + 3) >> 2;
-  const size_t i = (size_t)blockIdx.x * 256 + threadIdx.x;
-  if (i >= n4) return;
-  f32x4 v[8];
-#pragma unroll
-  for (int z = 0; z < 8; ++z)
-    v[z] = z < nsplit ? *reinterpret_cast<const f32x4*>(slabs + (size_t)z * stride + 4 * i) : f32x4{0.f, 0.f, 0.f, 0.f};
-  f32x4 s = v[0];
-#pragma unroll
-  for (int z = 1; z < 8; ++z) s += v[z];
-  if (4 * i + 3 < n) {
-    f32x4 o = s;
-    if (beta != 0.f) o += beta * *reinterpret_cast<const f32x4*>(dw + 4 * i);
-    *reinterpret_cast<f32x4*>(dw + 4 * i) = o;
-  } else {
-#pragma unroll
-    for (int e = 0; e < 4; ++e)
-      if (4 * i + e < n) dw[4 * i + e] = (beta != 0.f ? beta * dw[4 * i + e] : 0.f) + s[e];
-  }
+  slab_reduce_few_body(slabs, dw, n, nsplit, stride, beta, (size_t)blockIdx.x * 256 + threadIdx.x);
 }
 
 struct PackArgs {
@@ -4369,34 +4338,46 @@
 }
 
 static int bwd_filter_impl(const TdgConvDesc* d, const ConvSwitches& sw, int n_images, const void* x, int n_first, const void* x2,
-                           const void* y, float* dw, float beta, void* workspace, size_t workspace_bytes, hipStream_t s, const char** dry);
+                           const void* y, float* dw, float beta, void* workspace, size_t workspace_bytes, hipStream_t s, const char** dry,
+                           TdgSlabLayout* defer = nullptr);
 
 static int conv_bwd_filter(const TdgConvDesc* d, int n_images, const void* x, const void* y, float* dw, float beta, void* workspace,
-                           size_t workspace_bytes, hipStream_t s, const char** dry) {
+                           size_t workspace_bytes, hipStream_t s, const char** dry, TdgSlabLayout* defer = nullptr) {
   const int rc = validate_wgrad(d, n_images);
   if (rc) return rc;
-  return bwd_filter_impl(d, conv_switches(), n_images, x, n_images, nullptr, y, dw, beta, workspace, workspace_bytes, s, dry);
+  return bwd_filter_impl(d, conv_switches(), n_images, x, n_images, nullptr, y, dw, beta, workspace, workspace_bytes, s, dry, defer);
+}
+
+static bool wgrad2_one_launch(const TdgConvDesc* d, int n_images, int n_first, const ConvSwitches& sw) {
+  return plan_wgrad(d, n_images, sw).dma && ((long long)n_first * d->oh * d->ow) % 2 == 0;
 }
 
 static int conv_bwd_filter2(const TdgConvDesc* d, int n_images, const void* x, int n_first, const void* x2, const void* y, float* dw,
-                            float beta, void* workspace, size_t workspace_bytes, hipStream_t s, const char** dry) {
+                            float beta, void* workspace, size_t workspace_bytes, hipStream_t s, const char** dry,
+                            TdgSlabLayout* defer = nullptr) {
   TDG_CHECK_ARG(n_first > 0 && n_first < n_images && x2, "tdg_conv2d_bwd_filter2: n_first %d outside (0, %d) or null x2", n_first, n_images);
   int rc = validate_wgrad(d, n_images);
   if (rc) return rc;
   const ConvSwitches sw = conv_switches();
-  if (plan_wgrad(d, n_images, sw).dma && ((long long)n_first * d->oh * d->ow) % 2 == 0)
-    return bwd_filter_impl(d, sw, n_images, x, n_first, x2, y, dw, beta, workspace, workspace_bytes, s, dry);
-  rc = bwd_filter_impl(d, sw, n_first, x, n_first, nullptr, y, dw, beta, workspace, workspace_bytes, s, dry);
+  if (wgrad2_one_launch(d, n_images, n_first, sw))
+    return bwd_filter_impl(d, sw, n_images, x, n_first, x2, y, dw, beta, workspace, workspace_bytes, s, dry, defer);
+  rc = bwd_filter_impl(d, sw, n_first, x, n_first, nullptr, y, dw, beta, workspace, workspace_bytes, s, dry, defer);
   if (rc) return rc;
   const char* y2 = static_cast<const char*>(y) + (size_t)n_first * d->oh * d->ow * d->ks * tdg_dtype_size(d->dtype);
   const int n2 = n_images - n_first;
-  return bwd_filter_impl(d, sw, n2, x2, n2, nullptr, y2, dw, 1.0f, workspace, workspace_bytes, s, dry);
+  if (defer) {
+    const size_t used = (size_t)defer->nsplit[0] * (size_t)defer->slab_stride * sizeof(float);
+    workspace = static_cast<char*>(workspace) + used;
+    workspace_bytes = workspace_bytes > used ? workspace_bytes - used : 0;
+  }
+  return bwd_filter_impl(d, sw, n2, x2, n2, nullptr, y2, dw, 1.0f, workspace, workspace_bytes, s, dry, defer);
 }
 
 static int bwd_filter_impl(const TdgConvDesc* d, const ConvSwitches& sw, int n_images, const void* x, int n_first, const void* x2,
-                           const void* y, float* dw, float beta, void* workspace, size_t workspace_bytes, hipStream_t s, const char** dry) {
+                           const void* y, float* dw, float beta, void* workspace, size_t workspace_bytes, hipStream_t s, const char** dry,
+                           TdgSlabLayout* defer) {
   const WgradPlan p = plan_wgrad(d, n_images, sw);
-  TDG_CHECK_ARG(x && y && dw && workspace, "tdg_conv2d_bwd_filter: null pointer");
+  TDG_CHECK_ARG(x && y && (dw || defer) && workspace, "tdg_conv2d_bwd_filter: null pointer");
   if (workspace_bytes < p.ws_bytes) {
     tdg_set_error("tdg_conv2d_bwd_filter: workspace %zu < %zu bytes", workspace_bytes, p.ws_bytes);
     return TDG_EWORKSPACE;
@@ -4441,6 +4422,13 @@
   const int rc = launch_wgrad(a, c, conv_flops(d, n_images), s);
   if (rc) return rc;
   const size_t n = (size_t)a.ntaps * d->c * d->k;
+  if (defer) {
+    defer->nsplit[defer->ngroups++] = a.nsplit;
+    defer->slab_stride = a.slab_stride;
+    defer->n = (int64_t)n;
+    defer->bytes += (size_t)a.nsplit * (size_t)a.slab_stride * sizeof(float);
+    return TDG_OK;
+  }
   return tdg_launch("slab_reduce", 0, 0.0, s, [&] {
     if (a.nsplit <= 8 && ((uintptr_t)dw & 15) == 0) {
       hipLaunchKernelGGL(slab_reduce_few_kernel, dim3((unsigned)(((n + 3) / 4 + 255) / 256)), dim3(256), 0, s, a.slabs, dw, n, a.nsplit,
@@ -4460,6 +4448,41 @@
 int tdg_conv2d_bwd_filter2(const TdgConvDesc* d, int n_images, const void* x, int n_first, const void* x2, const void* y,
                            float* dw, float beta, void* workspace, size_t workspace_bytes, void* stream) {
   return conv_bwd_filter2(d, n_images, x, n_first, x2, y, dw, beta, workspace, workspace_bytes, (hipStream_t)stream, nullptr);
+}
+
+int tdg_conv2d_bwd_filter_slabs(const TdgConvDesc* d, int n_images, const void* x, const void* y, void* slabs, size_t slabs_bytes,
+                                TdgSlabLayout* layout, void* stream) {
+  TDG_CHECK_ARG(layout, "tdg_conv2d_bwd_filter_slabs: null layout");
+  memset(layout, 0, sizeof(*layout));
+  return conv_bwd_filter(d, n_images, x, y, nullptr, 0.f, slabs, slabs_bytes, (hipStream_t)stream, nullptr, layout);
+}
+
+int tdg_conv2d_bwd_filter2_slabs(const TdgConvDesc* d, int n_images, const void* x, int n_first, const void* x2, const void* y,
+                                 void* slabs, size_t slabs_bytes, TdgSlabLayout* layout, void* stream) {
+  TDG_CHECK_ARG(layout, "tdg_conv2d_bwd_filter2_slabs: null layout");
+  memset(layout, 0, sizeof(*layout));
+  return conv_bwd_filter2(d, n_images, x, n_first, x2, y, nullptr, 0.f, slabs, slabs_bytes, (hipStream_t)stream, nullptr, layout);
+}
+
+int tdg_conv2d_bwd_filter_slab_layout(const TdgConvDesc* d, int n_images, int n_first, TdgSlabLayout* layout) {
+  TDG_CHECK_ARG(layout, "tdg_conv2d_bwd_filter_slab_layout: null layout");
+  memset(layout, 0, sizeof(*layout));
+  const int rc = validate_wgrad(d, n_images);
+  if (rc) return rc;
+  TDG_CHECK_ARG(n_first >= 0 && n_first < n_images, "tdg_conv2d_bwd_filter_slab_layout: n_first %d outside [0, %d)", n_first, n_images);
+  const ConvSwitches sw = conv_switches();
+  layout->n = (int64_t)d->kh * d->kw * d->c * d->k;
+  layout->slab_stride = tdg_round_up(layout->n, 4);
+  if (n_first == 0 || wgrad2_one_launch(d, n_images, n_first, sw)) {
+    layout->ngroups = 1;
+    layout->nsplit[0] = plan_wgrad(d, n_images, sw).nsplit;
+  } else {
+    layout->ngroups = 2;
+    layout->nsplit[0] = plan_wgrad(d, n_first, sw).nsplit;
+    layout->nsplit[1] = plan_wgrad(d, n_images - n_first, sw).nsplit;
+  }
+  layout->bytes = (size_t)(layout->nsplit[0] + layout->nsplit[1]) * (size_t)layout->slab_stride * sizeof(float);
+  return TDG_OK;
 }
 
 int tdg_conv2d_dispatch(const TdgConvDesc* d, int n_images, int form, const TdgEpilogue* epi, int n_first, char* name, size_t name_bytes) {
diff --git a/3dgan_amd/csrc/tdg_reduce.h b/3dgan_amd/csrc/tdg_reduce.h
--- /dev/null
+++ b/3dgan_amd/csrc/tdg_reduce.h
@@ -0,0 +1,43 @@
+#pragma once
+#include "tdg_common.h"
+
+__device__ __forceinline__ void slab_reduce_body(const float* __restrict__ slabs, float* __restrict__ dw, size_t n, int nsplit,
+                                                 size_t stride, float beta, size_t blk, const unsigned tid, f32x4 (*sh)[16]) {
+  const int tx = tid & 15, tz = tid >> 4;
+  const size_t n4 = (n + 3) >> 2;
+  const size_t i = blk * 16 + tx;
+  f32x4 s = {0.f, 0.f, 0.f, 0.f};
+  if (i < n4)
+    for (int z = tz; z < nsplit; z += 16) s += *reinterpret_cast<const f32x4*>(slabs + (size_t)z * stride + 4 * i);
+  sh[tz][tx] = s;
+  __syncthreads();
+  if (tz != 0 || i >= n4) return;
+  s = sh[0][tx];
+#pragma unroll
+  for (int k = 1; k < 16; ++k) s += sh[k][tx];
+#pragma unroll
+  for (int e = 0; e < 4; ++e)
+    if (4 * i + e < n) dw[4 * i + e] = (beta != 0.f ? beta * dw[4 * i + e] : 0.f) + s[e];
+}
+
+__device__ __forceinline__ void slab_reduce_few_body(const float* __restrict__ slabs, float* __restrict__ dw, size_t n, int nsplit,
+                                                     size_t stride, float beta, size_t i) {
+  const size_t n4 = (n + 3) >> 2;
+  if (i >= n4) return;
+  f32x4 v[8];
+#pragma unroll
+  for (int z = 0; z < 8; ++z)
+    v[z] = z < nsplit ? *reinterpret_cast<const f32x4*>(slabs + (size_t)z * stride + 4 * i) : f32x4{0.f, 0.f, 0.f, 0.f};
+  f32x4 s = v[0];
+#pragma unroll
+  for (int z = 1; z < 8; ++z) s += v[z];
+  if (4 * i + 3 < n) {
+    f32x4 o = s;
+    if (beta != 0.f) o += beta * *reinterpret_cast<const f32x4*>(dw + 4 * i);
+    *reinterpret_cast<f32x4*>(dw + 4 * i) = o;
+  } else {
+#pragma unroll
+    for (int e = 0; e < 4; ++e)
+      if (4 * i + e < n) dw[4 * i + e] = (beta != 0.f ? beta * dw[4 * i + e] : 0.f) + s[e];
+  }
+}
diff --git a/3dgan_amd/engine.py b/3dgan_amd/engine.py
--- a/3dgan_amd/engine.py
+++ b/3dgan_amd/engine.py
@@ -1,4 +1,5 @@
 import collections
+import contextlib
 import ctypes as C
 import math
 
@@ -106,6 +107,22 @@
         self.size = 0
         self.params = self.grads = None
         self.views, self.grad_views = {}, {}
+        self.defer = None
+
+    @contextlib.contextmanager
+    def deferring(self, scope):
+        if scope is None:
+            yield
+            return
+        self.defer = scope
+        try:
+            yield
+        except BaseException:
+            scope.drop()
+            raise
+        finally:
+            self.defer = None
+        scope.flush()
 
     def declare(self, name, shape):
         if name in self.index:
@@ -526,6 +543,7 @@
         beta = 1.0 if acc else 0.0
         p0, pn = (img0, n) if param_images is None else param_images
         g = self.store.grad
+        dfr = self.store.defer if want_params else None
         have_db = None
         for L in reversed(self.layers):
             r0, rn = img0 * L.rpi, n * L.rpi
@@ -544,8 +562,11 @@
                 cols = L.spec.in_size
                 if want_params and qn > 0:
                     K.colsum_weighted(self.ws, self.dtype, L.inp.ptr(q0), qn, cols, cols, _sub(L.seed, q0, qn),
-                                      g(L.wname), beta)
-                    _lib.call('tdg_sum_f32', K.ptr(L.seed, 4 * q0), qn, K.ptr(g(L.bname)), beta, K.stream())
+                                      g(L.wname), beta, defer=dfr, key=('dw', id(L)))
+                    if dfr is not None:
+                        dfr.add(_lib.FIN_SUM, K.ptr(L.seed, 4 * q0), g(L.bname), qn, beta=beta)
+                    else:
+                        _lib.call('tdg_sum_f32', K.ptr(L.seed, 4 * q0), qn, K.ptr(g(L.bname)), beta, K.stream())
                 if need_in:
                     _lib.call('tdg_rowouter', self.dtype, K.ptr(L.seed, 4 * d0), K.ptr(self.store[L.wname]), dn, cols,
                               mmode, mleak, msrc.ptr(dimg * below.rpi) if msrc is not None else None, L.gin.ptr(d0), K.stream())
@@ -591,15 +612,16 @@
                 if have_db is not None and have_db[0] is L and have_db[1] is None:
                     pass
                 elif have_db is not None and have_db[0] is L and K.nblk(have_db[1]):
-                    K.bias_grad_from_partials(have_db[1], L.spec.out_size, g(L.bname), beta)
+                    K.bias_grad_from_partials(have_db[1], L.spec.out_size, g(L.bname), beta, defer=dfr)
                 else:
-                    K.bias_grad(self.ws, L.delta, L.spec.out_size, g(L.bname), rows=qn * hw, beta=beta, dy_ptr=L.delta.ptr(q0))
+                    K.bias_grad(self.ws, L.delta, L.spec.out_size, g(L.bname), rows=qn * hw, beta=beta, dy_ptr=L.delta.ptr(q0),
+                                defer=dfr, key=('db', id(L)))
                 if defer_wgrad:
                     pass
                 elif L.spec.kind == 'deconv2d':
-                    L.conv.bwd_filter(L.delta.ptr(q0), L.inp.ptr(q0), g(L.wname), qn, beta)
+                    L.conv.bwd_filter(L.delta.ptr(q0), L.inp.ptr(q0), g(L.wname), qn, beta, defer=dfr)
                 else:
-                    L.conv.bwd_filter(L.inp.ptr(q0), L.delta.ptr(q0), g(L.wname), qn, beta)
+                    L.conv.bwd_filter(L.inp.ptr(q0), L.delta.ptr(q0), g(L.wname), qn, beta, defer=dfr)
             if need_in:
                 mptr = msrc.ptr(dimg * below.rpi) if msrc is not None else None
                 fuse = (want_params and below is not None and not below.rowdot and not below.spec.normed and below.spec.kind != 'residual' and
@@ -607,7 +629,8 @@
                         L.rpi == 1 and below.rpi == 1 and p0 == img0 and 0 < pn <= n and (d0, dn) == (r0, rn))
                 if fuse:
                     epi = K.colsum_epilogue(self.ws, dn * below.h.h * below.h.w, below.spec.out_size, K.COL_SUM,
-                                            images=(pn if pn < n else 0), mask_mode=mmode, leak=mleak, mask_src=mptr)
+                                            images=(pn if pn < n else 0), defer=dfr, key=('db', id(below)),
+                                            mask_mode=mmode, leak=mleak, mask_src=mptr)
                     have_db = (below, epi)
                 else:
                     epi = K.epilogue(mask_mode=mmode, leak=mleak, mask_src=mptr)
@@ -626,7 +649,8 @@
             r0, rn = img0 * L.rpi, n * L.rpi
             if L.rowdot:
                 cols = L.spec.in_size
-                K.colsum_weighted(self.ws, self.dtype, t_prev.ptr(0), rn, cols, cols, None, g(L.wname), beta)
+                K.colsum_weighted(self.ws, self.dtype, t_prev.ptr(0), rn, cols, cols, None, g(L.wname), beta,
+                                  defer=self.store.defer, key=('dw_tan', id(L)))
                 break
             if L.spec.normed or L.spec.kind != 'conv2d' or L.act.code not in (K.ACT_LRELU, K.ACT_RELU):
                 raise NotImplementedError('tangent pass: layer %s is not a BN-free (l)relu conv' % L.spec.name)
@@ -647,7 +671,7 @@
         beta = 1.0 if acc else 0.0
         for L in layers:
             L.conv.bwd_filter2(L.inp.ptr(0), n_first * L.rpi, L.tan_src.ptr(0), L.delta.ptr(0), self.store.grad(L.wname),
-                               (n_first + n_tan) * L.rpi, beta)
+                               (n_first + n_tan) * L.rpi, beta, defer=self.store.defer)
 
     def tangent_backward(self, img0, n, acc=True):
         beta = 1.0 if acc else 0.0
diff --git a/3dgan_amd/kernels.py b/3dgan_amd/kernels.py
--- a/3dgan_amd/kernels.py
+++ b/3dgan_amd/kernels.py
@@ -91,11 +91,11 @@
     return e
 
 
-def colsum_epilogue(ws, rows, c, mode, images=0, **kw):
+def colsum_epilogue(ws, rows, c, mode, images=0, defer=None, key=None, **kw):
     e = epilogue(**kw)
     nblk_max = rows // 64 + 8
     nbytes = nblk_max * 2 * c * 4
-    buf = ws.ensure(nbytes)
+    buf = ws.ensure(nbytes) if defer is None else defer.buffer(key, nbytes)
     e.col_partial, e.col_partial_bytes, e.col_mode, e.col_images = buf.data_ptr(), nbytes, mode, images
     e._nblk = C.c_int32(0)
     e.col_nblk_out = C.pointer(e._nblk)
@@ -106,7 +106,9 @@
     return int(e._nblk.value) if hasattr(e, '_nblk') else 0
 
 
-def bias_grad_from_partials(e, c, db, beta=0.0):
+def bias_grad_from_partials(e, c, db, beta=0.0, defer=None):
+    if defer is not None:
+        return defer.add(_lib.FIN_COLSUM, e.col_partial, db, c, count=nblk(e), beta=beta)
     _lib.call('tdg_col_finalize_sum', C.c_void_p(e.col_partial), nblk(e), c, ptr(db), beta, stream())
 
 
@@ -177,6 +179,7 @@
         self.ws_bytes = lib.tdg_conv2d_bwd_filter_workspace_bytes(C.byref(self.desc), big.n)
         self.ws = None
         self.filter_shape = (kh, kw, big.c, small.c)
+        self._layouts, self._got = {}, _lib.SlabLayout()
 
     def workspace(self):
         if self.ws is None:
@@ -223,22 +226,52 @@
                       C.byref(epi) if epi is not None else None, stream())
         TIMER.wrap(self._tag('bwd_data'), self.flops(n_images), go) if TIMER is not None else go()
 
-    def bwd_filter(self, x_ptr, y_ptr, dw, n_images, beta=0.0):
-        ws = self.workspace()
+    def slab_layout(self, n_images, n_first=0):
+        lay = self._layouts.get((n_images, n_first))
+        if lay is None:
+            lay = self._layouts[(n_images, n_first)] = _lib.SlabLayout()
+            _lib.call('tdg_conv2d_bwd_filter_slab_layout', C.byref(self.desc), n_images, n_first, C.byref(lay))
+        return lay
+
+    def _deferrable(self, defer, n_images, n_first=0):
+        return self.slab_layout(n_images, n_first) if defer is not None else None
+
+    def _file_slabs(self, defer, buf, dw, beta):
+        lay, off = self._got, 0
+        for g in range(lay.ngroups):
+            defer.add(_lib.FIN_SLABS, buf.data_ptr() + off, dw, lay.n, count=lay.nsplit[g], beta=beta if g == 0 else 1.0,
+                      stride=lay.slab_stride)
+            off += lay.nsplit[g] * lay.slab_stride * 4
+
+    def bwd_filter(self, x_ptr, y_ptr, dw, n_images, beta=0.0, defer=None):
+        lay = self._deferrable(defer, n_images)
+        ws = self.workspace() if lay is None else defer.buffer(('slabs', id(self)), lay.bytes)
 
         def go():
-            _lib.call('tdg_conv2d_bwd_filter', C.byref(self.desc), n_images, x_ptr, y_ptr, ptr(dw), beta,
-                      ptr(ws), ws.numel(), stream())
+            if lay is None:
+                _lib.call('tdg_conv2d_bwd_filter', C.byref(self.desc), n_images, x_ptr, y_ptr, ptr(dw), beta,
+                          ptr(ws), ws.numel(), stream())
+            else:
+                _lib.call('tdg_conv2d_bwd_filter_slabs', C.byref(self.desc), n_images, x_ptr, y_ptr, ptr(ws), ws.numel(),
+                          C.byref(self._got), stream())
         TIMER.wrap(self._tag('bwd_filter'), self.flops(n_images), go) if TIMER is not None else go()
-
-
-    def bwd_filter2(self, x_ptr, n_first, x2_ptr, y_ptr, dw, n_images, beta=0.0):
-        ws = self.workspace()
+        if lay is not None:
+            self._file_slabs(defer, ws, dw, beta)
+
+    def bwd_filter2(self, x_ptr, n_first, x2_ptr, y_ptr, dw, n_images, beta=0.0, defer=None):
+        lay = self._deferrable(defer, n_images, n_first)
+        ws = self.workspace() if lay is None else defer.buffer(('slabs', id(self)), lay.bytes)
 
         def go():
-            _lib.call('tdg_conv2d_bwd_filter2', C.byref(self.desc), n_images, x_ptr, n_first, x2_ptr, y_ptr, ptr(dw), beta,
-                      ptr(ws), ws.numel(), stream())
+            if lay is None:
+                _lib.call('tdg_conv2d_bwd_filter2', C.byref(self.desc), n_images, x_ptr, n_first, x2_ptr, y_ptr, ptr(dw), beta,
+                          ptr(ws), ws.numel(), stream())
+            else:
+                _lib.call('tdg_conv2d_bwd_filter2_slabs', C.byref(self.desc), n_images, x_ptr, n_first, x2_ptr, y_ptr, ptr(ws),
+                          ws.numel(), C.byref(self._got), stream())
         TIMER.wrap(self._tag('bwd_filter'), self.flops(n_images), go) if TIMER is not None else go()
+        if lay is not None:
+            self._file_slabs(defer, ws, dw, beta)
 
 
 class Workspace:
@@ -254,6 +287,42 @@
         return self.buf
 
 
+class Deferred:
+
+    def __init__(self, device):
+        self.device = device
+        self.jobs, self._pool, self._uses, self._retired = [], {}, {}, []
+
+    def buffer(self, key, nbytes):
+        k = self._uses.get(key, 0)
+        self._uses[key] = k + 1
+        bufs = self._pool.setdefault(key, [])
+        if k < len(bufs) and bufs[k].numel() >= nbytes:
+            return bufs[k]
+        if torch.cuda.is_current_stream_capturing():
+            raise RuntimeError('deferred reduction %r needs %d bytes that the warm-up pass did not allocate' % (key, nbytes))
+        buf = torch.empty(max(int(nbytes), 16), dtype=torch.uint8, device=self.device)
+        if k < len(bufs):
+            self._retired.append(bufs[k])
+            bufs[k] = buf
+        else:
+            bufs.append(buf)
+        return buf
+
+    def add(self, kind, src, out, n, count=0, beta=0.0, stride=0, acc_f32=False):
+        src = src.value if isinstance(src, C.c_void_p) else int(src)
+        self.jobs.append(_lib.FinalizeJob(kind, 1 if acc_f32 else 0, src, out.data_ptr(), int(n), int(stride), int(count), float(beta)))
+
+    def flush(self):
+        jobs, self.jobs, self._uses = self.jobs, [], {}
+        for i in range(0, len(jobs), _lib.FINALIZE_MAX_JOBS):
+            part = jobs[i:i + _lib.FINALIZE_MAX_JOBS]
+            _lib.call('tdg_finalize_multi', (_lib.FinalizeJob * len(part))(*part), len(part), stream())
+
+    def drop(self):
+        self.jobs, self._uses = [], {}
+
+
 def bn_fwd(ws, u, c, beta, act, pre, h, stats, rows=None, leak=0.2, eps=1e-3, u_ptr=None, pre_ptr=None, h_ptr=None):
     rows = u.rows if rows is None else rows
     lib = _lib.load()
@@ -281,14 +350,24 @@
               ptr(w), w.numel(), stream())
 
 
-def bias_grad(ws, dy, c, db, rows=None, beta=0.0, dy_ptr=None):
+def bias_grad(ws, dy, c, db, rows=None, beta=0.0, dy_ptr=None, defer=None, key=None):
     rows = dy.rows if rows is None else rows
+    if defer is not None:
+        buf = defer.buffer(key, _lib.load().tdg_col_partial_bytes(dy.dtype, rows, c, dy.cs))
+        nb = C.c_int(0)
+        _lib.call('tdg_bias_grad_partial', dy.dtype, dy_ptr or dy.ptr(), rows, c, dy.cs, ptr(buf), buf.numel(), C.byref(nb), stream())
+        return defer.add(_lib.FIN_COLSUM, buf.data_ptr(), db, c, count=nb.value, beta=beta, acc_f32=dy.dtype == BF16)
     need = _lib.load().tdg_bn_workspace_bytes(rows, c)
     w = ws.ensure(need)
     _lib.call('tdg_bias_grad', dy.dtype, dy_ptr or dy.ptr(), rows, c, dy.cs, ptr(db), beta, ptr(w), w.numel(), stream())
 
 
-def colsum_weighted(ws, dtype, x_ptr, rows, cols, cs, coef, dw, beta=0.0):
+def colsum_weighted(ws, dtype, x_ptr, rows, cols, cs, coef, dw, beta=0.0, defer=None, key=None):
+    if defer is not None:
+        buf = defer.buffer(key, _lib.load().tdg_col_partial_bytes(dtype, rows, cols, cs))
+        nb = C.c_int(0)
+        _lib.call('tdg_colsum_weighted_partial', dtype, x_ptr, rows, cols, cs, ptr(coef), ptr(buf), buf.numel(), C.byref(nb), stream())
+        return defer.add(_lib.FIN_COLSUM, buf.data_ptr(), dw, cols, count=nb.value, beta=beta, acc_f32=dtype == BF16)
     need = _lib.load().tdg_colsum_workspace_bytes(rows, cols)
     w = ws.ensure(need)
     _lib.call('tdg_colsum_weighted', dtype, x_ptr, rows, cols, cs, ptr(coef), ptr(dw), beta, ptr(w), w.numel(), stream())
diff --git a/3dgan_amd/models/gan.py b/3dgan_amd/models/gan.py
--- a/3dgan_amd/models/gan.py
+++ b/3dgan_amd/models/gan.py
@@ -105,6 +105,7 @@
         (self.x_stage,) = self.staging((B, h, w, c))
         self._seed_g = None
         self.alpha = torch.zeros(B, dtype=torch.float32, device=dev)
+        self._defer = K.Deferred(dev) if os.environ.get('TDG_DEFER', '1') != '0' else None
         self.scal = torch.zeros(16, dtype=torch.float32, device=dev)
         self.refresh()
 
@@ -144,6 +145,8 @@
         if self._ahead is None:
             return ''
         B = self.B
+        if self.iwgan and self._defer is not None:
+            return '+ahead%s' % (self._ahead or '')
         self.D.x.view(B, B).buf.copy_(self.G_ahead.layers[-1].h.view(self._ahead * B, B).buf)
         return '+ahead'
 
@@ -161,6 +164,17 @@
         self.sess.random_uniform(self.alpha, B, 'alpha')
         _lib.call('tdg_gp_interp', self.sess.dtype, self.D.x.ptr(0), self.D.x.ptr(B), K.ptr(self.alpha), B,
                   self.img_elems, self.D.x.ptr(out_slot * B), K.stream())
+
+    def _critic_inputs(self, out_slot=2, ahead=None):
+        if self._defer is None:
+            self._rescale_real()
+            return self._interpolate(out_slot)
+        B = self.B
+        h, w, c = self.args.image_shape
+        self.sess.random_uniform(self.alpha, B, 'alpha')
+        g_src = self.G_ahead.layers[-1].h.ptr(ahead * B) if ahead is not None else None
+        _lib.call('tdg_critic_inputs', self.sess.dtype, K.ptr(self.x_stage), B, h * w, c, self.D.x.cs, 2.0, -0.5, g_src,
+                  K.ptr(self.alpha), self.D.x.ptr(0), self.D.x.ptr(B), self.D.x.ptr(out_slot * B), K.stream())
 
     def _d_forward(self, first_slot, nslots):
         B = self.B
@@ -231,11 +245,13 @@
             self.optimizer_step(store, ('d_grads' + tag, self._d_grads), ('d_apply', self._d_apply), 'd_step')
 
     def _d_grads_and_apply(self):
-        self._d_grads()
+        with self.d_store.deferring(self._defer):
+            self._d_grads()
         self._d_apply()
 
     def _g_grads_and_apply(self):
-        self._g_grads()
+        with self.g_store.deferring(self._defer):
+            self._g_grads()
         self._g_apply()
 
     def _d_apply(self):
@@ -258,10 +274,14 @@
     def _d_grads_a(self, whole=False):
         B, R = self.B, self.B * self.rows_per_image
         self._clip_critic()
-        self._rescale_real()
+        one_launch = self.iwgan and self._defer is not None
+        if not one_launch:
+            self._rescale_real()
         if self._ahead is None:
             self._generate(backward_follows=False)
-        if self.iwgan:
+        if one_launch:
+            self._critic_inputs(ahead=self._ahead)
+        elif self.iwgan:
             self._interpolate()
         scores = self._d_forward(0, self.nslots)
         self._means(scores)
@@ -272,6 +292,8 @@
             self._penalty_from_v(tangent_seed=True)
             self.D.tangent_forward(2 * B, B, acc=True)
             convs = list(reversed(self.D.conv_layers())) if whole else [self._d_big_layer]
+            if whole and self.d_store.defer is not None:
+                convs.reverse()
             self.D.merged_wgrad(2 * B, B, convs)
         else:
             self.D.backward(0, B, bn_pass=0, want_params=True, acc=False)
@@ -313,8 +335,7 @@
 
     def _g_display_d_loss(self):
         B, R = self.B, self.B * self.rows_per_image
-        self._rescale_real()
-        self._interpolate(out_slot=1)
+        self._critic_inputs(out_slot=1)
         scores = self._d_forward(0, 2)
         _lib.call('tdg_mean_f32', K.ptr(scores, 0), R, K.ptr(self.scal, 4 * self.S_DREAL), K.stream())
         self._seeds(None, 1.0)
@@ -325,9 +346,10 @@
         B, R = self.B, self.B * self.rows_per_image
         self._generate()
         if self.display_d_loss:
-            self._rescale_real()
             if self.iwgan:
-                self._interpolate()
+                self._critic_inputs()
+            else:
+                self._rescale_real()
             scores = self._d_forward(0, self.nslots)
         else:
             scores = self._d_forward(1, 1)
diff --git a/include/tdg.h b/include/tdg.h
--- a/include/tdg.h
+++ b/include/tdg.h
@@ -86,6 +86,19 @@
                           float* dw, float beta, void* workspace, size_t workspace_bytes, void* stream);
 int tdg_conv2d_bwd_filter2(const TdgConvDesc* d, int n_images, const void* x, int n_first, const void* x2, const void* y,
                            float* dw, float beta, void* workspace, size_t workspace_bytes, void* stream);
+typedef struct TdgSlabLayout {
+  int32_t ngroups;
+  int32_t nsplit[2];
+  int32_t reserved;
+  int64_t slab_stride;
+  int64_t n;
+  size_t bytes;
+} TdgSlabLayout;
+int tdg_conv2d_bwd_filter_slabs(const TdgConvDesc* d, int n_images, const void* x, const void* y, void* slabs, size_t slabs_bytes,
+                                TdgSlabLayout* layout, void* stream);
+int tdg_conv2d_bwd_filter2_slabs(const TdgConvDesc* d, int n_images, const void* x, int n_first, const void* x2, const void* y,
+                                 void* slabs, size_t slabs_bytes, TdgSlabLayout* layout, void* stream);
+int tdg_conv2d_bwd_filter_slab_layout(const TdgConvDesc* d, int n_images, int n_first, TdgSlabLayout* layout);
 enum { TDG_FORM_FWD = 0, TDG_FORM_BWD_DATA = 1, TDG_FORM_BWD_FILTER = 2 };
 int tdg_conv2d_dispatch(const TdgConvDesc* d, int n_images, int form, const TdgEpilogue* epi, int n_first, char* name,
                         size_t name_bytes);
@@ -98,6 +111,25 @@
 int tdg_colsum_weighted(int dtype, const void* x, int rows, int cols, int cs, const float* coef,
                         float* dw, float beta, void* workspace, size_t workspace_bytes, void* stream);
 size_t tdg_colsum_workspace_bytes(int rows, int cols);
+
+int tdg_bias_grad_partial(int dtype, const void* dy, int rows, int c, int cs, float* partial, size_t partial_bytes,
+                          int* nblk_out, void* stream);
+int tdg_colsum_weighted_partial(int dtype, const void* x, int rows, int cols, int cs, const float* coef, float* partial,
+                                size_t partial_bytes, int* nblk_out, void* stream);
+size_t tdg_col_partial_bytes(int dtype, int rows, int c, int cs);
+enum { TDG_FIN_COLSUM = 0, TDG_FIN_SUM = 1, TDG_FIN_SLABS = 2 };
+#define TDG_FINALIZE_MAX_JOBS 64
+typedef struct TdgFinalizeJob {
+  int32_t kind;
+  int32_t acc_f32;
+  const float* src;
+  float* out;
+  int64_t n;
+  int64_t stride;
+  int32_t count;
+  float beta;
+} TdgFinalizeJob;
+int tdg_finalize_multi(const TdgFinalizeJob* jobs, int n_jobs, void* stream);
 
 size_t tdg_bn_workspace_bytes(int rows, int c);
 int tdg_bn_fwd(int dtype, const void* u, int rows, int c, int cs, const float* beta, float eps,
@@ -132,6 +164,8 @@
 int tdg_cast_from_f32(int dtype, const float* in, size_t n, void* out, void* stream);
 int tdg_gp_interp(int dtype, const void* x, const void* g, const float* alpha, int rows, int cols,
                   void* xhat, void* stream);
+int tdg_critic_inputs(int dtype, const float* in, int n_images, int pix_per_image, int c, int cs, float scale, float shift,
+                      const void* g_src, const float* alpha, void* slot0, void* slot1, void* xhat, void* stream);
 int tdg_sumsq(int dtype, const void* x, size_t n, float* acc, float beta, void* workspace,
               size_t workspace_bytes, void* stream);
 size_t tdg_reduce_workspace_bytes(size_t n);
```

Result: no change. 32000 images/sec (median of 6 runs) (+0.8%).
